# multiview-stitcher/multiview-stitcher

Measured on AMD Instinct MI355X. Metric: Mvoxels/s register+fuse, 3D tile grid, higher is better.
Workload: dtype u16 in/out, f32 accumulate, f64 coordinates

## Files before the change

multiview-stitcher_amd/csrc/mvs_context.hip:

```cpp
#include "mvs_internal.h"
#include <vector>
#include <algorithm>

#include <algorithm>
#include <cstring>

static MvsContext g_ctx[MVS_MAX_DEVICES * MVS_MAX_LANES];

MvsContext* mvs_ctx(int device) {
    if (device < 0 || (device & 0xff) >= MVS_MAX_DEVICES || (device >> 8) >= MVS_MAX_LANES) return nullptr;
    return &g_ctx[mvs_ctx_index(device)];
}

int mvs_fail(MvsContext* c, int code, const char* fmt, ...) {
    char buf[1024];
    va_list ap;
    va_start(ap, fmt);
    vsnprintf(buf, sizeof(buf), fmt, ap);
    va_end(ap);
    if (c) { c->last_error = buf; c->last_code = code; }
    return code;
}

int mvs_check_ready(int device, MvsContext** out) {
// ... 73 lines not shown
    *host = c->mbox_host;
    *dev = c->mbox_dev;
    return MVS_OK;
}

__global__ void mvs_small_copy_kernel(const uint4* __restrict__ src, uint4* __restrict__ dst, size_t n16) {
    for (size_t i = (size_t)blockIdx.x * blockDim.x + threadIdx.x; i < n16; i += (size_t)gridDim.x * blockDim.x) dst[i] = src[i];
}
int mvs_upload_from_mapped(MvsContext* c, void* dst_dev, const void* src_mapped_dev, size_t nbytes) {
    if ((((uintptr_t)dst_dev | (uintptr_t)src_mapped_dev) & 15) || (nbytes & 15))
        return mvs_fail(c, MVS_ERR_INVALID_ARG, "mvs_upload_from_mapped: 16-byte granularity");
    const size_t n16 = nbytes / 16;
    if (!n16) return MVS_OK;
    const unsigned blocks = (unsigned)std::min<size_t>((n16 + 255) / 256, 64);
    hipLaunchKernelGGL(mvs_small_copy_kernel, dim3(blocks), dim3(256), 0, c->stream, (const uint4*)src_mapped_dev, (uint4*)dst_dev, n16);
    MVS_HIP_TRY(c, hipGetLastError());
    return MVS_OK;
}

int mvs_ensure_aux_streams(MvsContext* c) {
    if (c->ev_fork) return MVS_OK;
    MVS_HIP_TRY(c, hipEventCreateWithFlags(&c->ev_fork, hipEventDisableTiming));
    int prio_lo = 0, prio_hi = 0;
    hipDeviceGetStreamPriorityRange(&prio_lo, &prio_hi);
    for (int a = 0; a < 4; ++a) {
        MVS_HIP_TRY(c, hipStreamCreateWithPriority(&c->aux_stream[a], hipStreamNonBlocking, prio_lo));
        MVS_HIP_TRY(c, hipEventCreateWithFlags(&c->ev_join[a], hipEventDisableTiming));
    }
    return MVS_OK;
}

__global__ void mvs_copy_bytes_kernel(const unsigned char* __restrict__ src, unsigned char* __restrict__ dst, size_t nbytes) {
    const size_t n16 = nbytes >> 4, tid = (size_t)blockIdx.x * blockDim.x + threadIdx.x, nth = (size_t)gridDim.x * blockDim.x;
    for (size_t i = tid; i < n16; i += nth) reinterpret_cast<uint4*>(dst)[i] = reinterpret_cast<const uint4*>(src)[i];
    for (size_t i = (n16 << 4) + tid; i < nbytes; i += nth) dst[i] = src[i];
}
int mvs_upload_small(MvsContext* c, void* dst_dev, const void* src_pinned, size_t nbytes) {
    if (!nbytes) return MVS_OK;
    void* sdev = nullptr;
    if (nbytes <= ((size_t)32 << 20) && !(((uintptr_t)dst_dev | (uintptr_t)src_pinned) & 15) &&
        hipHostGetDevicePointer(&sdev, const_cast<void*>(src_pinned), 0) == hipSuccess && sdev) {
        const unsigned blocks = (unsigned)std::min<size_t>(((nbytes >> 4) + 255) / 256 + 1, 512);
        hipLaunchKernelGGL(mvs_copy_bytes_kernel, dim3(blocks), dim3(256), 0, c->stream, (const unsigned char*)sdev, (unsigned char*)dst_dev, nbytes);
        MVS_HIP_TRY(c, hipGetLastError());
        return MVS_OK;
    }
    (void)hipGetLastError();
    MVS_HIP_TRY(c, hipMemcpyAsync(dst_dev, src_pinned, nbytes, hipMemcpyHostToDevice, c->stream));
    return MVS_OK;
}

void mvs_pinned_mark(MvsContext* c, int slot) {
    const int k = slot ? 1 : 0;
    if (hipEventRecord(c->pinned_ev[k], c->stream) == hipSuccess) c->pinned_pending[k] = true;
    else hipStreamSynchronize(c->stream);
}

static size_t pool_round(uint64_t nbytes) {
    if (nbytes == 0) nbytes = 1;
    const size_t q = nbytes >= ((size_t)1 << 20) ? ((size_t)2 << 20) : 4096;
    return (nbytes + q - 1) / q * q;
}

static void pool_flush(MvsContext* c) {
    if (c->pool_free.empty()) return;
    hipStreamSynchronize(c->stream);
    for (auto& kv : c->pool_free) hipFree(kv.second);
    c->pool_free.clear();
    c->pool_cached_bytes = 0;
}

struct MvsBoolOption { const char* key; bool MvsContext::* field; };
static const MvsBoolOption kBoolOptions[] = {
    {"force_generic", &MvsContext::force_generic},
    {"no_regions", &MvsContext::no_regions},
    {"deconv_general", &MvsContext::deconv_general},
    {"dct_general", &MvsContext::dct_general},
    {"rows_v1", &MvsContext::rows_v1},
    {"cb_mask_count", &MvsContext::cb_mask_count},
    {"cb_mask_closed_form", &MvsContext::cb_mask_closed_form},
    {"fuse_mixed", &MvsContext::fuse_mixed},
    {"serial_classes", &MvsContext::serial_classes},
    {"reg_unfused", &MvsContext::reg_unfused},
    {"ssim_two_pass", &MvsContext::ssim_two_pass},
    {"ssim_f32", &MvsContext::ssim_f32},
    {"ssim_prune", &MvsContext::ssim_prune},
    {"materialize_shifts", &MvsContext::materialize_shifts},
    {"cb_exact", &MvsContext::cb_exact},
    {"cb_blend_generic", &MvsContext::cb_blend_generic},
    {"cb_nosplit", &MvsContext::cb_nosplit},
    {"cb_unpaired", &MvsContext::cb_unpaired},
    {"fft_no_pair", &MvsContext::fft_no_pair},
    {"fft_no_slab", &MvsContext::fft_no_slab},
    {"fft_no_line", &MvsContext::fft_no_line},
};
static int set_option(MvsContext* c, const char* key, int64_t value) {
    for (const MvsBoolOption& e : kBoolOptions)
        if (!strcmp(key, e.key)) {
            c->*e.field = value != 0;
            return MVS_OK;
        }
    if (!strcmp(key, "pool_cache_limit_mb")) {
        std::lock_guard<std::mutex> plock(c->pool_mu);
        c->pool_cache_limit = (size_t)std::max<int64_t>(value, 0) << 20;
        if (c->pool_cached_bytes > c->pool_cache_limit) pool_flush(c);
        return MVS_OK;
    }
    if (!strcmp(key, "cb_taps_f64")) {
        if (value < 0 || value > 3) return mvs_fail(c, MVS_ERR_INVALID_ARG, "mvs_set_option: cb_taps_f64 is 0, 1, 2 or 3");
        c->cb_taps = (int)value;
        return MVS_OK;
    }
    if (!strcmp(key, "fft_slab_axes")) {
        if (value < 0 || value > 7) return mvs_fail(c, MVS_ERR_INVALID_ARG, "mvs_set_option: fft_slab_axes is a mask of 3 bits");
        c->fft_slab_axes = (int)value;
        return MVS_OK;
    }
    if (!strcmp(key, "ablate")) {
        c->ablate = (int)value;
        return MVS_OK;
    }
    return mvs_fail(c, MVS_ERR_INVALID_ARG, "mvs_set_option: unknown key '%s'", key);
}
struct MvsCounter { const char* key; double MvsContext::* real; long long MvsContext::* count; };
static const MvsCounter kCounters[] = {
    {"reg_alg_bytes", &MvsContext::reg_alg_bytes, nullptr},
    {"reg_alg_bytes_full", &MvsContext::reg_alg_bytes_full, nullptr},
    {"reg_pairs", nullptr, &MvsContext::reg_pairs},
    {"reg_candidates", nullptr, &MvsContext::reg_candidates},
    {"reg_rewalks", nullptr, &MvsContext::reg_rewalks},
    {"reg_pruned", nullptr, &MvsContext::reg_pruned},
    {"reg_cand_volumes", &MvsContext::reg_cand_volumes, nullptr},
    {"reg_slab_pairs", nullptr, &MvsContext::reg_slab_pairs},
    {"cb_mask_views", nullptr, &MvsContext::cb_mask_views},
    {"cb_mask_boxes", nullptr, &MvsContext::cb_mask_boxes},
    {"cb_line_launches", nullptr, &MvsContext::cb_line_launches},
    {"cb_overflows_redone", nullptr, &MvsContext::cb_overflows},
};

double mvs_rows_last_plan_ms(MvsContext* c);
double mvs_regions_last_plan_ms(MvsContext* c);
double mvs_regions_class_stat(MvsContext* c, int what, int cls);

extern "C" {

const char* mvs_version(void) { return "mvs_hip 0.1 (gfx950)"; }

int mvs_device_count(void) {
    int n = 0;
    if (hipGetDeviceCount(&n) != hipSuccess) return 0;
    return n;
}

int mvs_init(int device) {
    MvsContext* c = mvs_ctx(device);
    if (!c) return MVS_ERR_INVALID_ARG;
    std::lock_guard<std::recursive_mutex> lock(c->mu);
    if (c->ready) return MVS_OK;
    int n = 0;
    hipError_t e = hipGetDeviceCount(&n);
    if (e != hipSuccess || mvs_hip_device(device) >= n)
        return mvs_fail(c, MVS_ERR_HIP, "no HIP device %d (count=%d, %s)", mvs_hip_device(device), n,
                        hipGetErrorString(e));
    MVS_HIP_TRY(c, hipSetDevice(mvs_hip_device(device)));
    {
        const char* ev = nullptr;
#ifdef MVS_PROFILING_ABLATIONS
        ev = getenv("MVS_LANE_CU_MASK");
        if (ev) {
            const size_t pre = !strncmp(ev, "xcd", 3) ? 3 : (!strncmp(ev, "spread", 6) ? 6 : 0);
            if (!pre || ev[pre] < '1' || ev[pre] > '8' || ev[pre + 1] != '\0') ev = nullptr;
        }
#endif
        const int lane = (device >> 8) & 0xff;
        bool masked = false;
        if (ev && lane < 15) {
            hipDeviceProp_t prop;
            MVS_HIP_TRY(c, hipGetDeviceProperties(&prop, mvs_hip_device(device)));
            const int ncu = prop.multiProcessorCount;
            const bool xcd = !strncmp(ev, "xcd", 3);
            const int k = std::max(1, std::min(8, atoi(ev + (xcd ? 3 : 6))));
            std::vector<uint32_t> mask((size_t)(ncu + 31) / 32, 0u);
            for (int i = 0; i < ncu; ++i) {
                bool on;
                if (xcd) { const int x = i % 8, first = (lane * k) % 8; on = ((x - first + 8) % 8) < k; }
                else { const int slot = (i / 8) % 8, first = (lane * k) % 8; on = ((slot - first + 8) % 8) < k; }
                if (on) mask[(size_t)i / 32] |= 1u << (i % 32);
            }
            if (hipExtStreamCreateWithCUMask(&c->own_stream, (uint32_t)mask.size(), mask.data()) == hipSuccess) masked = true;
            else (void)hipGetLastError();
        }
        if (!masked) MVS_HIP_TRY(c, hipStreamCreateWithFlags(&c->own_stream, hipStreamNonBlocking));
    }
    MVS_HIP_TRY(c, hipEventCreate(&c->ev_start));
    MVS_HIP_TRY(c, hipEventCreate(&c->ev_stop));
    MVS_HIP_TRY(c, hipEventCreateWithFlags(&c->pinned_ev[0], hipEventDisableTiming));
    MVS_HIP_TRY(c, hipEventCreateWithFlags(&c->pinned_ev[1], hipEventDisableTiming));
    c->pinned_pending[0] = c->pinned_pending[1] = false;
    c->stream = c->own_stream;
    c->device = device;
    c->pool_cache_limit = ((device >> 8) ? (size_t)4 : (size_t)32) << 30;
    if (((device >> 8) & 0xff) == 0) {
        size_t f = 0, t = 0;
        if (hipMemGetInfo(&f, &t) == hipSuccess) c->pool_cache_limit = std::max(c->pool_cache_limit, t / 2);
        else (void)hipGetLastError();
    }
    {
        static const char* const env_switch[][2] = {{"MVS_SSIM_PRUNE", "ssim_prune"},   {"MVS_SSIM_F32", "ssim_f32"},
                                                    {"MVS_FUSE_MIXED", "fuse_mixed"},   {"MVS_FFT_SLAB_AXES", "fft_slab_axes"},
                                                    {"MVS_FFT_NO_SLAB", "fft_no_slab"}, {"MVS_FFT_NO_PAIR", "fft_no_pair"}};
        for (const auto& e : env_switch) {
            const char* ev = getenv(e[0]);
            if (ev && *ev) (void)set_option(c, e[1], atoi(ev));
        }
    }
    c->ready = true;
// ... 401 lines not shown
```

multiview-stitcher_amd/csrc/mvs_fft.h:

```cpp
#pragma once
#include "mvs_internal.h"

struct MvsFftFuse {
    const float* re_src = nullptr;
    const float* im_src = nullptr;
    const float2* xp_src = nullptr;
    float2* xp_p2 = nullptr;
    int xp_sel_a = 0, xp_sel_b = 0;
    bool xp_used = false;
    float* peak_val[2] = {nullptr, nullptr};
    long long* peak_idx[2] = {nullptr, nullptr};
    int peak_cap = 0;
    int n_peak = 0;
    bool src_used = false;
};
int mvs_fft3_c2c(MvsContext* c, float2* data, const int64_t shape[3], bool inverse, MvsFftFuse* fuse = nullptr);
int mvs_phasecorr_slab_axis(const MvsContext* c, const int64_t shape[3]);
int mvs_phasecorr_slab_peaks(const int64_t shape[3], int short_axis);
int mvs_phasecorr_slab(MvsContext* c, const float* a, const float* b, float2* Z, float2* CC, float2* P2, float2* dc, const int64_t shape[3],
                       int short_axis, int sel_a, int sel_b, float* const peak_val[2], long long* const peak_idx[2], float2* z0_out);
bool mvs_fft_reg_length(int n);

__device__ __forceinline__ void mvs_xpower_scales(float2 z0, long long n, float* scale_phase, float* scale_plain) {
    const float dc = fabsf(z0.x * z0.y);
    *scale_plain = (dc > 0.f && dc < INFINITY) ? ldexpf(1.f, -ilogbf(dc)) : 1.f;
    *scale_phase = ldexpf(1.f, -ilogbf((float)n));
}
__device__ __forceinline__ float2 mvs_xpower_value(float2 z, float2 m, int sel_a, int sel_b, float scale_phase, float scale_plain,
                                                   float2* p_out, float2* p1_out) {
    const float floor_ = 100.f * 1.1920928955078125e-7f;
    const float2 f = make_float2(0.5f * (z.x + m.x), 0.5f * (z.y - m.y));
    const float2 g = make_float2(0.5f * (z.y + m.y), -0.5f * (z.x - m.x));
    const float2 p = make_float2(f.x * g.x + f.y * g.y, f.y * g.x - f.x * g.y);
    const float a = fmaxf(hypotf(p.x, p.y), floor_);
    const float2 p1 = make_float2(p.x / a, p.y / a);
    *p_out = p;
    *p1_out = p1;
    const float2 pa = sel_a ? p1 : p;
    if (sel_b < 0) return pa;
    const float2 pb = sel_b ? p1 : p;
    const float sa = sel_a ? scale_phase : scale_plain, sb = sel_b ? scale_phase : scale_plain;
    return make_float2(pa.x * sa - pb.y * sb, pa.y * sa + pb.x * sb);
}
```

multiview-stitcher_amd/csrc/mvs_fft.hip:

```cpp
#include "mvs_fft.h"
#include "mvs_fft_dev.h"
#include "mvs_fft_reg.h"

#include <cmath>
#include <cstdlib>
#include <map>
#include <vector>

namespace {




__device__ __forceinline__ float2* stockham(float2* a, float2* b, int lpb, int M, int log2M, const float2* tw, bool inv) {
    const int half = M >> 1, quarter = M >> 2;
    const int log2q = log2M - 2;
    int s = 0;
    for (; s + 2 <= log2M; s += 2) {
        const int p = 1 << s;
        const int tstep = M >> (s + 2);
        for (int t = threadIdx.x; t < (lpb << log2q); t += blockDim.x) {
            const int line = t >> log2q, i = t & (quarter - 1);
            const int k = i & (p - 1);
            const int j = ((i - k) << 2) + k;
// ... 536 lines not shown
        rc = launch_pow2_lines(c, scr, p.M1, (long long)nl * p.M2, p.M2, p.M2, p.M, inv1);
        if (rc) break;
        hipLaunchKernelGGL(big_twiddle_kernel, dim3(grid(total)), dim3(256), 0, c->stream, scr, total, p.M, p.M2, log2M2, inv1 ? 1 : 0);
        rc = launch_pow2_lines(c, scr, p.M2, (long long)nl * p.M1, 1, 1, p.M2, inv1);
        if (rc) break;
        if (blu) {
            hipLaunchKernelGGL(big_mul_kernel, dim3(grid(total)), dim3(256), 0, c->stream, scr, p.bfft_t, total, p.M);
            rc = launch_pow2_lines(c, scr, p.M2, (long long)nl * p.M1, 1, 1, p.M2, true);
            if (rc) break;
            hipLaunchKernelGGL(big_twiddle_kernel, dim3(grid(total)), dim3(256), 0, c->stream, scr, total, p.M, p.M2, log2M2, 1);
            rc = launch_pow2_lines(c, scr, p.M1, (long long)nl * p.M2, p.M2, p.M2, p.M, true);
            if (rc) break;
        }
        hipLaunchKernelGGL(big_scatter_kernel, dim3(grid((long long)nl * n)), dim3(256), 0, c->stream, data, scr, l0, nl, n, p.M, p.M1, p.M2, stride,
                           inner, outer_stride, blu ? p.chirp : nullptr, inverse ? 1 : 0, blu ? 0 : 1);
    }
    hipError_t e = hipGetLastError();
    mvs_free(c->device, scr_v);
    if (rc) return rc;
    if (e != hipSuccess) return mvs_fail(c, MVS_ERR_HIP, "FFT four-step launch failed: %s", hipGetErrorString(e));
    return MVS_OK;
}

}

int mvs_fft_twiddles(MvsContext* c, int n, const float2** tw) {
    if (n < 2 || (n & (n - 1)) != 0) return mvs_fail(c, MVS_ERR_INVALID_ARG, "mvs_fft_twiddles: n = %d is not a power of two", n);
    FftPlan p;
    const int rc = get_plan(c, n, &p);
    if (rc) return rc;
    *tw = p.tw;
    return MVS_OK;
}

bool mvs_fft_reg_length(int n) {
    if (n < 2) return false;
    if (mvs_dft_line_length(n)) return true;
    if ((n & (n - 1)) == 0) return n == 64 || n == 128 || n == 256;
    int M = 1;
    while (M < 2 * n - 1) M <<= 1;
    return M >= 64 && M <= 256;
}

int mvs_fft3_c2c(MvsContext* c, float2* data, const int64_t shape[3], bool inverse, MvsFftFuse* fuse) {
    const long long nz = shape[0], ny = shape[1], nx = shape[2];
    int first_axis = -1, last_axis = -1;
    for (int axis = 2; axis >= 0; --axis)
        if (shape[axis] > 1) { if (first_axis < 0) first_axis = axis; last_axis = axis; }
    if (fuse) { fuse->n_peak = 0; fuse->src_used = false; fuse->xp_used = false; }
    for (int axis = 2; axis >= 0; --axis) {
        const int n = (int)shape[axis];
        if (n == 1) continue;
        const bool pow2n = (n & (n - 1)) == 0;
        if (n > 4096 || (!pow2n && n > 2048)) {
            int rcb;
            if (axis == 2) rcb = fft_axis_big(c, data, n, nz * ny, 1, 1, nx, inverse);
            else if (axis == 1) rcb = fft_axis_big(c, data, n, nz * nx, nx, nx, ny * nx, inverse);
            else rcb = fft_axis_big(c, data, n, ny * nx, ny * nx, ny * nx, 0, inverse);
            if (rcb) return rcb;
            continue;
        }
        FftPlan p;
        int rc = get_plan(c, n, &p);
        if (rc) return rc;
        FftArgs A;
        A.data = data;
        A.n = n; A.M = p.M; A.log2M = p.log2M;
        A.inverse = inverse ? 1 : 0;
        A.tw = p.tw; A.chirp = p.chirp; A.bfft = p.bfft;
        if (axis == 2) { A.stride = 1; A.n_lines = nz * ny; A.inner = 1; A.outer_stride = nx; }
        else if (axis == 1) { A.stride = nx; A.n_lines = nz * nx; A.inner = nx; A.outer_stride = ny * nx; }
        else { A.stride = ny * nx; A.n_lines = ny * nx; A.inner = ny * nx; A.outer_stride = 0; }
        int lpb = std::max(1, std::min(8, 4096 / p.M));
        if (axis == 2) lpb = std::max(1, std::min(8, 2048 / p.M));
        A.lpb = lpb;
        const size_t lds = (2ull * lpb * p.M + p.M / 2 + 1) * sizeof(float2);
        const long long nblocks = (A.n_lines + lpb - 1) / lpb;
        const bool reg_pow2 = !p.bluestein && (n == 64 || n == 128 || n == 256);
        const bool reg_blue = p.bluestein && p.M <= 256 && p.M >= 64;
        const bool reg_line = mvs_dft_line_length(n) && !c->fft_no_line;
        if (reg_pow2 || reg_blue || reg_line) {
            const int lpw = reg_line ? 64 : ((reg_pow2 && n == 64) || (reg_blue && p.M == 64)) ? 32 : 16;
            unsigned grid = (unsigned)((A.n_lines + lpw - 1) / lpw);
            if (fuse && axis == first_axis && fuse->re_src && fuse->im_src) {
                A.re_src = fuse->re_src;
                A.im_src = fuse->im_src;
                fuse->src_used = true;
            }
            if (fuse && axis == first_axis && axis == 2 && inverse && fuse->xp_src && fuse->xp_p2) {
                A.xp_src = fuse->xp_src; A.xp_p2 = fuse->xp_p2;
                A.xp_ny = (int)ny; A.xp_nz = (int)nz;
                A.xp_sel_a = fuse->xp_sel_a; A.xp_sel_b = fuse->xp_sel_b;
                fuse->xp_used = true;
                if (reg_pow2 && lpw % 2 == 0 && !c->fft_no_pair) {
                    const long long h = ny / 2 + 1, ncanon = h + ((nz - 1) / 2) * ny + ((nz % 2 == 0) ? h : 0);
                    A.xp_pair = 1;
                    grid = (unsigned)((ncanon + lpw / 2 - 1) / (lpw / 2));
                }
            }
            if (fuse && axis == last_axis && fuse->peak_val[0] && (long long)grid <= fuse->peak_cap) {
                for (int k = 0; k < 2; ++k) { A.peak_val[k] = fuse->peak_val[k]; A.peak_idx[k] = fuse->peak_idx[k]; }
                fuse->n_peak = (int)grid;
            }
            if (reg_line) {
                if (!(n <= 44 ? mvs_launch_dft_line_lo(c, A, grid) : mvs_launch_dft_line_hi(c, A, grid))) return mvs_fail(c, MVS_ERR_UNSUPPORTED, "FFT: no whole-line kernel for n = %d", n);
            } else if (reg_pow2) {
                if (n == 256) hipLaunchKernelGGL((fft_reg2_kernel<16, 16>), dim3(grid), dim3(256), 0, c->stream, A);
                else if (n == 128) hipLaunchKernelGGL((fft_reg2_kernel<16, 8>), dim3(grid), dim3(256), 0, c->stream, A);
                else hipLaunchKernelGGL((fft_reg2_kernel<8, 8>), dim3(grid), dim3(256), 0, c->stream, A);
            } else {
                if (p.M == 256) hipLaunchKernelGGL((bluestein_reg_kernel<16, 16>), dim3(grid), dim3(256), 0, c->stream, A);
                else if (p.M == 128) hipLaunchKernelGGL((bluestein_reg_kernel<16, 8>), dim3(grid), dim3(256), 0, c->stream, A);
                else hipLaunchKernelGGL((bluestein_reg_kernel<8, 8>), dim3(grid), dim3(256), 0, c->stream, A);
            }
        } else if (p.bluestein) {
            MVS_HIP_TRY(c, hipFuncSetAttribute((const void*)fft_lines_kernel<true>, hipFuncAttributeMaxDynamicSharedMemorySize, (int)lds));
            hipLaunchKernelGGL(fft_lines_kernel<true>, dim3((unsigned)nblocks), dim3(256), lds, c->stream, A);
        } else {
            MVS_HIP_TRY(c, hipFuncSetAttribute((const void*)fft_lines_kernel<false>, hipFuncAttributeMaxDynamicSharedMemorySize, (int)lds));
            hipLaunchKernelGGL(fft_lines_kernel<false>, dim3((unsigned)nblocks), dim3(256), lds, c->stream, A);
        }
        MVS_HIP_TRY(c, hipGetLastError());
    }
    return MVS_OK;
}
```

multiview-stitcher_amd/csrc/mvs_fft_dev.h:

```cpp
#pragma once
#include "mvs_fft.h"

struct FftArgs {
    float2* data;
    long long n_lines;
    int n;
    int M, log2M;
    long long stride;
    long long inner;
    long long outer_stride;
    int lpb;
    int inverse;
    const float2* tw;
    const float2* chirp;
    const float2* bfft;
    const float* re_src = nullptr;
    const float* im_src = nullptr;
    float* peak_val[2] = {nullptr, nullptr};
    long long* peak_idx[2] = {nullptr, nullptr};
    const float2* xp_src = nullptr;
    float2* xp_p2 = nullptr;
    int xp_ny = 0, xp_nz = 0, xp_sel_a = 0, xp_sel_b = 0;
    int xp_pair = 0;
};

__device__ __forceinline__ long long line_base(const FftArgs& A, int l) {
    const int inner = (int)A.inner;
    return (long long)(l / inner) * A.outer_stride + (l % inner);
}

__device__ __forceinline__ float2 fft_load(const FftArgs& A, long long i) {
    if (!A.re_src) return A.data[i];
    float re = A.re_src[i], im = A.im_src[i];
    re = (re != re) ? 0.f : re;
    im = (im != im) ? 0.f : im;
    return make_float2(re, im);
}
struct XpLine { long long mbase; float scale_phase, scale_plain; };
__device__ __forceinline__ XpLine xp_line(const FftArgs& A, long long l) {
    XpLine x;
    const int ky = (int)(l % A.xp_ny), kz = (int)(l / A.xp_ny);
    const int my = ky ? A.xp_ny - ky : 0, mz = kz ? A.xp_nz - kz : 0;
    x.mbase = ((long long)mz * A.xp_ny + my) * A.n;
    x.scale_phase = x.scale_plain = 1.f;
    if (A.xp_sel_b >= 0) mvs_xpower_scales(A.xp_src[0], (long long)A.xp_nz * A.xp_ny * A.n, &x.scale_phase, &x.scale_plain);
    return x;
}
__device__ __forceinline__ float2 xp_load(const FftArgs& A, const XpLine& xl, long long base, int kx) {
    const int mx = kx ? A.n - kx : 0;
    float2 p, p1;
    const float2 v = mvs_xpower_value(A.xp_src[base + kx], A.xp_src[xl.mbase + mx], A.xp_sel_a, A.xp_sel_b, xl.scale_phase, xl.scale_plain, &p, &p1);
    A.xp_p2[base + kx] = p;
    return v;
}
struct Peak2 { float v[2]; long long i[2]; };
__device__ __forceinline__ void peak_init(Peak2& p) { p.v[0] = p.v[1] = -1.f; p.i[0] = p.i[1] = 0x7fffffffffffffffLL; }
__device__ __forceinline__ void peak_add(Peak2& p, float2 o, long long idx) {
    const float a[2] = {fabsf(o.x), fabsf(o.y)};
#pragma unroll
    for (int k = 0; k < 2; ++k)
        if (a[k] > p.v[k] || (a[k] == p.v[k] && idx < p.i[k])) { p.v[k] = a[k]; p.i[k] = idx; }
}
struct SlabArgs {
    float2* data = nullptr;
    const float* re_src = nullptr;
    const float* im_src = nullptr;
    int S = 0, L = 0;
    int short_contig = 0;
    int inverse = 0;
    long long slab_stride = 0;
    long long row_stride = 0;
    const float2* tw = nullptr;
    float2* dc = nullptr;
    float* peak_val[2] = {nullptr, nullptr};
    long long* peak_idx[2] = {nullptr, nullptr};
};
bool mvs_launch_slab_lo(MvsContext* c, const SlabArgs& A, unsigned grid, size_t lds_bytes, hipError_t* err);
bool mvs_launch_slab_hi(MvsContext* c, const SlabArgs& A, unsigned grid, size_t lds_bytes, hipError_t* err);

struct LongArgs {
    const float2* Z = nullptr;
    float2* CC = nullptr;
    float2* P2 = nullptr;
    long long stride = 0;
    int PA = 0, PB = 0;
    long long pa_stride = 0;
    int sel_a = 0, sel_b = 0;
    const float2* tw = nullptr;
    const float2* dc = nullptr;
    int ndc = 0;
    long long ntotal = 0;
    float2* z0_out = nullptr;
};
int mvs_fft_twiddles(MvsContext* c, int n, const float2** tw);

constexpr bool mvs_dft_line_length(int n) {
    if (n < 17 || n > 64 || (n & (n - 1)) == 0) return false;
    for (int p = 2; p <= 19; ++p)
        while (n % p == 0) n /= p;
    return n == 1;
}
bool mvs_launch_dft_line_lo(MvsContext* c, const FftArgs& A, unsigned grid);
bool mvs_launch_dft_line_hi(MvsContext* c, const FftArgs& A, unsigned grid);
```

multiview-stitcher_amd/csrc/mvs_fft_slab.hip:

```cpp
#include "mvs_fft.h"
#include "mvs_fft_dev.h"
#include "mvs_fft_reg.h"

#include <algorithm>

namespace {

template <int R1, int R2>
__global__ __launch_bounds__(256) void long_xp_kernel(LongArgs A) {
    constexpr int M = R1 * R2, TPL = R1 > R2 ? R1 : R2, LPB = 256 / TPL;
    constexpr int PS = TPL + 1, LS = (TPL * PS > M ? TPL * PS : M) + 1;
    __shared__ float2 ex[LPB * LS];
    __shared__ float2 tw[M / 2];
    __shared__ float2 red[256];
    const int tid = (int)threadIdx.x;
    for (int t = tid; t < M / 2; t += 256) tw[t] = A.tw[t];
    red[tid] = tid < A.ndc ? A.dc[tid] : make_float2(0.f, 0.f);
    __syncthreads();
    for (int off = 128; off > 0; off >>= 1) {
        if (tid < off) red[tid] = make_float2(red[tid].x + red[tid + off].x, red[tid].y + red[tid + off].y);
        __syncthreads();
    }
    const float2 z0 = red[0];
    float scale_phase = 1.f, scale_plain = 1.f;
// ... 15 lines not shown
        }
    }
    bool live = a >= 0;
    bool selfp = false;
    if (live) {
        const int ma = a ? A.PA - a : 0, mb = b ? A.PB - b : 0;
        selfp = ma == a && mb == b;
        if (line & 1) {
            if (selfp) live = false;
            a = ma; b = mb;
        }
    }
    const long long base = live ? (long long)a * A.pa_stride + b : 0;
    float2* row = ex + line * LS;
    const float2* prow = ex + (selfp ? line : (line ^ 1)) * LS;
    if (idx < R2) {
        float2 v[R1];
#pragma unroll
        for (int q = 0; q < R1; ++q) v[q] = live ? A.Z[base + (long long)(q * R2 + idx) * A.stride] : make_float2(0.f, 0.f);
        dft_reg<R1>(v);
#pragma unroll
        for (int p = 0; p < R1; ++p) row[p * PS + idx] = p == 0 ? v[0] : cmul(v[p], tw_at(tw, idx * p, M / 2));
    }
    __syncthreads();
    float2 u[R2];
    if (idx < R1) {
#pragma unroll
        for (int j = 0; j < R2; ++j) u[j] = row[idx * PS + j];
        dft_reg<R2>(u);
    }
    __syncthreads();
    if (idx < R1) {
#pragma unroll
        for (int k = 0; k < R2; ++k) row[idx + R1 * k] = u[k];
    }
    __syncthreads();
    if (idx < R1) {
#pragma unroll
        for (int k = 0; k < R2; ++k) {
            const int m = idx + R1 * k;
            const float2 zp = prow[(M - m) & (M - 1)];
            float2 p, p1;
            const float2 w = mvs_xpower_value(u[k], zp, A.sel_a, A.sel_b, scale_phase, scale_plain, &p, &p1);
            if (live) A.P2[base + (long long)m * A.stride] = p;
            u[k] = make_float2(w.y, w.x);
        }
    }
    __syncthreads();
    if (idx < R1) {
        dft_reg<R2>(u);
#pragma unroll
        for (int p = 0; p < R2; ++p) row[p * PS + idx] = p == 0 ? u[0] : cmul(u[p], tw_at(tw, idx * p, M / 2));
    }
    __syncthreads();
    if (idx < R2) {
        float2 w[R1];
#pragma unroll
        for (int j = 0; j < R1; ++j) w[j] = row[idx * PS + j];
        dft_reg<R1>(w);
        if (live) {
#pragma unroll
            for (int k = 0; k < R1; ++k) A.CC[base + (long long)(idx + R2 * k) * A.stride] = make_float2(w[k].y, w[k].x);
        }
    }
}

bool slab_long_length(int64_t n) { return n == 64 || n == 128 || n == 256; }

}

int mvs_phasecorr_slab_axis(const MvsContext* c, const int64_t shape[3]) {
    if (c->fft_no_slab || c->fft_no_line || c->reg_unfused) return -1;
    int as = -1;
    for (int k = 0; k < 3; ++k) {
        if (slab_long_length(shape[k])) continue;
        if (shape[k] > 64 || !mvs_dft_line_length((int)shape[k]) || as >= 0) return -1;
        as = k;
    }
    if (as >= 0 && !((c->fft_slab_axes >> as) & 1)) return -1;
    return as;
}
int mvs_phasecorr_slab_peaks(const int64_t shape[3], int short_axis) { return (int)(short_axis == 0 ? shape[1] : shape[0]); }

int mvs_phasecorr_slab(MvsContext* c, const float* a, const float* b, float2* Z, float2* CC, float2* P2, float2* dc, const int64_t shape[3],
                       int short_axis, int sel_a, int sel_b, float* const peak_val[2], long long* const peak_idx[2], float2* z0_out) {
    const long long nz = shape[0], ny = shape[1], nx = shape[2];
    const int S = (int)shape[short_axis];
    SlabArgs F;
    LongArgs G;
    int L, N2;
    if (short_axis == 2) {
        L = (int)ny; N2 = (int)nz;
        F.short_contig = 1; F.slab_stride = ny * nx; F.row_stride = nx;
        G.stride = ny * nx; G.PA = (int)ny; G.PB = (int)nx; G.pa_stride = nx;
    } else if (short_axis == 1) {
        L = (int)nx; N2 = (int)nz;
        F.short_contig = 0; F.slab_stride = ny * nx; F.row_stride = nx;
        G.stride = ny * nx; G.PA = (int)ny; G.PB = (int)nx; G.pa_stride = nx;
    } else {
        L = (int)nx; N2 = (int)ny;
        F.short_contig = 0; F.slab_stride = nx; F.row_stride = ny * nx;
        G.stride = nx; G.PA = (int)nz; G.PB = (int)nx; G.pa_stride = ny * nx;
    }
    const int nslab = N2;
    if (nslab > 256) return mvs_fail(c, MVS_ERR_UNSUPPORTED, "phase correlation (slab path): %d slabs", nslab);
    const int R1 = L == 64 ? 8 : 16, R2 = L == 256 ? 16 : 8;
    F.S = S; F.L = L;
    const int lpb = 256 / std::max(R1, R2), ls = (std::max(L, R1 * (R2 + 1)) + 1) | 1;
    const size_t lds = (size_t)std::max(lpb * ls, 64 * (S | 1)) * sizeof(float2);
    int rc = mvs_fft_twiddles(c, L, &F.tw);
    if (rc) return rc;
    rc = mvs_fft_twiddles(c, N2, &G.tw);
    if (rc) return rc;
    F.data = Z; F.re_src = a; F.im_src = b; F.inverse = 0; F.dc = dc;
    hipError_t err = hipSuccess;
    if (!(S <= 44 ? mvs_launch_slab_lo(c, F, (unsigned)nslab, lds, &err) : mvs_launch_slab_hi(c, F, (unsigned)nslab, lds, &err)))
        return mvs_fail(c, MVS_ERR_UNSUPPORTED, "phase correlation (slab path): no slab kernel for S = %d", S);
    MVS_HIP_TRY(c, err);
    G.Z = Z; G.CC = CC; G.P2 = P2; G.sel_a = sel_a; G.sel_b = sel_b; G.dc = dc; G.ndc = nslab; G.ntotal = nz * ny * nx; G.z0_out = z0_out;
    {
        const long long h = G.PB / 2 + 1, ncanon = h + (long long)((G.PA - 1) / 2) * G.PB + ((G.PA % 2 == 0) ? h : 0);
        const int lpw = N2 == 64 ? 32 : 16;
        const unsigned grid = (unsigned)((ncanon + lpw / 2 - 1) / (lpw / 2));
        if (N2 == 256) MVS_DUP("long_xp", hipLaunchKernelGGL((long_xp_kernel<16, 16>), dim3(grid), dim3(256), 0, c->stream, G));
        else if (N2 == 128) hipLaunchKernelGGL((long_xp_kernel<16, 8>), dim3(grid), dim3(256), 0, c->stream, G);
        else hipLaunchKernelGGL((long_xp_kernel<8, 8>), dim3(grid), dim3(256), 0, c->stream, G);
        MVS_HIP_TRY(c, hipGetLastError());
    }
    F.data = CC; F.re_src = nullptr; F.im_src = nullptr; F.inverse = 1; F.dc = nullptr;
    for (int k = 0; k < 2; ++k) { F.peak_val[k] = peak_val[k]; F.peak_idx[k] = peak_idx[k]; }
    if (!(S <= 44 ? mvs_launch_slab_lo(c, F, (unsigned)nslab, lds, &err) : mvs_launch_slab_hi(c, F, (unsigned)nslab, lds, &err)))
        return mvs_fail(c, MVS_ERR_UNSUPPORTED, "phase correlation (slab path): no slab kernel for S = %d", S);
    MVS_HIP_TRY(c, err);
    return MVS_OK;
}
```

multiview-stitcher_amd/csrc/mvs_fft_slab.inc:

```
#include "mvs_dft_small.h"
#include "mvs_fft_dev.h"
#include "mvs_fft_reg.h"

namespace {

__device__ __forceinline__ void slab_peak_flush(Peak2 p, const SlabArgs& A) {
    __shared__ float sv[2][4];
    __shared__ long long si[2][4];
    const int lane = threadIdx.x & 63, wave = threadIdx.x >> 6;
#pragma unroll
    for (int k = 0; k < 2; ++k) {
        for (int off = 32; off > 0; off >>= 1) {
            const float ob = __shfl_down(p.v[k], off);
            const long long oi = __shfl_down(p.i[k], off);
            if (ob > p.v[k] || (ob == p.v[k] && oi < p.i[k])) { p.v[k] = ob; p.i[k] = oi; }
        }
        if (lane == 0) { sv[k][wave] = p.v[k]; si[k][wave] = p.i[k]; }
    }
    __syncthreads();
    if (threadIdx.x == 0) {
#pragma unroll
        for (int k = 0; k < 2; ++k) {
            for (int w = 1; w < 4; ++w)
                if (sv[k][w] > p.v[k] || (sv[k][w] == p.v[k] && si[k][w] < p.i[k])) { p.v[k] = sv[k][w]; p.i[k] = si[k][w]; }
            A.peak_val[k][blockIdx.x] = p.v[k];
            A.peak_idx[k][blockIdx.x] = p.i[k];
        }
    }
}

__device__ __forceinline__ float2 slab_load(const SlabArgs& A, long long g, bool inv) {
    if (A.re_src) {
        float re = A.re_src[g], im = A.im_src[g];
        re = (re != re) ? 0.f : re;
        im = (im != im) ? 0.f : im;
        return make_float2(re, im);
    }
    const float2 x = A.data[g];
    return inv ? make_float2(x.y, x.x) : x;
}

template <int S, int R1, int R2>
__device__ __forceinline__ void slab_long_axis(float2 (&v)[S], float2* __restrict__ T, const float2* __restrict__ tw, const SlabArgs& A,
                                               long long base, bool inv, Peak2& pk) {
    constexpr int M = R1 * R2, TPL = R1 > R2 ? R1 : R2, LPB = 256 / TPL, PS = R2 + 1;
    constexpr int LS = ((R1 * PS > M ? R1 * PS : M) + 1) | 1;
    constexpr int NB = (S + LPB - 1) / LPB;
    const int tid = (int)threadIdx.x;
    const int line = A.short_contig ? tid % LPB : tid / TPL, idx = A.short_contig ? tid / LPB : tid % TPL;
    float2* row = T + line * LS;
    sdft::static_for<0, NB>([&](auto b_) {
        constexpr int s0 = decltype(b_)::value * LPB;
        if (tid < M) {
            sdft::static_for<0, LPB>([&](auto l_) {
                constexpr int l = decltype(l_)::value;
                if constexpr (s0 + l < S) T[l * LS + tid] = v[s0 + l];
            });
        }
        __syncthreads();
        const int s = s0 + line;
        const bool live = s < S;
        float2 x[R1];
        if (live && idx < R2) {
#pragma unroll
            for (int q = 0; q < R1; ++q) x[q] = row[q * R2 + idx];
            dft_reg<R1>(x);
        }
        __syncthreads();
        if (live && idx < R2) {
#pragma unroll
            for (int p = 0; p < R1; ++p) row[p * PS + idx] = p == 0 ? x[0] : cmul(x[p], tw_at(tw, idx * p, M / 2));
        }
        __syncthreads();
        if (live && idx < R1) {
            float2 u[R2];
#pragma unroll
            for (int j = 0; j < R2; ++j) u[j] = row[idx * PS + j];
            dft_reg<R2>(u);
            if (A.dc && s == 0 && idx == 0) A.dc[blockIdx.x] = u[0];
#pragma unroll
            for (int k = 0; k < R2; ++k) {
                const int m = idx + R1 * k;
                const float2 o = inv ? make_float2(u[k].y, u[k].x) : u[k];
                const long long g = A.short_contig ? base + (long long)m * S + s : base + (long long)s * A.row_stride + m;
                if (A.peak_val[0]) peak_add(pk, o, g); else A.data[g] = o;
            }
        }
        __syncthreads();
    });
}

template <int S>
__global__ __launch_bounds__(256) void slab_kernel(SlabArgs A) {
    constexpr int LSH = S | 1;
    constexpr int NW = (64 * S + 255) / 256;
    extern __shared__ float2 T[];
    __shared__ float2 tw[128];
    const int tid = (int)threadIdx.x;
    const int L = A.L;
    for (int t = tid; t < L / 2; t += 256) tw[t] = A.tw[t];
    const long long base = (long long)blockIdx.x * A.slab_stride;
    const bool inv = A.inverse != 0;
    const bool mine = tid < L;
    float2 v[S];
    if (!A.short_contig) {
        sdft::static_for<0, S>([&](auto s_) {
            constexpr int s = decltype(s_)::value;
            v[s] = mine ? slab_load(A, base + (long long)s * A.row_stride + tid, inv) : make_float2(0.f, 0.f);
        });
    } else {
        sdft::static_for<0, S>([&](auto s_) { constexpr int s = decltype(s_)::value; v[s] = make_float2(0.f, 0.f); });
        for (int r0 = 0; r0 < L; r0 += 64) {
            const int nt = (L - r0 < 64 ? L - r0 : 64) * S;
            float2 w[NW];
// ... 46 lines not shown
```

multiview-stitcher_amd/csrc/mvs_fuse.hip:

```cpp
#include "mvs_internal.h"
#include "mvs_fuse_dev.h"
#include "mvs_dct_dev.h"
#include "mvs_fuse_tr.h"

#include <cmath>
#include <cstring>
#include <type_traits>

namespace {

constexpr int kBrickX = 64;
constexpr int kVPT = 4;
constexpr int kLdsTables = 8;

struct FuseParams {
    const DevView* views;
    int nviews;
    void* out;
    int oz, oy, ox;
    int tz, ty, tx;
    int nbz, nby, nbx;
    int bz, by;
    const int* cull;
    int ablate;
// ... 822 lines not shown
    }
    d->pad[0] = (order == 0) ? 0.f : 1.f;
    d->tr_ok = 1;
}

template <typename TIn, int ORDER>
__global__ __launch_bounds__(256) void resample_kernel(DevView V, float* out, int oz, int oy, int ox, float cval, int z0, int y0, int x0) {
    const long long n = (long long)oz * oy * ox;
    for (long long i = (long long)blockIdx.x * blockDim.x + threadIdx.x; i < n; i += (long long)gridDim.x * blockDim.x) {
        int x = (int)(i % ox);
        long long t = i / ox;
        int y = (int)(t % oy);
        int z = (int)(t / oy);
        const double pz = (double)(z + z0), py = (double)(y + y0), px = (double)(x + x0);
        const double cz = ((pz * V.m[0] + py * V.m[1]) + px * V.m[2]) + V.off[0];
        const double cy = ((pz * V.m[3] + py * V.m[4]) + px * V.m[5]) + V.off[1];
        const double cx = ((pz * V.m[6] + py * V.m[7]) + px * V.m[8]) + V.off[2];
        const bool inb = !(cz < 0.0 || cz > (double)(V.nz - 1) || cy < 0.0 || cy > (double)(V.ny - 1) ||
                           cx < 0.0 || cx > (double)(V.nx - 1));
        out[i] = inb ? sample_view<TIn, ORDER>(V, cz, cy, cx) : cval;
    }
}

template <typename TIn>
__global__ __launch_bounds__(256) void crop_int_kernel(const TIn* __restrict__ data, long long stride_z, long long stride_y, int nz, int ny,
                                                       int nx, int tz, int ty, int tx, float* __restrict__ out, int oz, int oy, int ox,
                                                       float cval, char* __restrict__ stats) {
    typedef TIn in8_t __attribute__((ext_vector_type(8), aligned(sizeof(TIn))));
    typedef float f4_t __attribute__((ext_vector_type(4), aligned(4)));
    const int gpr = (ox + 7) / 8;
    const long long ngroups = (long long)oz * oy * gpr;
    float smn = INFINITY, smx = -INFINITY;
    long long snv = 0;
    for (long long g = (long long)blockIdx.x * blockDim.x + threadIdx.x; g < ngroups; g += (long long)gridDim.x * blockDim.x) {
        const int xg = (int)(g % gpr) * 8;
        const long long row = g / gpr;
        const int y = (int)(row % oy), z = (int)(row / oy);
        const int iz = z + tz, iy = y + ty, ix = xg + tx;
        float* o = out + row * ox + xg;
        const bool zy = iz >= 0 && iz < nz && iy >= 0 && iy < ny;
        const TIn* p = data + (long long)iz * stride_z + (long long)iy * stride_y + ix;
        if (zy && xg + 8 <= ox && ix >= 0 && ix + 8 <= nx) {
            const in8_t v = *reinterpret_cast<const in8_t*>(p);
            f4_t a, b;
            a.x = (float)v[0]; a.y = (float)v[1]; a.z = (float)v[2]; a.w = (float)v[3];
            b.x = (float)v[4]; b.y = (float)v[5]; b.z = (float)v[6]; b.w = (float)v[7];
            *reinterpret_cast<f4_t*>(o) = a;
            *reinterpret_cast<f4_t*>(o + 4) = b;
            if (stats) {
                smn = fminf(smn, fminf(fminf(fminf(a.x, a.y), fminf(a.z, a.w)), fminf(fminf(b.x, b.y), fminf(b.z, b.w))));
                smx = fmaxf(smx, fmaxf(fmaxf(fmaxf(a.x, a.y), fmaxf(a.z, a.w)), fmaxf(fmaxf(b.x, b.y), fmaxf(b.z, b.w))));
                snv += 8;
            }
        } else {
            for (int j = 0; j < 8 && xg + j < ox; ++j) {
                const bool in = zy && ix + j >= 0 && ix + j < nx;
                const float v = in ? (float)p[j] : cval;
                o[j] = v;
                if (stats && in) { smn = fminf(smn, v); smx = fmaxf(smx, v); ++snv; }
            }
        }
    }
    if (stats) {
        for (int off = 32; off > 0; off >>= 1) {
            smn = fminf(smn, __shfl_down(smn, off));
            smx = fmaxf(smx, __shfl_down(smx, off));
            snv += __shfl_down(snv, off);
        }
        __shared__ float s_mn[4], s_mx[4];
        __shared__ long long s_nv[4];
        const int lane = threadIdx.x & 63, wave = threadIdx.x >> 6;
        if (lane == 0) { s_mn[wave] = smn; s_mx[wave] = smx; s_nv[wave] = snv; }
        __syncthreads();
        if (threadIdx.x == 0) {
            for (int w = 1; w < 4; ++w) { smn = fminf(smn, s_mn[w]); smx = fmaxf(smx, s_mx[w]); snv += s_nv[w]; }
            const int nb = gridDim.x;
            ((float*)stats)[blockIdx.x] = smn;
            ((float*)stats)[nb + blockIdx.x] = smx;
            ((long long*)(stats + (size_t)nb * 8))[blockIdx.x] = snv;
        }
    }
}

template <typename TIn>
__global__ __launch_bounds__(1024) void crop_bin_kernel(const TIn* __restrict__ data, long long stride_z, long long stride_y, int nz, int ny,
                                                       int nx, int bz, int by, int bx, int tz, int ty, int tx, float* __restrict__ out, int oz,
                                                       int oy, int ox, float cval, char* __restrict__ stats) {
    typedef float f4_t __attribute__((ext_vector_type(4), aligned(4)));
    typedef unsigned int u32x4_t __attribute__((ext_vector_type(4), aligned(4)));
    const int gpr = (ox + 7) / 8;
    const long long ngroups = (long long)oz * oy * gpr;
    const double inv = 1.0 / ((double)bz * by * bx);
    const bool pairs_aligned = (((unsigned long long)data & 3ull) == 0ull) && ((stride_z & 1ll) == 0ll) && ((stride_y & 1ll) == 0ll);
    float smn = INFINITY, smx = -INFINITY;
    long long snv = 0;
    for (long long g = (long long)blockIdx.x * blockDim.x + threadIdx.x; g < ngroups; g += (long long)gridDim.x * blockDim.x) {
        const int xg0 = (int)(g % gpr) * 8;
        const int xg = (ox >= 8 && xg0 + 8 > ox) ? ox - 8 : xg0;
        const int dup = xg0 - xg;
        const long long row = g / gpr;
        const int y = (int)(row % oy), z = (int)(row / oy);
        const int iz = z + tz, iy = y + ty, ix = xg + tx;
        float* o = out + row * ox + xg;
        const bool zy = iz >= 0 && iz < nz && iy >= 0 && iy < ny;
        const TIn* p = data + (long long)iz * bz * stride_z + (long long)iy * by * stride_y + (long long)ix * bx;
        float v[8];
        bool in[8];
        if (sizeof(TIn) == 2 && bx == 2 && pairs_aligned && zy && xg + 8 <= ox && ix >= 0 && ix + 8 <= nx) {
            unsigned int acc[8] = {0u, 0u, 0u, 0u, 0u, 0u, 0u, 0u};
            for (int dz = 0; dz < bz; ++dz)
                for (int dy = 0; dy < by; ++dy) {
                    const TIn* r = p + (long long)dz * stride_z + (long long)dy * stride_y;
                    const u32x4_t a = *reinterpret_cast<const u32x4_t*>(r);
                    const u32x4_t b = *reinterpret_cast<const u32x4_t*>(r + 8);
#pragma unroll
                    for (int k = 0; k < 4; ++k) { acc[k] += (a[k] & 0xffffu) + (a[k] >> 16); acc[4 + k] += (b[k] & 0xffffu) + (b[k] >> 16); }
                }
#pragma unroll
            for (int k = 0; k < 8; ++k) { v[k] = (float)(TIn)((double)acc[k] * inv); in[k] = true; }
        } else if (sizeof(TIn) == 2 && bx == 2 && pairs_aligned) {
            for (int j = 0; j < 8; ++j) {
                in[j] = zy && xg + j < ox && ix + j >= 0 && ix + j < nx;
                v[j] = cval;
                if (!in[j]) continue;
                unsigned int acc = 0u;
                for (int dz = 0; dz < bz; ++dz)
                    for (int dy = 0; dy < by; ++dy) {
                        const unsigned int w = *reinterpret_cast<const unsigned int*>(p + (long long)dz * stride_z + (long long)dy * stride_y + (long long)j * 2);
                        acc += (w & 0xffffu) + (w >> 16);
                    }
                v[j] = (float)(TIn)((double)acc * inv);
            }
        } else {
            for (int j = 0; j < 8; ++j) {
                in[j] = zy && xg + j < ox && ix + j >= 0 && ix + j < nx;
                v[j] = cval;
                if (!in[j]) continue;
                double acc = 0.0;
                for (int dz = 0; dz < bz; ++dz)
                    for (int dy = 0; dy < by; ++dy) {
                        const TIn* r = p + (long long)dz * stride_z + (long long)dy * stride_y + (long long)j * bx;
                        for (int dx = 0; dx < bx; ++dx) acc += (double)r[dx];
                    }
                v[j] = (float)(TIn)(acc * inv);
            }
        }
        if (xg + 8 <= ox) {
            f4_t a, b;
            a.x = v[0]; a.y = v[1]; a.z = v[2]; a.w = v[3];
            b.x = v[4]; b.y = v[5]; b.z = v[6]; b.w = v[7];
            *reinterpret_cast<f4_t*>(o) = a;
            *reinterpret_cast<f4_t*>(o + 4) = b;
        } else {
            for (int j = 0; j < 8 && xg + j < ox; ++j) o[j] = v[j];
        }
        if (stats)
            for (int j = 0; j < 8; ++j)
                if (in[j] && xg + j < ox && j >= dup) { smn = fminf(smn, v[j]); smx = fmaxf(smx, v[j]); ++snv; }
    }
    if (stats) {
        for (int off = 32; off > 0; off >>= 1) {
            smn = fminf(smn, __shfl_down(smn, off));
            smx = fmaxf(smx, __shfl_down(smx, off));
            snv += __shfl_down(snv, off);
        }
        __shared__ float s_mn[16], s_mx[16];
        __shared__ long long s_nv[16];
        const int lane = threadIdx.x & 63, wave = threadIdx.x >> 6;
        if (lane == 0) { s_mn[wave] = smn; s_mx[wave] = smx; s_nv[wave] = snv; }
        __syncthreads();
        if (threadIdx.x == 0) {
            for (int w = 1; w < (int)(blockDim.x >> 6); ++w) { smn = fminf(smn, s_mn[w]); smx = fmaxf(smx, s_mx[w]); snv += s_nv[w]; }
            const int nb = gridDim.x;
            ((float*)stats)[blockIdx.x] = smn;
            ((float*)stats)[nb + blockIdx.x] = smx;
            ((long long*)(stats + (size_t)nb * 8))[blockIdx.x] = snv;
        }
    }
}

static bool is_integer_crop(const DevView& V, int dtype, int t[3]) {
    if (dtype != MVS_U8 && dtype != MVS_U16) return false;
    const double I[9] = {1, 0, 0, 0, 1, 0, 0, 0, 1};
    for (int k = 0; k < 9; ++k)
        if (V.m[k] != I[k]) return false;
    for (int k = 0; k < 3; ++k) {
        if (!(V.off[k] == std::floor(V.off[k])) || std::fabs(V.off[k]) > 1e9) return false;
        t[k] = (int)V.off[k];
    }
    return true;
}

__global__ __launch_bounds__(256) void blend_kernel(DevView V, float* out, int oz, int oy, int ox, int z0, int y0, int x0) {
    const long long n = (long long)oz * oy * ox;
    for (long long i = (long long)blockIdx.x * blockDim.x + threadIdx.x; i < n; i += (long long)gridDim.x * blockDim.x) {
        int x = (int)(i % ox);
        long long t = i / ox;
        int y = (int)(t % oy);
        int z = (int)(t / oy);
        const double pz = (double)(z + z0), py = (double)(y + y0), px = (double)(x + x0);
        const double cz = ((pz * V.wm[0] + py * V.wm[1]) + px * V.wm[2]) + V.woff[0];
        const double cy = ((pz * V.wm[3] + py * V.wm[4]) + px * V.wm[5]) + V.woff[1];
        const double cx = ((pz * V.wm[6] + py * V.wm[7]) + px * V.wm[8]) + V.woff[2];
        out[i] = blend_weight<false>(V.edt, V.wnz, cz, cy, cx);
    }
}

struct BoxItem { const void* data; long long stride_z, stride_y; int nz, ny, nx, tz, ty, tx; float* out; int oz, oy, ox, z0, y0, x0; };
struct BoxBatch { BoxItem v[8]; int blk0[9]; };
template <typename TIn>
__global__ __launch_bounds__(256) void crop_int_batch_kernel(BoxBatch B, float cval) {
    typedef TIn in8_t __attribute__((ext_vector_type(8), aligned(sizeof(TIn))));
    typedef float f4_t __attribute__((ext_vector_type(4), aligned(4)));
    int v = 0;
    while (v < 7 && (int)blockIdx.x >= B.blk0[v + 1]) ++v;
    const BoxItem& C = B.v[v];
    const int bx = (int)blockIdx.x - B.blk0[v], nbk = B.blk0[v + 1] - B.blk0[v];
    const TIn* data = (const TIn*)C.data;
    const int gpr = (C.ox + 7) / 8;
    const long long ngroups = (long long)C.oz * C.oy * gpr;
    for (long long g = (long long)bx * blockDim.x + threadIdx.x; g < ngroups; g += (long long)nbk * blockDim.x) {
        const int xg = (int)(g % gpr) * 8;
        const long long row = g / gpr;
        const int y = (int)(row % C.oy), z = (int)(row / C.oy);
        const int iz = z + C.tz, iy = y + C.ty, ix = xg + C.tx;
        float* o = C.out + row * C.ox + xg;
        const bool zy = iz >= 0 && iz < C.nz && iy >= 0 && iy < C.ny;
        const TIn* p = data + (long long)iz * C.stride_z + (long long)iy * C.stride_y + ix;
        if (zy && xg + 8 <= C.ox && ix >= 0 && ix + 8 <= C.nx) {
            const in8_t q = *reinterpret_cast<const in8_t*>(p);
// ... 374 lines not shown
        char* s = nullptr;
        if (host_bytes) {
            s = (char*)mvs_scratch(c, 0, host_bytes);
            if (!s) return mvs_alloc_failed(c);
        }
        rc = mvs_stage_view(c, *view, es, s, &cursor, &dptr);
        if (rc) return rc;
    }
    mvs_view_t tmp = *view;
    if (!need_data) { tmp.shape[0] = tmp.shape[1] = tmp.shape[2] = 1; tmp.stride[0] = tmp.stride[1] = tmp.stride[2] = 1; }
    return fill_dev_view(c, tmp, ndim, dptr, d);
}
}

extern "C" int mvs_resample(int device, const mvs_view_t* view, const int64_t out_shape[3],
                            int32_t order, float cval, float* out, int32_t out_mem) {
    return mvs_resample_impl(device, view, out_shape, order, cval, out, out_mem, MvsResampleOpts{});
}

int mvs_resample_impl(int device, const mvs_view_t* view, const int64_t out_shape[3], int32_t order, float cval, float* out, int32_t out_mem,
                      const MvsResampleOpts& ro) {
    MvsContext* c;
    int rc = mvs_check_ready(device, &c);
    if (rc) return rc;
    std::lock_guard<std::recursive_mutex> lock(c->mu);
    if (!view || !out_shape || !out) return mvs_fail(c, MVS_ERR_INVALID_ARG, "mvs_resample: NULL argument");
    if (order != 0 && order != 1) return mvs_fail(c, MVS_ERR_UNSUPPORTED, "mvs_resample: order %d (only 0|1)", order);
    for (int k = 0; k < 3; ++k)
        if (out_shape[k] < 1 || out_shape[k] > 0x7fffffffLL)
            return mvs_fail(c, MVS_ERR_INVALID_ARG, "mvs_resample: bad out_shape");
    MVS_HIP_TRY(c, hipSetDevice(mvs_hip_device(device)));
    DevView d;
    rc = stage_single_view(c, view, 3, true, &d);
    if (rc) return rc;
    const long long n = (long long)out_shape[0] * out_shape[1] * out_shape[2];
    float* dout = out;
    if (out_mem == MVS_MEM_HOST) {
        dout = (float*)mvs_scratch(c, 1, (size_t)n * 4);
        if (!dout) return mvs_alloc_failed(c);
    }
    MVS_HIP_TRY(c, hipEventRecord(c->ev_start, c->stream));
    mvs_launch_resample(c, d, view->dtype, order, cval, dout, out_shape, nullptr, out_mem == MVS_MEM_DEVICE ? ro.stats : nullptr, ro.stats_k);
    MVS_HIP_TRY(c, hipGetLastError());
    MVS_HIP_TRY(c, hipEventRecord(c->ev_stop, c->stream));
    c->timing_valid = true;
    if (out_mem == MVS_MEM_HOST)
        MVS_HIP_TRY(c, hipMemcpyAsync(out, dout, (size_t)n * 4, hipMemcpyDeviceToHost, c->stream));
    if (!(ro.defer_sync && out_mem == MVS_MEM_DEVICE)) MVS_HIP_TRY(c, hipStreamSynchronize(c->stream));
    return MVS_OK;
}

extern "C" int mvs_blend_weights(int device, const mvs_view_t* view, int32_t ndim,
                                 const int64_t out_shape[3], float* out, int32_t out_mem) {
    MvsContext* c;
    int rc = mvs_check_ready(device, &c);
    if (rc) return rc;
    std::lock_guard<std::recursive_mutex> lock(c->mu);
    if (!view || !out_shape || !out) return mvs_fail(c, MVS_ERR_INVALID_ARG, "mvs_blend_weights: NULL argument");
    if (ndim != 2 && ndim != 3) return mvs_fail(c, MVS_ERR_INVALID_ARG, "mvs_blend_weights: ndim must be 2 or 3");
    MVS_HIP_TRY(c, hipSetDevice(mvs_hip_device(device)));
    DevView d;
    rc = stage_single_view(c, view, ndim, false, &d);
    if (rc) return rc;
    const long long n = (long long)out_shape[0] * out_shape[1] * out_shape[2];
    float* dout = out;
    if (out_mem == MVS_MEM_HOST) {
        dout = (float*)mvs_scratch(c, 1, (size_t)n * 4);
        if (!dout) return mvs_alloc_failed(c);
    }
    int nblocks = (int)std::min<long long>((n + 255) / 256, 256 * 16);
    MVS_HIP_TRY(c, hipEventRecord(c->ev_start, c->stream));
    hipLaunchKernelGGL(blend_kernel, dim3(nblocks), dim3(256), 0, c->stream, d, dout, (int)out_shape[0],
                       (int)out_shape[1], (int)out_shape[2], 0, 0, 0);
    MVS_HIP_TRY(c, hipGetLastError());
    MVS_HIP_TRY(c, hipEventRecord(c->ev_stop, c->stream));
    c->timing_valid = true;
    if (out_mem == MVS_MEM_HOST)
        MVS_HIP_TRY(c, hipMemcpyAsync(out, dout, (size_t)n * 4, hipMemcpyDeviceToHost, c->stream));
    MVS_HIP_TRY(c, hipStreamSynchronize(c->stream));
    return MVS_OK;
}


int mvs_crop_bin_impl(int device, const mvs_view_t* view, const int32_t bin[3], const int64_t out_shape[3], float* out, const MvsResampleOpts& ro) {
    MvsContext* c;
    int rc = mvs_check_ready(device, &c);
    if (rc) return rc;
    std::lock_guard<std::recursive_mutex> lock(c->mu);
    if (!view || !bin || !out_shape || !out) return mvs_fail(c, MVS_ERR_INVALID_ARG, "mvs_crop_bin: NULL argument");
    if ((view->dtype != MVS_U8 && view->dtype != MVS_U16) || view->mem != MVS_MEM_DEVICE || view->stride[2] != 1)
        return mvs_fail(c, MVS_ERR_UNSUPPORTED, "mvs_crop_bin: needs a device-resident uint8 / uint16 window with unit x stride");
    const double I[9] = {1, 0, 0, 0, 1, 0, 0, 0, 1};
    int t[3], nb3[3];
    for (int k = 0; k < 9; ++k)
        if (view->matrix[k] != I[k]) return mvs_fail(c, MVS_ERR_UNSUPPORTED, "mvs_crop_bin: the view must be a whole-pixel translation");
    for (int k = 0; k < 3; ++k) {
        if (bin[k] < 1 || view->shape[k] < bin[k] || view->shape[k] % bin[k] || out_shape[k] < 1 || out_shape[k] > 0x7fffffffLL)
            return mvs_fail(c, MVS_ERR_INVALID_ARG, "mvs_crop_bin: bad bin / shape on axis %d", k);
        if (!(view->offset[k] == std::floor(view->offset[k])) || std::fabs(view->offset[k]) > 1e9)
            return mvs_fail(c, MVS_ERR_UNSUPPORTED, "mvs_crop_bin: the view must be a whole-pixel translation");
        t[k] = (int)view->offset[k];
        nb3[k] = (int)(view->shape[k] / bin[k]);
    }
    if ((long long)bin[0] * bin[1] > 16384) return mvs_fail(c, MVS_ERR_UNSUPPORTED, "mvs_crop_bin: bin too large");
    MVS_HIP_TRY(c, hipSetDevice(mvs_hip_device(device)));
    const long long ng = (long long)out_shape[0] * out_shape[1] * ((out_shape[2] + 7) / 8);
    const int nthr = 1024;
    int nblk = (int)std::min<long long>((ng + nthr - 1) / nthr, 256 * 8);
    char* stats = nullptr;
    if (ro.stats && ro.stats->base && ro.stats->nb > 0) {
        stats = ro.stats->base + (size_t)(ro.stats_k & 1) * (size_t)ro.stats->nb * 16;
        nblk = ro.stats->nb;
        ro.stats->done[ro.stats_k & 1] = true;
    }
    if (view->dtype == MVS_U8)
        MVS_DUP("crop", hipLaunchKernelGGL(crop_bin_kernel<unsigned char>, dim3(nblk), dim3(nthr), 0, c->stream, (const unsigned char*)view->data, (long long)view->stride[0],
                           (long long)view->stride[1], nb3[0], nb3[1], nb3[2], (int)bin[0], (int)bin[1], (int)bin[2], t[0], t[1], t[2], out,
                           (int)out_shape[0], (int)out_shape[1], (int)out_shape[2], NAN, stats));
    else
        MVS_DUP("crop", hipLaunchKernelGGL(crop_bin_kernel<unsigned short>, dim3(nblk), dim3(nthr), 0, c->stream, (const unsigned short*)view->data, (long long)view->stride[0],
                           (long long)view->stride[1], nb3[0], nb3[1], nb3[2], (int)bin[0], (int)bin[1], (int)bin[2], t[0], t[1], t[2], out,
                           (int)out_shape[0], (int)out_shape[1], (int)out_shape[2], NAN, stats));
    MVS_HIP_TRY(c, hipGetLastError());
    if (!ro.defer_sync) MVS_HIP_TRY(c, hipStreamSynchronize(c->stream));
    return MVS_OK;
}

int mvs_fill_dev_view(MvsContext* c, const mvs_view_t& v, int ndim, const void* dev_data, DevView* d) {
    return fill_dev_view(c, v, ndim, dev_data, d);
}

void mvs_launch_resample(MvsContext* c, const DevView& d, int dtype, int order, float cval, float* out, const int64_t shape[3], const int* box0,
                         MvsCropStats* crop_stats, int crop_stats_k) {
    const long long n = (long long)shape[0] * shape[1] * shape[2];
    int t[3];
    const int b0[3] = {box0 ? box0[0] : 0, box0 ? box0[1] : 0, box0 ? box0[2] : 0};
    if (!c->force_generic && is_integer_crop(d, dtype, t)) {
        for (int k = 0; k < 3; ++k) t[k] += b0[k];
        const long long ng = (long long)shape[0] * shape[1] * ((shape[2] + 7) / 8);
        int nb = (int)std::min<long long>((ng + 255) / 256, 256 * 16);
        char* stats = nullptr;
        if (crop_stats && crop_stats->base && crop_stats->nb > 0 && cval != cval && !box0) {
            stats = crop_stats->base + (size_t)(crop_stats_k & 1) * (size_t)crop_stats->nb * 16;
            nb = crop_stats->nb;
            crop_stats->done[crop_stats_k & 1] = true;
        }
        if (dtype == MVS_U8)
            hipLaunchKernelGGL(crop_int_kernel<unsigned char>, dim3(nb), dim3(256), 0, c->stream, (const unsigned char*)d.data, d.stride_z, d.stride_y,
                               d.nz, d.ny, d.nx, t[0], t[1], t[2], out, (int)shape[0], (int)shape[1], (int)shape[2], cval, stats);
        else
            hipLaunchKernelGGL(crop_int_kernel<unsigned short>, dim3(nb), dim3(256), 0, c->stream, (const unsigned short*)d.data, d.stride_z, d.stride_y,
                               d.nz, d.ny, d.nx, t[0], t[1], t[2], out, (int)shape[0], (int)shape[1], (int)shape[2], cval, stats);
        return;
    }
    const int nblocks = (int)std::min<long long>((n + 255) / 256, 256 * 16);
#define MVS_RS(T, O) hipLaunchKernelGGL((resample_kernel<T, O>), dim3(nblocks), dim3(256), 0, c->stream, d, out, \
                                        (int)shape[0], (int)shape[1], (int)shape[2], cval, b0[0], b0[1], b0[2])
    mvs_dispatch_dtype(dtype, [&](auto tag) {
        using T = decltype(tag);
        if (order) MVS_RS(T, 1); else MVS_RS(T, 0);
    });
#undef MVS_RS
}

void mvs_launch_blend(MvsContext* c, const DevView& d, float* out, const int64_t shape[3], const int* box0) {
    const long long n = (long long)shape[0] * shape[1] * shape[2];
    const int nblocks = (int)std::min<long long>((n + 255) / 256, 256 * 16);
    hipLaunchKernelGGL(blend_kernel, dim3(nblocks), dim3(256), 0, c->stream, d, out, (int)shape[0], (int)shape[1], (int)shape[2],
                       box0 ? box0[0] : 0, box0 ? box0[1] : 0, box0 ? box0[2] : 0);
}

void mvs_launch_boxes_batch(MvsContext* c, const DevView* hviews, const DevView* dviews, int n_views, int dtype, int order, float cval,
                            float* const* res_out, float* const* blend_out, const int64_t (*shapes)[3], const int (*box0)[3], const TrView* tr) {
    if (n_views > 8 || c->force_generic) {
        for (int i = 0; i < n_views; ++i) {
            if (shapes[i][0] * shapes[i][1] * shapes[i][2] == 0) continue;
            mvs_launch_resample(c, hviews[i], dtype, order, cval, res_out[i], shapes[i], box0[i]);
            mvs_launch_blend(c, hviews[i], blend_out[i], shapes[i], box0[i]);
        }
        return;
    }
    BoxBatch R, W;
    memset(&R, 0, sizeof(R));
    memset(&W, 0, sizeof(W));
    int nr = 0, nw = 0;
    for (int i = 0; i < 8; ++i) {
        R.blk0[i] = nr;
        W.blk0[i] = nw;
        if (i >= n_views) continue;
        const long long n = (long long)shapes[i][0] * shapes[i][1] * shapes[i][2];
        if (n == 0) continue;
        BoxItem it;
        memset(&it, 0, sizeof(it));
        it.oz = (int)shapes[i][0]; it.oy = (int)shapes[i][1]; it.ox = (int)shapes[i][2];
        it.z0 = box0[i][0]; it.y0 = box0[i][1]; it.x0 = box0[i][2];
        int t[3];
        if (is_integer_crop(hviews[i], dtype, t)) {
            it.data = hviews[i].data; it.stride_z = hviews[i].stride_z; it.stride_y = hviews[i].stride_y;
            it.nz = hviews[i].nz; it.ny = hviews[i].ny; it.nx = hviews[i].nx;
            it.tz = t[0] + box0[i][0]; it.ty = t[1] + box0[i][1]; it.tx = t[2] + box0[i][2];
            it.out = res_out[i];
            R.v[i] = it;
            const long long ng = (long long)shapes[i][0] * shapes[i][1] * ((shapes[i][2] + 7) / 8);
            nr += (int)std::min<long long>((ng + 255) / 256, 256 * 16);
        } else {
            mvs_launch_resample(c, hviews[i], dtype, order, cval, res_out[i], shapes[i], box0[i]);
        }
// ... 62 lines not shown
```

multiview-stitcher_amd/csrc/mvs_internal.h:

```cpp
#pragma once
#include <hip/hip_runtime.h>

#include <cstdarg>
#include <cstdint>
#include <cstdio>
#include <map>
#include <mutex>
#include <unordered_map>
#include <string>
#include <vector>

#include "mvs_hip.h"

#define MVS_MAX_DEVICES 16
#define MVS_MAX_LANES 16
static inline int mvs_hip_device(int id) { return id & 0xff; }
static inline int mvs_ctx_index(int id) { return ((id >> 8) & 0xff) * MVS_MAX_DEVICES + (id & 0xff); }

struct MvsScratch {
    void* ptr = nullptr;
    size_t cap = 0;
};

struct MvsContext {
    int device = -1;
    bool ready = false;
    hipStream_t own_stream = nullptr;
    hipStream_t stream = nullptr;
    hipEvent_t ev_start = nullptr, ev_stop = nullptr;
    bool timing_valid = false;
    int ablate = 0;
    bool force_generic = false;
    double reg_alg_bytes = 0.0;
    double reg_alg_bytes_full = 0.0;
    long long reg_pairs = 0, reg_candidates = 0, reg_pruned = 0;
    long long reg_slab_pairs = 0;
    double reg_cand_volumes = 0.0;
    hipStream_t aux_stream[4] = {nullptr, nullptr, nullptr, nullptr};
    hipEvent_t ev_fork = nullptr, ev_join[4] = {nullptr, nullptr, nullptr, nullptr};
    bool fuse_mixed = false;
    bool serial_classes = false;
    bool reg_unfused = false;
    bool ssim_f32 = true;
    long long reg_rewalks = 0;
    bool ssim_prune = true;
    bool fft_no_pair = false;
    bool ssim_two_pass = false;
    bool materialize_shifts = false;
    std::recursive_mutex mu;
    std::string last_error;
    MvsScratch dev[16];
    void* pinned = nullptr;
    size_t pinned_cap = 0;
    void* pinned2 = nullptr;
    size_t pinned2_cap = 0;
    hipEvent_t pinned_ev[2] = {nullptr, nullptr};
    hipEvent_t ticket_ev[32] = {};
    uint32_t ticket_next = 0;
    bool pinned_pending[2] = {false, false};
    int last_code = 0;
    void* mbox_host = nullptr;
    void* mbox_dev = nullptr;
    size_t mbox_cap = 0;
    uint64_t mbox_gen = 0;
    bool cb_mask_closed_form = false;
    bool cb_mask_count = false;
    long long cb_mask_views = 0, cb_mask_boxes = 0;
    bool cb_exact = false;
    bool cb_blend_generic = false;
    int cb_taps = 1;
    int* cb_flag_host = nullptr;
    int* cb_flag_dev = nullptr;
    long long cb_overflows = 0, cb_line_launches = 0;
    bool cb_nosplit = false;
    bool cb_unpaired = false;
    int fft_slab_axes = 4;
    bool fft_no_slab = false;
    bool fft_no_line = false;
    bool no_regions = false;
    bool deconv_general = false;
    bool dct_general = false;
    bool rows_v1 = false;
    std::mutex pool_mu;
    std::multimap<size_t, void*> pool_free;
    std::unordered_map<void*, size_t> pool_live;
    size_t pool_cached_bytes = 0;
    long long pool_misses = 0, pool_releases = 0;
    double pool_miss_bytes = 0.0;
    size_t pool_cache_limit = (size_t)32 << 30;
};

struct MvsScoreOpts {
    bool both_crops_finite = false;
    bool argmax_only = false;
    double value_bound = INFINITY;
    const float* raw_u16_keys[2] = {nullptr, nullptr};
    float raw_range[4] = {0.f, 0.f, 0.f, 0.f};
};
#ifdef MVS_PROFILING_ABLATIONS
bool mvs_dup_kernel(const char* tag);
#define MVS_DUP(tag, ...) do { __VA_ARGS__; if (mvs_dup_kernel(tag)) { __VA_ARGS__; } } while (0)
#else
#define MVS_DUP(tag, ...) do { __VA_ARGS__; } while (0)
#endif
struct MvsCropStats {
    char* base = nullptr;
    int nb = 0;
    uint64_t gen = 0;
    bool done[2] = {false, false};
};
struct MvsResampleOpts {
    bool defer_sync = false;
    MvsCropStats* stats = nullptr;
    int stats_k = 0;
};
int mvs_score_candidates_impl(int device, const float* fixed, const float* moving, int32_t mem, int32_t ndim, const int64_t shape[3],
                              const double* t_candidates, int32_t n_candidates, int32_t region_mode, double data_range, double im1_min,
                              int32_t quality_for_all, double* ssim_out, double* spearman_out, int32_t* code_out, const MvsScoreOpts& so);
int mvs_crop_bin_impl(int device, const mvs_view_t* view, const int32_t bin[3], const int64_t out_shape[3], float* out, const MvsResampleOpts& ro);
int mvs_resample_impl(int device, const mvs_view_t* view, const int64_t out_shape[3], int32_t order, float cval, float* out, int32_t out_mem,
                      const MvsResampleOpts& ro);

MvsContext* mvs_ctx(int device);
bool mvs_transfer_is_ticket(uint64_t ticket);
int mvs_transfer_event(MvsContext* c, uint64_t ticket, hipEvent_t* ev);
void mvs_transfer_shutdown(int dev);
int mvs_fail(MvsContext* c, int code, const char* fmt, ...);
int mvs_check_ready(int device, MvsContext** out);
void* mvs_scratch(MvsContext* c, int slot, size_t nbytes);
void* mvs_pinned(MvsContext* c, size_t nbytes);
void* mvs_pinned_slot(MvsContext* c, int slot, size_t nbytes);
void mvs_pinned_mark(MvsContext* c, int slot);
int mvs_mailbox(MvsContext* c, size_t nbytes, void** host, void** dev);
int mvs_ensure_aux_streams(MvsContext* c);
int mvs_upload_from_mapped(MvsContext* c, void* dst_dev, const void* src_mapped_dev, size_t nbytes);
int mvs_upload_small(MvsContext* c, void* dst_dev, const void* src_pinned, size_t nbytes);

static inline int mvs_alloc_failed(const MvsContext* c) { return c->last_code ? c->last_code : MVS_ERR_HIP; }

#define MVS_HIP_TRY(c, expr)                                                         \
    do {                                                                             \
        hipError_t _e = (expr);                                                      \
        if (_e != hipSuccess) {                                                      \
            (void)hipGetLastError();  \
            return mvs_fail((c), _e == hipErrorOutOfMemory ? MVS_ERR_OUT_OF_MEMORY : MVS_ERR_HIP,  \
                            "%s failed: %s (%s:%d)", #expr, hipGetErrorString(_e), __FILE__, __LINE__); \
        }                                                                            \
    } while (0)

struct MvsWorkArea {
    MvsContext* c;
    void* ptr = nullptr;
    explicit MvsWorkArea(MvsContext* ctx) : c(ctx) {}
    MvsWorkArea(const MvsWorkArea&) = delete;
    MvsWorkArea& operator=(const MvsWorkArea&) = delete;
    int alloc(size_t nbytes) { return mvs_malloc(c->device, nbytes, &ptr); }
    int release() {
        void* p = ptr;
        ptr = nullptr;
        return mvs_free(c->device, p);
    }
    ~MvsWorkArea() {
        if (!ptr) return;
        (void)hipStreamSynchronize(c->stream);
        mvs_free(c->device, ptr);
    }
};

static inline size_t align_up(size_t v, size_t a = 256) { return (v + a - 1) / a * a; }

static inline size_t mvs_dtype_size(int dtype) {
    switch (dtype) {
        case MVS_U8: return 1;
        case MVS_U16: return 2;
        case MVS_F32: return 4;
        default: return 0;
    }
}

template <typename F>
static inline void mvs_dispatch_dtype(int dtype, F&& f) {
    switch (dtype) {
        case MVS_U8: f((unsigned char)0); break;
        case MVS_U16: f((unsigned short)0); break;
        default: f(0.f); break;
    }
}
```

multiview-stitcher_amd/csrc/mvs_pair.hip:

```cpp
#include "mvs_internal.h"

int mvs_rescale_pair_device(MvsContext* c, const float* in0, const float* in1, long long n, float* out0, float* out1,
                            float mn[2], float mx[2], long long nvalid[2], long long n_not_u16[2], const MvsCropStats* parked);

#include <algorithm>
#include <cmath>
#include <vector>

static int register_crops_impl(int device, const float* fixed, const float* moving, int32_t mem, int32_t ndim, const int64_t shape[3],
                               int32_t upsample_factor, int32_t region_mode, int32_t constant_check, double t_out[3], double* quality_out,
                               int32_t* status_out, int32_t* n_candidates_out, const MvsCropStats* parked);

extern "C" int mvs_register_crops(int device, const float* fixed, const float* moving, int32_t mem, int32_t ndim, const int64_t shape[3],
                                  int32_t upsample_factor, int32_t region_mode, int32_t constant_check, double t_out[3], double* quality_out,
                                  int32_t* status_out, int32_t* n_candidates_out) {
    return register_crops_impl(device, fixed, moving, mem, ndim, shape, upsample_factor, region_mode, constant_check, t_out, quality_out, status_out,
                               n_candidates_out, nullptr);
}

static int register_crops_impl(int device, const float* fixed, const float* moving, int32_t mem, int32_t ndim, const int64_t shape[3],
                               int32_t upsample_factor, int32_t region_mode, int32_t constant_check, double t_out[3], double* quality_out,
                               int32_t* status_out, int32_t* n_candidates_out, const MvsCropStats* parked) {
    MvsContext* c;
    int rc = mvs_check_ready(device, &c);
    if (rc) return rc;
    std::lock_guard<std::recursive_mutex> lock(c->mu);
    if (!fixed || !moving || !shape || !t_out || !quality_out || !status_out)
        return mvs_fail(c, MVS_ERR_INVALID_ARG, "mvs_register_crops: NULL argument");
    if (ndim != 2 && ndim != 3) return mvs_fail(c, MVS_ERR_INVALID_ARG, "mvs_register_crops: ndim must be 2 or 3");
    if (ndim == 2 && shape[0] != 1) return mvs_fail(c, MVS_ERR_INVALID_ARG, "mvs_register_crops: 2D needs shape[0]==1");
    if (region_mode < -1 || region_mode > 1) return mvs_fail(c, MVS_ERR_INVALID_ARG, "mvs_register_crops: region_mode must be -1, 0 or 1");
    const int64_t n = shape[0] * shape[1] * shape[2];
    if (n < 1) return mvs_fail(c, MVS_ERR_INVALID_ARG, "mvs_register_crops: empty shape");
    const int k0 = 3 - ndim;
    t_out[0] = t_out[1] = t_out[2] = 0.0;
    *quality_out = NAN;
    *status_out = 0;
    if (n_candidates_out) *n_candidates_out = 0;

    float* r0 = (float*)mvs_scratch(c, 9, (size_t)n * 4);
    float* r1 = (float*)mvs_scratch(c, 10, (size_t)n * 4);
    if (!r0 || !r1) return mvs_alloc_failed(c);
    float min0, max0, min1, max1;
    int64_t nv0, nv1;
    const float* raw_keys0 = nullptr;
    const float* raw_keys1 = nullptr;
    if (mem == MVS_MEM_DEVICE) {
        MVS_HIP_TRY(c, hipSetDevice(mvs_hip_device(device)));
        float mn[2], mx[2];
        long long nv[2], not_u16[2];
        rc = mvs_rescale_pair_device(c, fixed, moving, n, r0, r1, mn, mx, nv, not_u16, parked);
        if (rc) return rc;
        raw_keys0 = (not_u16[0] == 0) ? fixed : nullptr;
        raw_keys1 = (not_u16[1] == 0) ? moving : nullptr;
        min0 = mn[0]; max0 = mx[0]; nv0 = nv[0];
        min1 = mn[1]; max1 = mx[1]; nv1 = nv[1];
    } else {
        rc = mvs_rescale_intensity(device, fixed, mem, n, r0, MVS_MEM_DEVICE, &min0, &max0, &nv0);
        if (rc) return rc;
        rc = mvs_rescale_intensity(device, moving, mem, n, r1, MVS_MEM_DEVICE, &min1, &max1, &nv1);
        if (rc) return rc;
    }
    if (constant_check && (min0 == max0 || min1 == max1)) {
        *status_out = 2;
        return MVS_OK;
    }
    const bool has_nan = (nv0 < n) || (nv1 < n);
    if (region_mode < 0) region_mode = has_nan ? 1 : 0;

    const int32_t norms[2] = {1, 0};
    double shifts[6];
    rc = mvs_phasecorr_multi(device, r0, r1, MVS_MEM_DEVICE, ndim, shape, norms, 2, upsample_factor, shifts, nullptr, nullptr);
    if (rc) return rc;
    std::vector<std::vector<float>> estimates;
    for (int e = 0; e < 2; ++e) {
        std::vector<float> s(ndim);
        for (int k = 0; k < ndim; ++k) s[k] = (float)shifts[3 * e + k0 + k];
        estimates.push_back(s);
    }
    if (has_nan) estimates.push_back(std::vector<float>(ndim, 0.f));

    auto rescaled_range = [](float mn, float mx, int64_t nv, float& lo, float& hi) {
        if (nv == 0) { lo = hi = NAN; return; }
        if (mx != mn) { lo = 0.f; hi = 1.f; } else { lo = hi = mn; }
    };
    float lo0, hi0, lo1, hi1;
    rescaled_range(min0, max0, nv0, lo0, hi0);
    rescaled_range(min1, max1, nv1, lo1, hi1);
    auto nanmaxf = [](float a, float b) { return (a != a) ? b : (b != b) ? a : std::max(a, b); };
    auto nanminf = [](float a, float b) { return (a != a) ? b : (b != b) ? a : std::min(a, b); };
    const float data_range = nanmaxf(hi0, hi1) - nanminf(lo0, lo1);
    const double im1_min = (double)lo1;

    float max_shift = 0.f;
    for (int k = 0; k < ndim; ++k) max_shift = std::max(max_shift, (float)shape[k0 + k]);
    std::vector<double> cand;
    for (const std::vector<float>& sc : estimates) {
        int nvar[3], idx[3] = {0, 0, 0};
        float var[3][4];
        for (int d = 0; d < ndim; ++d) {
            const float nn = (float)shape[k0 + d];
            if (sc[d] == 0.f) { nvar[d] = 1; var[d][0] = sc[d]; }
            else { nvar[d] = 4; var[d][0] = sc[d]; var[d][1] = -sc[d]; var[d][2] = -(sc[d] - nn); var[d][3] = -sc[d] - nn; }
        }
        for (;;) {
            float amax = 0.f;
            for (int d = 0; d < ndim; ++d) amax = std::max(amax, std::fabs(var[d][idx[d]]));
            if (amax < max_shift)
                for (int d = 0; d < ndim; ++d) cand.push_back((double)var[d][idx[d]]);
            int d = ndim - 1;
            while (d >= 0 && ++idx[d] == nvar[d]) { idx[d] = 0; --d; }
            if (d < 0) break;
        }
    }
    const int n_all = (int)(cand.size() / (size_t)ndim);
    if (n_candidates_out) *n_candidates_out = n_all;
    if (n_all == 0) {
        *status_out = 1;
        return MVS_OK;
    }

    std::vector<int> uniq_of(n_all, -1);
    std::vector<double> uniq;
    for (int i = 0; i < n_all; ++i) {
        const int nu = (int)(uniq.size() / (size_t)ndim);
        for (int u = 0; u < nu && uniq_of[i] < 0; ++u) {
            bool same = true;
            for (int d = 0; d < ndim; ++d) same = same && (uniq[(size_t)u * ndim + d] == cand[(size_t)i * ndim + d]);
            if (same) uniq_of[i] = u;
        }
        if (uniq_of[i] < 0) {
            uniq_of[i] = nu;
            for (int d = 0; d < ndim; ++d) uniq.push_back(cand[(size_t)i * ndim + d]);
        }
    }
    const int n_uniq = (int)(uniq.size() / (size_t)ndim);
    std::vector<double> ssim_u(n_uniq), spear_u(n_uniq);
    std::vector<int32_t> code_u(n_uniq);
    MvsScoreOpts so;
    so.both_crops_finite = !has_nan && std::isfinite(min0) && std::isfinite(max0) && std::isfinite(min1) && std::isfinite(max1) &&
                           !c->materialize_shifts;
    so.raw_u16_keys[0] = c->materialize_shifts ? nullptr : raw_keys0;
    so.raw_u16_keys[1] = c->materialize_shifts ? nullptr : raw_keys1;
    so.raw_range[0] = min0; so.raw_range[1] = max0; so.raw_range[2] = min1; so.raw_range[3] = max1;
    so.argmax_only = true;
    so.value_bound = (double)std::max(std::max(std::fabs(lo0), std::fabs(hi0)), std::max(std::fabs(lo1), std::fabs(hi1)));
    const double cand_vol0 = c->reg_cand_volumes;
    rc = mvs_score_candidates_impl(device, r0, r1, MVS_MEM_DEVICE, ndim, shape, uniq.data(), n_uniq, region_mode, (double)data_range, im1_min, 0,
                                   ssim_u.data(), spear_u.data(), code_u.data(), so);
    if (rc) return rc;
    int n_scored = 0;
    for (int u = 0; u < n_uniq; ++u) n_scored += (code_u[u] == 0) ? 1 : 0;
    double cand_vol = c->reg_cand_volumes - cand_vol0;
    if (!(cand_vol > 0.0)) { cand_vol = (double)n_scored; c->reg_cand_volumes = cand_vol0 + cand_vol; }
    c->reg_alg_bytes += (double)n * (2.0 * 28.0 + 20.0 * cand_vol + 64.0);
    c->reg_alg_bytes_full += (double)n * (2.0 * 28.0 + 20.0 * (double)n_scored + 64.0);
    c->reg_pairs += 1;
    c->reg_candidates += n_scored;

    int best_pos = -1, pos = 0;
    double best = 0.0, best_quality = NAN;
    for (int i = 0; i < n_all; ++i) {
        const int u = uniq_of[i];
        if (code_u[u] == 2) continue;
        const double sv = ssim_u[u];
        if (sv == sv && (best_pos < 0 || sv > best)) { best = sv; best_pos = pos; best_quality = spear_u[u]; }
        ++pos;
    }
    if (best_pos < 0) {
        *status_out = 3;
        return MVS_OK;
    }
    for (int d = 0; d < ndim; ++d) t_out[k0 + d] = cand[(size_t)best_pos * ndim + d];
    *quality_out = best_quality;
    return MVS_OK;
}


static int register_views_impl(int device, const mvs_view_t* fixed_view, const mvs_view_t* moving_view, int32_t ndim, const int64_t out_shape[3],
                               int32_t upsample_factor, int32_t region_mode, int32_t constant_check, const int32_t* bin, double t_out[3],
                               double* quality_out, int32_t* status_out, int32_t* n_candidates_out);

extern "C" int mvs_register_views(int device, const mvs_view_t* fixed_view, const mvs_view_t* moving_view, int32_t ndim,
                                  const int64_t out_shape[3], int32_t upsample_factor, int32_t region_mode, int32_t constant_check,
                                  double t_out[3], double* quality_out, int32_t* status_out, int32_t* n_candidates_out) {
    return register_views_impl(device, fixed_view, moving_view, ndim, out_shape, upsample_factor, region_mode, constant_check, nullptr, t_out,
                               quality_out, status_out, n_candidates_out);
}

static int register_views_impl(int device, const mvs_view_t* fixed_view, const mvs_view_t* moving_view, int32_t ndim, const int64_t out_shape[3],
                               int32_t upsample_factor, int32_t region_mode, int32_t constant_check, const int32_t* bin, double t_out[3],
                               double* quality_out, int32_t* status_out, int32_t* n_candidates_out) {
    MvsContext* c;
    int rc = mvs_check_ready(device, &c);
    if (rc) return rc;
    std::lock_guard<std::recursive_mutex> lock(c->mu);
    if (!fixed_view || !moving_view || !out_shape) return mvs_fail(c, MVS_ERR_INVALID_ARG, "mvs_register_views: NULL argument");
    for (int k = 0; k < 3; ++k)
        if (out_shape[k] < 1) return mvs_fail(c, MVS_ERR_INVALID_ARG, "mvs_register_views: bad out_shape");
    const int64_t n = out_shape[0] * out_shape[1] * out_shape[2];
    float* crop0 = (float*)mvs_scratch(c, 11, (size_t)n * 4);
    float* crop1 = (float*)mvs_scratch(c, 12, (size_t)n * 4);
    if (!crop0 || !crop1) return mvs_alloc_failed(c);
    const int nb_stats = (int)std::min<int64_t>(std::min<int64_t>((n + 255) / 256, 256 * 8), 512);
    void *mb_host = nullptr, *mb_dev = nullptr;
    rc = mvs_mailbox(c, (size_t)nb_stats * 32, &mb_host, &mb_dev);
    if (rc) return rc;
    MvsCropStats stats;
    stats.base = c->reg_unfused ? nullptr : (char*)mb_dev;
    stats.nb = nb_stats;
    stats.gen = c->mbox_gen;
    MvsResampleOpts ro;
    ro.defer_sync = true;
    ro.stats = &stats;
    ro.stats_k = 0;
    rc = bin ? mvs_crop_bin_impl(device, fixed_view, bin, out_shape, crop0, ro) : mvs_resample_impl(device, fixed_view, out_shape, 1, NAN, crop0, MVS_MEM_DEVICE, ro);
    if (rc) return rc;
    ro.stats_k = 1;
    rc = bin ? mvs_crop_bin_impl(device, moving_view, bin, out_shape, crop1, ro) : mvs_resample_impl(device, moving_view, out_shape, 1, NAN, crop1, MVS_MEM_DEVICE, ro);
    if (rc) return rc;
    return register_crops_impl(device, crop0, crop1, MVS_MEM_DEVICE, ndim, out_shape, upsample_factor, region_mode, constant_check, t_out,
                               quality_out, status_out, n_candidates_out, &stats);
}


#include <atomic>
#include <condition_variable>
#include <thread>

namespace {
inline int64_t bisect_left(const double* c, int64_t n, double x) {
    int64_t lo = 0, hi = n;
    while (lo < hi) { const int64_t mid = (lo + hi) / 2; if (c[mid] < x) lo = mid + 1; else hi = mid; }
    return lo;
}
inline int64_t bisect_right(const double* c, int64_t n, double x) {
    int64_t lo = 0, hi = n;
    while (lo < hi) { const int64_t mid = (lo + hi) / 2; if (x < c[mid]) hi = mid; else lo = mid + 1; }
    return lo;
}
inline double around10(double x) { return std::rint(x * 1e10) / 1e10; }
inline double pymax(double a, double b) { return b > a ? b : a; }
inline double pymin(double a, double b) { return b < a ? b : a; }
}

extern "C" int mvs_plan_pairs(int32_t ndim, int32_t n_views, const double* const* coords, const int64_t* coord_len, const double* translation,
                              const double* tol, int32_t n_pairs, const int32_t* pairs, int64_t* windows_out, double* out_origin_out,
                              double* out_spacing_out, int64_t* out_shape_out, double* matrix_diag_out, double* offset_out, int32_t* status_out) {
    if (ndim < 1 || ndim > 3 || n_views < 1 || n_pairs < 0 || !coords || !coord_len || !translation || (n_pairs > 0 && !pairs) || !windows_out ||
        !out_origin_out || !out_spacing_out || !out_shape_out || !matrix_diag_out || !offset_out || !status_out)
        return MVS_ERR_INVALID_ARG;
    for (int v = 0; v < n_views * ndim; ++v)
        if (!coords[v] || coord_len[v] < 1) return MVS_ERR_INVALID_ARG;
    for (int p = 0; p < n_pairs; ++p) {
        const int v[2] = {pairs[2 * p], pairs[2 * p + 1]};
        status_out[p] = 1;
        if (v[0] < 0 || v[1] < 0 || v[0] >= n_views || v[1] >= n_views) return MVS_ERR_INVALID_ARG;
        double lowers[2][3], uppers[2][3];
        bool ok = true;
        for (int k = 0; k < ndim && ok; ++k) {
            double lo2[2], hi2[2];
            for (int i = 0; i < 2; ++i) {
                const double* c = coords[(size_t)v[i] * ndim + k];
                int64_t n = coord_len[(size_t)v[i] * ndim + k];
                double o = c[0];
                const double s = n > 1 ? c[1] - c[0] : 1.0;
                if (tol) { n = n + (int64_t)std::ceil(2 * tol[k] / s); o = o - tol[k]; }
                const double t = translation[(size_t)v[i] * ndim + k];
                lo2[i] = o + t;
                hi2[i] = ((double)(n - 1) * 1.0 * s + o) + t;
            }
            const double lo = pymax(lo2[0], lo2[1]), hi = pymin(hi2[0], hi2[1]);
            if (hi < lo) { ok = false; break; }
            const double up = 1.0 * (hi - lo) + lo;
            for (int i = 0; i < 2; ++i) {
                const double t = translation[(size_t)v[i] * ndim + k];
                lowers[i][k] = lo + (-t);
                uppers[i][k] = up + (-t);
            }
        }
        if (!ok) continue;
        double origins[2][3], spacings[2][3];
        for (int i = 0; i < 2 && ok; ++i)
            for (int k = 0; k < ndim; ++k) {
                const double* c = coords[(size_t)v[i] * ndim + k];
                const int64_t n = coord_len[(size_t)v[i] * ndim + k];
                const double gs = n > 1 ? c[1] - c[0] : 1.0;
                const double start = lowers[i][k] - 1e-6 - gs, stop = uppers[i][k] + 1e-6 + gs;
                const int64_t a = bisect_left(c, n, start), b = bisect_right(c, n, stop);
                if (b <= a) { ok = false; break; }
                windows_out[(((size_t)p * 2 + i) * 3 + k) * 2] = a;
                windows_out[(((size_t)p * 2 + i) * 3 + k) * 2 + 1] = b;
                origins[i][k] = c[a];
                spacings[i][k] = (b - a > 1) ? c[a + 1] - c[a] : 1.0;
            }
        if (!ok) continue;
        for (int k = 0; k < ndim; ++k) {
            const double osp = pymax(spacings[0][k], spacings[1][k]);
            const double oo = lowers[0][k];
            out_spacing_out[(size_t)p * 3 + k] = osp;
            out_origin_out[(size_t)p * 3 + k] = oo;
            out_shape_out[(size_t)p * 3 + k] = (int64_t)std::floor((uppers[0][k] - lowers[0][k]) / osp + 1);
            const double t_rel = translation[(size_t)v[0] * ndim + k] + (-translation[(size_t)v[1] * ndim + k]);
            for (int i = 0; i < 2; ++i) {
                const double tt = i == 0 ? 0.0 : t_rel;
// ... 139 lines not shown
```

multiview-stitcher_amd/csrc/mvs_reg.hip:

```cpp
#include "mvs_fft.h"

#include <rocprim/warp/warp_reduce.hpp>

#include <cfloat>
#include <cmath>
#include <vector>

namespace {

__global__ void pack_pair_kernel(const float* __restrict__ a, const float* __restrict__ b, float2* __restrict__ dst, long long n) {
    for (long long i = (long long)blockIdx.x * blockDim.x + threadIdx.x; i < n; i += (long long)gridDim.x * blockDim.x) {
        float va = a[i], vb = b[i];
        if (va != va) va = 0.f;
        if (vb != vb) vb = 0.f;
        dst[i] = make_float2(va, vb);
    }
}

__global__ void xpower_packed_kernel(const float2* __restrict__ Z, float2* __restrict__ P1, float2* __restrict__ P2,
                                     float2* __restrict__ C, int nz, int ny, int nx, int sel_a, int sel_b) {
    const long long n = (long long)nz * ny * nx;
    float scale_phase = 1.f, scale_plain = 1.f;
    if (sel_b >= 0) mvs_xpower_scales(Z[0], n, &scale_phase, &scale_plain);
    for (long long i = (long long)blockIdx.x * blockDim.x + threadIdx.x; i < n; i += (long long)gridDim.x * blockDim.x) {
// ... 210 lines not shown
#pragma unroll
                for (int i = 0; i < 4; ++i) {
                    if (64 * i >= nx) continue;
                    r.x += kx[i].x * s[j][b][i].x - kx[i].y * s[j][b][i].y;
                    r.y += kx[i].x * s[j][b][i].y + kx[i].y * s[j][b][i].x;
                }
                WaveSum().reduce(r.x, r.x, wsum[wave]);
                WaveSum().reduce(r.y, r.y, wsum[wave]);
                if (lane == 0) red[wave][(j * U + b) * U + a] = r;
            }
        }
    __syncthreads();
    if (threadIdx.x < 2 * U * U) {
        const int t = threadIdx.x, j = t / (U * U), ba = t % (U * U);
        float2 r = red[0][t];
        for (int w = 1; w < 4; ++w) { r.x += red[w][t].x; r.y += red[w][t].y; }
        q.out[j][(long long)blockIdx.x * (U * U) + ba] = r;
    }
}

__global__ __launch_bounds__(256) void updft_mid_kernel(const float2* __restrict__ in, const float2* __restrict__ K, float2* __restrict__ out,
                                                        int n_outer, int n_red, int n_inner, int U, int kdiv = 1) {
    const long long total = (long long)n_outer * U * n_inner;
    const int lane = threadIdx.x & 63;
    for (long long t = (long long)blockIdx.x * 4 + (threadIdx.x >> 6); t < total; t += (long long)gridDim.x * 4) {
        const int i = (int)(t % n_inner);
        const int b = (int)((t / n_inner) % U);
        const int o = (int)(t / ((long long)n_inner * U));
        float2 acc = make_float2(0.f, 0.f);
        for (int r = lane; r < n_red; r += 64) {
            const float2 v = in[((long long)o * n_red + r) * n_inner + i];
            const float2 k = kdiv == 1 ? K[b * n_red + r] : K[b * (n_red / kdiv) + r / kdiv];
            acc.x += k.x * v.x - k.y * v.y;
            acc.y += k.x * v.y + k.y * v.x;
        }
        for (int off = 32; off > 0; off >>= 1) {
            acc.x += __shfl_down(acc.x, off);
            acc.y += __shfl_down(acc.y, off);
        }
        if (lane == 0) out[t] = acc;
    }
}

__global__ __launch_bounds__(256) void nanminmax_kernel(const float* __restrict__ a, long long n, float* __restrict__ pmin,
                                                        float* __restrict__ pmax, long long* __restrict__ pvalid) {
    float mn = INFINITY, mx = -INFINITY;
    long long nv = 0;
    for (long long i = (long long)blockIdx.x * blockDim.x + threadIdx.x; i < n; i += (long long)gridDim.x * blockDim.x) {
        const float v = a[i];
        if (v == v) {
            mn = fminf(mn, v); mx = fmaxf(mx, v); ++nv;
            if (!(v >= 0.f && v <= 65535.f && v == floorf(v))) nv += 1ll << 32;
        }
    }
    for (int off = 32; off > 0; off >>= 1) {
        mn = fminf(mn, __shfl_down(mn, off));
        mx = fmaxf(mx, __shfl_down(mx, off));
        nv += __shfl_down(nv, off);
    }
    __shared__ float smn[4], smx[4];
    __shared__ long long snv[4];
    const int lane = threadIdx.x & 63, wave = threadIdx.x >> 6;
    if (lane == 0) { smn[wave] = mn; smx[wave] = mx; snv[wave] = nv; }
    __syncthreads();
    if (threadIdx.x == 0) {
        for (int w = 1; w < 4; ++w) { mn = fminf(mn, smn[w]); mx = fmaxf(mx, smx[w]); nv += snv[w]; }
        pmin[blockIdx.x] = mn; pmax[blockIdx.x] = mx; pvalid[blockIdx.x] = nv;
    }
}

__global__ void rescale_kernel(const float* __restrict__ src, float* __restrict__ dst, long long n, float lo, float hi, int degenerate) {
    const float d = hi - lo;
    for (long long i = (long long)blockIdx.x * blockDim.x + threadIdx.x; i < n; i += (long long)gridDim.x * blockDim.x) {
        float v = src[i];
        if (v == v) {
            v = fminf(fmaxf(v, lo), hi);
            if (!degenerate) v = (v - lo) / d;
            v = v * 1.0f + 0.0f;
        }
        dst[i] = v;
    }
}

struct PairPtrs { const float* in[2]; float* out[2]; float lo[2], hi[2]; int degenerate[2]; };
__global__ __launch_bounds__(256) void nanminmax_pair_kernel(PairPtrs P, long long n, char* __restrict__ partials, int nb) {
    const int k = blockIdx.y;
    const float* __restrict__ a = P.in[k];
    char* part = partials + (size_t)k * nb * 16;
    float mn = INFINITY, mx = -INFINITY;
    long long nv = 0;
    for (long long i = (long long)blockIdx.x * blockDim.x + threadIdx.x; i < n; i += (long long)gridDim.x * blockDim.x) {
        const float v = a[i];
        if (v == v) {
            mn = fminf(mn, v); mx = fmaxf(mx, v); ++nv;
            if (!(v >= 0.f && v <= 65535.f && v == floorf(v))) nv += 1ll << 32;
        }
    }
    for (int off = 32; off > 0; off >>= 1) {
        mn = fminf(mn, __shfl_down(mn, off));
        mx = fmaxf(mx, __shfl_down(mx, off));
        nv += __shfl_down(nv, off);
    }
    __shared__ float smn[4], smx[4];
    __shared__ long long snv[4];
    const int lane = threadIdx.x & 63, wave = threadIdx.x >> 6;
    if (lane == 0) { smn[wave] = mn; smx[wave] = mx; snv[wave] = nv; }
    __syncthreads();
    if (threadIdx.x == 0) {
        for (int w = 1; w < 4; ++w) { mn = fminf(mn, smn[w]); mx = fmaxf(mx, smx[w]); nv += snv[w]; }
        ((float*)part)[blockIdx.x] = mn;
        ((float*)part)[nb + blockIdx.x] = mx;
        ((long long*)(part + (size_t)nb * 8))[blockIdx.x] = nv;
    }
}
__global__ void rescale_pair_kernel(PairPtrs P, long long n) {
    const int k = blockIdx.y;
    const float* __restrict__ src = P.in[k];
    float* __restrict__ dst = P.out[k];
    const float lo = P.lo[k], hi = P.hi[k];
    const int degenerate = P.degenerate[k];
    const float d = hi - lo;
    for (long long i = (long long)blockIdx.x * blockDim.x + threadIdx.x; i < n; i += (long long)gridDim.x * blockDim.x) {
        float v = src[i];
        if (v == v) {
            v = fminf(fmaxf(v, lo), hi);
            if (!degenerate) v = (v - lo) / d;
            v = v * 1.0f + 0.0f;
        }
        dst[i] = v;
    }
}

inline int grid_for(long long n) { return (int)std::min<long long>((n + 255) / 256, 256 * 8); }

__global__ void peek_kernel(const unsigned int* __restrict__ src, unsigned int* __restrict__ dst, int nwords) {
    for (int i = threadIdx.x; i < nwords; i += blockDim.x) dst[i] = src[i];
}

inline double fftfreq(int n, double d, int x) {
    const int half = (n - 1) / 2 + 1;
    return (double)(x < half ? x : x - n) / ((double)n * d);
}

}

int mvs_device_nanminmax(MvsContext* c, const float* d_in, long long n, float* mn, float* mx, long long* nvalid) {
    const int nb = grid_for(n);
    char* scratch = (char*)mvs_scratch(c, 3, (size_t)nb * 16);
    if (!scratch) return mvs_alloc_failed(c);
    float* pmin = (float*)scratch;
    float* pmax = pmin + nb;
    long long* pval = (long long*)(scratch + (size_t)nb * 8);
    hipLaunchKernelGGL(nanminmax_kernel, dim3(nb), dim3(256), 0, c->stream, d_in, n, pmin, pmax, pval);
    MVS_HIP_TRY(c, hipGetLastError());
    std::vector<char> h((size_t)nb * 16);
    MVS_HIP_TRY(c, hipMemcpyAsync(h.data(), scratch, h.size(), hipMemcpyDeviceToHost, c->stream));
    MVS_HIP_TRY(c, hipStreamSynchronize(c->stream));
    const float* hmin = (const float*)h.data();
    const float* hmax = hmin + nb;
    const long long* hval = (const long long*)(h.data() + (size_t)nb * 8);
    float a = INFINITY, b = -INFINITY;
    long long v = 0;
    for (int i = 0; i < nb; ++i) { a = std::min(a, hmin[i]); b = std::max(b, hmax[i]); v += hval[i]; }
    v &= 0xffffffffll;
    if (v == 0) { a = NAN; b = NAN; }
    *mn = a; *mx = b; *nvalid = v;
    return MVS_OK;
}

int mvs_rescale_pair_device(MvsContext* c, const float* in0, const float* in1, long long n, float* out0, float* out1,
                            float mn[2], float mx[2], long long nvalid[2], long long n_not_u16[2], const MvsCropStats* parked) {
    const int nb = std::min(grid_for(n), 512);
    void *mb_host = nullptr, *mb_dev = nullptr;
    int rcm = mvs_mailbox(c, (size_t)nb * 32, &mb_host, &mb_dev);
    if (rcm) return rcm;
    char* scratch = (char*)mb_dev;
    PairPtrs PP;
    PP.in[0] = in0; PP.in[1] = in1; PP.out[0] = out0; PP.out[1] = out1;
    if (!(parked && parked->done[0] && parked->done[1] && parked->nb == nb && parked->gen == c->mbox_gen && (void*)parked->base == mb_dev))
        hipLaunchKernelGGL(nanminmax_pair_kernel, dim3(nb, 2), dim3(256), 0, c->stream, PP, n, scratch, nb);
    MVS_HIP_TRY(c, hipGetLastError());
    MVS_HIP_TRY(c, hipStreamSynchronize(c->stream));
    for (int k = 0; k < 2; ++k) {
        const char* part = (const char*)mb_host + (size_t)k * nb * 16;
        const float* hmin = (const float*)part;
        const float* hmax = hmin + nb;
        const long long* hval = (const long long*)(part + (size_t)nb * 8);
        float a = INFINITY, b = -INFINITY;
        long long v = 0;
        for (int i = 0; i < nb; ++i) { a = std::min(a, hmin[i]); b = std::max(b, hmax[i]); v += hval[i]; }
        n_not_u16[k] = v >> 32;
        v &= 0xffffffffll;
        if (v == 0) { a = NAN; b = NAN; }
        mn[k] = a; mx[k] = b; nvalid[k] = v;
        PP.lo[k] = a; PP.hi[k] = b; PP.degenerate[k] = a == b ? 1 : 0;
    }
    MVS_DUP("rescale", hipLaunchKernelGGL(rescale_pair_kernel, dim3(nb, 2), dim3(256), 0, c->stream, PP, n));
    MVS_HIP_TRY(c, hipGetLastError());
    return MVS_OK;
}

int mvs_stage_float_volume(MvsContext* c, const float* src, int32_t mem, long long n, int slot, float** dptr) {
    if (mem == MVS_MEM_DEVICE) { *dptr = (float*)src; return MVS_OK; }
    float* d = (float*)mvs_scratch(c, slot, (size_t)n * 4);
    if (!d) return mvs_alloc_failed(c);
    MVS_HIP_TRY(c, hipMemcpyAsync(d, src, (size_t)n * 4, hipMemcpyHostToDevice, c->stream));
    *dptr = d;
    return MVS_OK;
}

extern "C" int mvs_rescale_intensity(int device, const float* in, int32_t mem, int64_t n, float* out, int32_t out_mem,
                                     float* min_out, float* max_out, int64_t* nvalid_out) {
    MvsContext* c;
    int rc = mvs_check_ready(device, &c);
    if (rc) return rc;
    std::lock_guard<std::recursive_mutex> lock(c->mu);
    if (!in || !out || n < 1) return mvs_fail(c, MVS_ERR_INVALID_ARG, "mvs_rescale_intensity: bad argument");
    MVS_HIP_TRY(c, hipSetDevice(mvs_hip_device(device)));
    float* din;
    rc = mvs_stage_float_volume(c, in, mem, n, 4, &din);
    if (rc) return rc;
    float mn, mx;
    long long nv;
    rc = mvs_device_nanminmax(c, din, n, &mn, &mx, &nv);
    if (rc) return rc;
    float* dout = out;
    if (out_mem == MVS_MEM_HOST) {
        dout = (float*)mvs_scratch(c, 5, (size_t)n * 4);
        if (!dout) return mvs_alloc_failed(c);
    }
    hipLaunchKernelGGL(rescale_kernel, dim3(grid_for(n)), dim3(256), 0, c->stream, din, dout, (long long)n, mn, mx, mn == mx ? 1 : 0);
    MVS_HIP_TRY(c, hipGetLastError());
    if (out_mem == MVS_MEM_HOST) MVS_HIP_TRY(c, hipMemcpyAsync(out, dout, (size_t)n * 4, hipMemcpyDeviceToHost, c->stream));
    MVS_HIP_TRY(c, hipStreamSynchronize(c->stream));
    if (min_out) *min_out = mn;
    if (max_out) *max_out = mx;
    if (nvalid_out) *nvalid_out = nv;
    return MVS_OK;
}

extern "C" int mvs_fft_c2c(int device, void* data, int32_t mem, int32_t ndim, const int64_t shape[3], int32_t inverse) {
    MvsContext* c;
    int rc = mvs_check_ready(device, &c);
    if (rc) return rc;
    std::lock_guard<std::recursive_mutex> lock(c->mu);
    if (!data || !shape || (ndim != 2 && ndim != 3)) return mvs_fail(c, MVS_ERR_INVALID_ARG, "mvs_fft_c2c: bad argument");
    for (int k = 0; k < 3; ++k)
        if (shape[k] < 1) return mvs_fail(c, MVS_ERR_INVALID_ARG, "mvs_fft_c2c: bad shape");
    if (ndim == 2 && shape[0] != 1) return mvs_fail(c, MVS_ERR_INVALID_ARG, "mvs_fft_c2c: 2D needs shape[0]==1");
    MVS_HIP_TRY(c, hipSetDevice(mvs_hip_device(device)));
    const size_t bytes = (size_t)shape[0] * shape[1] * shape[2] * sizeof(float2);
    float2* d = (float2*)data;
    if (mem == MVS_MEM_HOST) {
        d = (float2*)mvs_scratch(c, 6, bytes);
        if (!d) return mvs_alloc_failed(c);
        MVS_HIP_TRY(c, hipMemcpyAsync(d, data, bytes, hipMemcpyHostToDevice, c->stream));
    }
    rc = mvs_fft3_c2c(c, d, shape, inverse != 0);
    if (rc) return rc;
    if (mem == MVS_MEM_HOST) MVS_HIP_TRY(c, hipMemcpyAsync(data, d, bytes, hipMemcpyDeviceToHost, c->stream));
    MVS_HIP_TRY(c, hipStreamSynchronize(c->stream));
    return MVS_OK;
}

extern "C" int mvs_phasecorr(int device, const float* fixed, const float* moving, int32_t mem, int32_t ndim,
                             const int64_t shape[3], int32_t normalization, int32_t upsample_factor,
                             double shift_out[3], int64_t peak_index_out[3], float* peak_abs_out) {
    return mvs_phasecorr_multi(device, fixed, moving, mem, ndim, shape, &normalization, 1, upsample_factor, shift_out,
                               peak_index_out, peak_abs_out);
}

extern "C" int mvs_phasecorr_multi(int device, const float* fixed, const float* moving, int32_t mem, int32_t ndim,
                                   const int64_t shape[3], const int32_t* normalizations, int32_t n_norm,
                                   int32_t upsample_factor, double* shifts_out, int64_t* peak_indices_out,
                                   float* peak_abs_out_all) {
    MvsContext* c;
    int rc = mvs_check_ready(device, &c);
    if (rc) return rc;
    std::lock_guard<std::recursive_mutex> lock(c->mu);
    if (!fixed || !moving || !shape || !shifts_out || !normalizations || n_norm < 1)
        return mvs_fail(c, MVS_ERR_INVALID_ARG, "mvs_phasecorr: NULL argument");
    if (ndim != 2 && ndim != 3) return mvs_fail(c, MVS_ERR_INVALID_ARG, "mvs_phasecorr: ndim must be 2 or 3");
    if (upsample_factor < 1) return mvs_fail(c, MVS_ERR_INVALID_ARG, "mvs_phasecorr: upsample_factor < 1");
    for (int k = 0; k < 3; ++k)
        if (shape[k] < 1) return mvs_fail(c, MVS_ERR_INVALID_ARG, "mvs_phasecorr: bad shape");
    if (ndim == 2 && shape[0] != 1) return mvs_fail(c, MVS_ERR_INVALID_ARG, "mvs_phasecorr: 2D needs shape[0]==1");
    MVS_HIP_TRY(c, hipSetDevice(mvs_hip_device(device)));
    const long long n = (long long)shape[0] * shape[1] * shape[2];
    const int nz = (int)shape[0], ny = (int)shape[1], nx = (int)shape[2];

    float *da, *db;
    rc = mvs_stage_float_volume(c, fixed, mem, n, 4, &da);
    if (rc) return rc;
    rc = mvs_stage_float_volume(c, moving, mem, n, 5, &db);
    if (rc) return rc;
    float2* Z = (float2*)mvs_scratch(c, 6, (size_t)n * 8 * 4);
    if (!Z) return mvs_alloc_failed(c);
    float2* P1 = Z + n;
    float2* P2 = P1 + n;
    float2* CC = P2 + n;

    MVS_HIP_TRY(c, hipEventRecord(c->ev_start, c->stream));
    const int gb = grid_for(n);
    int first_axis = -1, last_axis = -1;
    for (int axis = 2; axis >= 0; --axis)
        if (shape[axis] > 1) { if (first_axis < 0) first_axis = axis; last_axis = axis; }
    const int slab_axis = (ndim == 3 && n_norm == 2 && (normalizations[0] != 0) != (normalizations[1] != 0) && !c->materialize_shifts &&
                           (int)ceilf((float)upsample_factor * 1.5f) <= 4)
                              ? mvs_phasecorr_slab_axis(c, shape) : -1;
    if (slab_axis >= 0) {
        rc = MVS_OK;
    } else if (first_axis >= 0 && mvs_fft_reg_length((int)shape[first_axis]) && !c->reg_unfused) {
        MvsFftFuse ff;
        ff.re_src = da;
        ff.im_src = db;
        rc = mvs_fft3_c2c(c, Z, shape, false, &ff);
    } else {
        hipLaunchKernelGGL(pack_pair_kernel, dim3(gb), dim3(256), 0, c->stream, da, db, Z, n);
        rc = mvs_fft3_c2c(c, Z, shape, false);
    }
    if (rc) return rc;
  const bool packed = n_norm == 2 && (normalizations[0] != 0) != (normalizations[1] != 0) && !c->materialize_shifts;
  const int up_U0 = (int)ceilf((float)upsample_factor * 1.5f);
  const size_t res_elems = upsample_factor > 1 ? (ndim == 3 ? (size_t)up_U0 * up_U0 * up_U0 : (size_t)up_U0 * up_U0) : 0;
  int ga = std::min(gb, 512);
  {
      int la = -1;
      for (int axis = 2; axis >= 0; --axis) if (shape[axis] > 1) la = axis;
      if (la >= 0 && mvs_fft_reg_length((int)shape[la])) ga = std::max<long long>(ga, (n / shape[la] + 15) / 16);
      if (slab_axis >= 0) ga = std::max(ga, mvs_phasecorr_slab_peaks(shape, slab_axis));
  }
  const size_t mb_red = (size_t)ga * 32, mb_z0 = mb_red, mb_res = mb_red + 256, mb_res_stride = align_up(res_elems * sizeof(float2));
  void *mb_host = nullptr, *mb_dev = nullptr;
  const size_t mb_k = mb_res + mb_res_stride * (size_t)n_norm;
  const size_t mb_kbytes = upsample_factor > 1 ? align_up((size_t)up_U0 * (size_t)(nz + ny + nx) * sizeof(float2)) : 0;
  rc = mvs_mailbox(c, mb_k + mb_kbytes * (size_t)n_norm, &mb_host, &mb_dev);
  if (rc) return rc;
  char* red = (char*)mb_dev;
  const char* hred = (const char*)mb_host;
  float packed_scale[2] = {1.f, 1.f};
  int n_red_packed = ga;
  const bool fuse_xp = slab_axis >= 0 || (packed && first_axis == 2 && mvs_fft_reg_length((int)nx) && up_U0 <= 4 && !c->reg_unfused);
  const bool fuse_yx = fuse_xp && ndim == 3 && up_U0 == 3 && nx <= 256 && ny >= 4;
  const int yx_chunks = fuse_yx ? std::max(1, std::min(kYxChunksMax, ((int)ny + kYxRows - 1) / kYxRows)) : 1;
  if (packed && slab_axis >= 0) {
    float* pv[2] = {(float*)red, (float*)(red + (size_t)ga * 16)};
    long long* pi[2] = {(long long*)(red + (size_t)ga * 8), (long long*)(red + (size_t)ga * 24)};
    rc = mvs_phasecorr_slab(c, da, db, Z, CC, P2, P1 , shape, slab_axis, normalizations[0] ? 1 : 0,
                            normalizations[1] ? 1 : 0, pv, pi, (float2*)((char*)mb_dev + mb_z0));
    if (rc) return rc;
    n_red_packed = mvs_phasecorr_slab_peaks(shape, slab_axis);
    c->reg_slab_pairs += 1;
    MVS_HIP_TRY(c, hipStreamSynchronize(c->stream));
    const float2 z0 = *(const float2*)((const char*)mb_host + mb_z0);
    const float dc = std::fabs(z0.x * z0.y);
    const float s_plain = (dc > 0.f && dc < INFINITY) ? std::ldexp(1.f, -std::ilogb(dc)) : 1.f;
    const float s_phase = std::ldexp(1.f, -std::ilogb((float)n));
    for (int ch = 0; ch < 2; ++ch) packed_scale[ch] = normalizations[ch] ? s_phase : s_plain;
  } else if (packed) {
    if (!fuse_xp)
        hipLaunchKernelGGL(xpower_packed_kernel, dim3(gb), dim3(256), 0, c->stream, Z, P1, P2, CC, nz, ny, nx, normalizations[0] ? 1 : 0,
                           normalizations[1] ? 1 : 0);
    MvsFftFuse fp;
    if (last_axis >= 0 && mvs_fft_reg_length((int)shape[last_axis]) && !c->reg_unfused) {
        fp.peak_val[0] = (float*)red; fp.peak_idx[0] = (long long*)(red + (size_t)ga * 8);
        fp.peak_val[1] = (float*)(red + (size_t)ga * 16); fp.peak_idx[1] = (long long*)(red + (size_t)ga * 24);
        fp.peak_cap = ga;
    }
    if (fuse_xp) { fp.xp_src = Z; fp.xp_p2 = P2; fp.xp_sel_a = normalizations[0] ? 1 : 0; fp.xp_sel_b = normalizations[1] ? 1 : 0; }
    rc = mvs_fft3_c2c(c, CC, shape, true, &fp);
    if (rc) return rc;
    if (fuse_xp && !fp.xp_used) return mvs_fail(c, MVS_ERR_UNSUPPORTED, "phase correlation: the fused cross-power pass was not taken");
    if (fp.n_peak > 0) {
        n_red_packed = fp.n_peak;
        hipLaunchKernelGGL(peek_kernel, dim3(1), dim3(64), 0, c->stream, (const unsigned int*)Z, (unsigned int*)((char*)mb_dev + mb_z0), 2);
    } else {
        hipLaunchKernelGGL(argmax_abs2_kernel, dim3(ga), dim3(256), 0, c->stream, CC, n, (float*)red, (long long*)(red + (size_t)ga * 8),
                           (float*)(red + (size_t)ga * 16), (long long*)(red + (size_t)ga * 24), Z, (float2*)((char*)mb_dev + mb_z0));
    }
    MVS_HIP_TRY(c, hipGetLastError());
    MVS_HIP_TRY(c, hipStreamSynchronize(c->stream));
    const float2 z0 = *(const float2*)((const char*)mb_host + mb_z0);
    const float dc = std::fabs(z0.x * z0.y);
    const float s_plain = (dc > 0.f && dc < INFINITY) ? std::ldexp(1.f, -std::ilogb(dc)) : 1.f;
    const float s_phase = std::ldexp(1.f, -std::ilogb((float)n));
    for (int ch = 0; ch < 2; ++ch) packed_scale[ch] = normalizations[ch] ? s_phase : s_plain;
  }
  struct NormState {
      float shift[3]; size_t nout = 0;
      const float2* P = nullptr; float2 *dk = nullptr, *o1 = nullptr, *o2 = nullptr, *o3 = nullptr; size_t koff[3] = {0, 0, 0};
  };
  std::vector<NormState> state((size_t)n_norm);
  const int up_U = (int)ceilf((float)upsample_factor * 1.5f);
  const size_t up_kbytes = align_up((size_t)up_U * (size_t)(nz + ny + nx) * sizeof(float2));
  const size_t up_s1 = (size_t)nz * ny * up_U, up_s2 = (size_t)nz * up_U * up_U, up_s3 = (size_t)up_U * up_U * up_U;
  const size_t up_bytes = up_kbytes + (up_s1 + up_s2 + up_s3) * sizeof(float2) + 1024;
  char* up_base = nullptr;
  if (upsample_factor > 1) {
      up_base = (char*)mvs_scratch(c, 7, up_bytes * (size_t)n_norm);
      if (!up_base) return mvs_alloc_failed(c);
  }
  for (int inorm = 0; inorm < n_norm; ++inorm) {
    const int normalization = normalizations[inorm];
    int64_t* peak_index_out = peak_indices_out ? peak_indices_out + 3 * inorm : nullptr;
    float* peak_abs_out = peak_abs_out_all ? peak_abs_out_all + inorm : nullptr;
    const float2* P = normalization ? P1 : P2;
    const char* hpart = hred + (packed ? (size_t)inorm * ga * 16 : 0);
    const int n_part = packed ? n_red_packed : ga;
    if (!packed) {
        hipLaunchKernelGGL(xpower_packed_kernel, dim3(gb), dim3(256), 0, c->stream, Z, P1, P2, CC, nz, ny, nx, normalization ? 1 : 0, -1);
        rc = mvs_fft3_c2c(c, CC, shape, true);
        if (rc) return rc;
        hipLaunchKernelGGL(argmax_abs_kernel<0>, dim3(ga), dim3(256), 0, c->stream, CC, n, (float*)red, (long long*)(red + (size_t)ga * 8));
        MVS_HIP_TRY(c, hipGetLastError());
        MVS_HIP_TRY(c, hipStreamSynchronize(c->stream));
    }
    float best = -1.f;
    long long bi = 0;
    {
        const float* hv = (const float*)hpart;
        const long long* hi = (const long long*)(hpart + (size_t)ga * 8);
        for (int i = 0; i < n_part; ++i)
            if (hv[i] > best || (hv[i] == best && hi[i] < bi)) { best = hv[i]; bi = hi[i]; }
    }
    if (packed) best /= packed_scale[inorm];
    const long long pz = bi / ((long long)ny * nx), py = (bi / nx) % ny, px = bi % nx;
    const long long peak[3] = {pz, py, px};
    if (peak_index_out) { peak_index_out[0] = pz; peak_index_out[1] = py; peak_index_out[2] = px; }
    if (peak_abs_out) *peak_abs_out = best / (float)n;

    float (&shift)[3] = state[inorm].shift;
// ... 283 lines not shown
```

multiview-stitcher_amd/csrc/mvs_score.hip:

```cpp
#include "mvs_internal.h"
#include "mvs_prune_search.h"

#include <cstring>

#include <rocprim/rocprim.hpp>

#include <cmath>
#include <cstdlib>
#include <vector>

int mvs_stage_float_volume(MvsContext* c, const float* src, int32_t mem, long long n, int slot, float** dptr);
int mvs_device_nanminmax(MvsContext* c, const float* d_in, long long n, float* mn, float* mx, long long* nvalid);

namespace {

constexpr int kStatBlocks = 1024;
constexpr int kMaxResident = 16;
static_assert(kMaxResident == kPruneMaxCand, "PruneSearch holds one batch");
constexpr int kChunk = 8;

inline int grid_for(long long n) { return (int)std::min<long long>((n + 255) / 256, 256 * 8); }

struct Shape3 { int nz, ny, nx; };

// ... 729 lines not shown
#pragma unroll
            for (int k = 0; k < NR; ++k) {
                an[k] = __int_as_float(__builtin_amdgcn_raw_buffer_load_b32(r0, v0[k], pn0, 0));
                ao[k] = have_old ? __int_as_float(__builtin_amdgcn_raw_buffer_load_b32(r0, v0[k], po0, 0)) : 0.f;
            }
        };
        if (col < LX) load_plane(z0 - H);
        const int xrow = tid / (TX / NO), xch = tid % (TX / NO);
        const bool xact = tid < TY * (TX / NO) && y0 + xrow < S.ny - pad;
        for (int p = z0 - H; p < z1 + H; ++p) {
            if (col < LX) {
#pragma unroll
                for (int k = 0; k < NR; ++k) {
                    const int row = wrow + 4 * k;
                    if (row >= LY) break;
                    const float a = an[k], a2 = ao[k];
                    s1[k] += (double)a - (double)a2;
                    s2[k] += (double)(a * a) - (double)(a2 * a2);
                    if (p >= z0 + H) {
                        sz_[0][row][col] = (float)(s1[k] * inv);
                        sz_[1][row][col] = (float)(s2[k] * inv);
                    }
                }
                if (p + 1 < z1 + H) load_plane(p + 1);
            }
            if (p < z0 + H) continue;
            __syncthreads();
            if (col < LX) {
#pragma unroll
                for (int a = 0; a < 2; ++a) {
                    float v[NI], f[NO];
#pragma unroll
                    for (int k = 0; k < NI; ++k) v[k] = sz_[a][wrow * NO + k][col];
                    box_means<WIN, NO>(v, f);
#pragma unroll
                    for (int k = 0; k < NO; ++k) sy_[a][wrow * NO + k][col] = f[k];
                }
            }
            __syncthreads();
            if (xact) {
                float f[2][NO];
#pragma unroll
                for (int a = 0; a < 2; ++a) {
                    float v[NI];
#pragma unroll
                    for (int k = 0; k < NI; ++k) v[k] = sy_[a][xrow][xch * NO + k];
                    box_means<WIN, NO>(v, f[a]);
                }
                const int obase = ((p - H) * S.ny + y0 + xrow) * S.nx + x0 + xch * NO;
#pragma unroll
                for (int k = 0; k < NO; ++k) {
                    if (x0 + xch * NO + k >= S.nx - pad) continue;
                    ux[obase + k] = f[0][k];
                    uxx[obase + k] = f[1][k];
                }
            }
        }
        __syncthreads();
    }
}

__global__ __launch_bounds__(256) void finish_region_kernel(const float* __restrict__ pmax, const int* __restrict__ phasnan,
                                                            const double* __restrict__ psum, RegionStats* __restrict__ out,
                                                            int nblk = kStatBlocks) {
    const size_t o = (size_t)blockIdx.x * kStatBlocks;
    float mx = -INFINITY;
    int hn = 0;
    double sum = 0.0;
    for (int i = threadIdx.x; i < nblk; i += 256) { mx = fmaxf(mx, pmax[o + i]); hn |= phasnan[o + i]; sum += psum[o + i]; }
    for (int off = 32; off > 0; off >>= 1) {
        mx = fmaxf(mx, __shfl_down(mx, off)); hn |= __shfl_down(hn, off); sum += __shfl_down(sum, off);
    }
    __shared__ float s_mx[4];
    __shared__ int s_hn[4];
    __shared__ double s_sum[4];
    if ((threadIdx.x & 63) == 0) { s_mx[threadIdx.x >> 6] = mx; s_hn[threadIdx.x >> 6] = hn; s_sum[threadIdx.x >> 6] = sum; }
    __syncthreads();
    if (threadIdx.x == 0) {
        for (int w = 1; w < 4; ++w) { mx = fmaxf(mx, s_mx[w]); hn |= s_hn[w]; sum += s_sum[w]; }
        out[blockIdx.x].mx = mx; out[blockIdx.x].hasnan = hn; out[blockIdx.x].ssim_sum = sum;
    }
}

__global__ __launch_bounds__(256) void compact_kernel(const float* __restrict__ im0, const float* __restrict__ im1t, long long n,
                                                      float* __restrict__ kx, float* __restrict__ ky,
                                                      unsigned int* __restrict__ counter, const float* __restrict__ raw0) {
    constexpr int K = 8;
    __shared__ unsigned int s_wave[4];
    __shared__ unsigned int s_base;
    const int lane = threadIdx.x & 63, wave = threadIdx.x >> 6;
    const long long tile = 256LL * K;
    for (long long t0 = (long long)blockIdx.x * tile; t0 < n; t0 += (long long)gridDim.x * tile) {
        const long long i0 = t0 + (long long)threadIdx.x * K;
        float a[K], b[K];
        unsigned int cnt = 0;
#pragma unroll
        for (int k = 0; k < K; ++k) {
            const long long i = i0 + k;
            a[k] = (i < n) ? im0[i] : NAN;
            b[k] = (i < n) ? im1t[i] : NAN;
            cnt += (a[k] == a[k] && b[k] == b[k]) ? 1u : 0u;
        }
        unsigned int incl = cnt;
        for (int off = 1; off < 64; off <<= 1) {
            const unsigned int o = __shfl_up(incl, off);
            if (lane >= off) incl += o;
        }
        if (lane == 63) s_wave[wave] = incl;
        __syncthreads();
        unsigned int wbase = 0;
        for (int w = 0; w < wave; ++w) wbase += s_wave[w];
        if (threadIdx.x == 255) s_base = atomicAdd(counter, wbase + incl);
        __syncthreads();
        unsigned int p = s_base + wbase + incl - cnt;
#pragma unroll
        for (int k = 0; k < K; ++k)
            if (a[k] == a[k] && b[k] == b[k]) {
                if (raw0) reinterpret_cast<unsigned int*>(kx)[p] = (unsigned int)raw0[i0 + k];
                else kx[p] = a[k];
                ky[p] = b[k] - 1.0f;
                ++p;
            }
        __syncthreads();
    }
}

constexpr int kRankItems = 8, kRankChunk = 256 * kRankItems;

template <typename K>
__device__ __forceinline__ void chunk_average_ranks(const K* __restrict__ sorted, unsigned int n, unsigned int chunk0,
                                                    float (&rank)[kRankItems], bool (&valid)[kRankItems]) {
    __shared__ unsigned int s_first[4], s_last[4], s_edge[2];
    const unsigned int tid = threadIdx.x, lane = tid & 63, wave = tid >> 6;
    const unsigned int base = chunk0 + tid * kRankItems;
    const unsigned int chunk_end = min(chunk0 + (unsigned int)kRankChunk, n);
    K k[kRankItems + 2];
#pragma unroll
    for (int j = 0; j < kRankItems + 2; ++j) {
        const long long idx = (long long)base + j - 1;
        k[j] = (idx >= 0 && idx < (long long)n) ? sorted[idx] : (K)0;
    }
    if (tid == 0) {
        unsigned int first = chunk0;
        if (chunk0 > 0 && chunk0 < n && sorted[chunk0 - 1] == sorted[chunk0]) {
            const K key = sorted[chunk0];
            unsigned int pos = chunk0, step = 1;
            while (pos >= step && sorted[pos - step] == key) { pos -= step; step <<= 1; }
            unsigned int lo = pos >= step ? pos - step + 1 : 0, hi = pos;
            while (lo < hi) { const unsigned int m = (lo + hi) >> 1; if (sorted[m] < key) lo = m + 1; else hi = m; }
            first = lo;
        }
        s_edge[0] = first;
    }
    if (tid == 64) {
        unsigned int last = chunk_end;
        if (chunk_end < n && chunk_end > 0 && sorted[chunk_end] == sorted[chunk_end - 1]) {
            const K key = sorted[chunk_end - 1];
            unsigned int pos = chunk_end - 1, step = 1;
            while (pos + step < n && sorted[pos + step] == key) { pos += step; step <<= 1; }
            unsigned int lo = pos + 1, hi = min(pos + step, n);
            while (lo < hi) { const unsigned int m = (lo + hi) >> 1; if (sorted[m] <= key) lo = m + 1; else hi = m; }
            last = lo;
        }
        s_edge[1] = last;
    }
    unsigned int first[kRankItems], cur = 0;
#pragma unroll
    for (int j = 0; j < kRankItems; ++j) {
        const unsigned int idx = base + j;
// ... 6 lines not shown
    for (int off = 1; off < 64; off <<= 1) {
        const unsigned int o = __shfl_up(incl, off);
        if (lane >= (unsigned int)off) incl = max(incl, o);
    }
    unsigned int carry_f = __shfl_up(incl, 1);
    if (lane == 0) carry_f = 0;
    if (lane == 63) s_first[wave] = incl;
    unsigned int last[kRankItems], curl = 0xffffffffu;
#pragma unroll
    for (int j = kRankItems - 1; j >= 0; --j) {
        const unsigned int idx = base + j;
        if (idx < n && (idx == n - 1 || k[j + 1] != k[j + 2])) curl = idx + 1;
        last[j] = curl;
    }
    unsigned int incl_l = curl;
#pragma unroll
    for (int off = 1; off < 64; off <<= 1) {
        const unsigned int o = __shfl_down(incl_l, off);
        if (lane + (unsigned int)off < 64) incl_l = min(incl_l, o);
    }
    unsigned int carry_l = __shfl_down(incl_l, 1);
    if (lane == 63) carry_l = 0xffffffffu;
    if (lane == 0) s_last[wave] = incl_l;
    __syncthreads();
    for (unsigned int w = 0; w < wave; ++w) carry_f = max(carry_f, s_first[w]);
    for (unsigned int w = wave + 1; w < 4; ++w) carry_l = min(carry_l, s_last[w]);
    const unsigned int edge_first = s_edge[0], edge_last = s_edge[1];
#pragma unroll
    for (int j = 0; j < kRankItems; ++j) {
        unsigned int f = max(first[j], carry_f), l = min(last[j], carry_l);
        f = f ? f - 1 : edge_first;
        if (l == 0xffffffffu) l = edge_last;
        rank[j] = (float)(0.5 * ((double)f + (double)l + 1.0));
    }
    __syncthreads();
}

template <typename K>
__global__ __launch_bounds__(256) void ranks_sorted_kernel(const K* __restrict__ sorted, unsigned int n, float* __restrict__ rank_out) {
    const unsigned int nchunks = (n + kRankChunk - 1) / kRankChunk;
    for (unsigned int c = blockIdx.x; c < nchunks; c += gridDim.x) {
        float rank[kRankItems];
        bool valid[kRankItems];
        chunk_average_ranks(sorted, n, c * kRankChunk, rank, valid);
        const unsigned int base = c * kRankChunk + threadIdx.x * kRankItems;
        if (base + kRankItems <= n) {
            *reinterpret_cast<float4*>(rank_out + base) = make_float4(rank[0], rank[1], rank[2], rank[3]);
            *reinterpret_cast<float4*>(rank_out + base + 4) = make_float4(rank[4], rank[5], rank[6], rank[7]);
        } else {
#pragma unroll
            for (int j = 0; j < kRankItems; ++j) if (valid[j]) rank_out[base + j] = rank[j];
        }
    }
}

__global__ __launch_bounds__(256) void rankcorr_kernel(const float* __restrict__ ysorted, const float* __restrict__ rx, unsigned int n,
                                                       double mean, double* __restrict__ partial) {
    double sxy = 0.0, sxx = 0.0, syy = 0.0;
    const unsigned int nchunks = (n + kRankChunk - 1) / kRankChunk;
    for (unsigned int c = blockIdx.x; c < nchunks; c += gridDim.x) {
        float rank[kRankItems];
        bool valid[kRankItems];
        chunk_average_ranks(ysorted, n, c * kRankChunk, rank, valid);
        const unsigned int base = c * kRankChunk + threadIdx.x * kRankItems;
#pragma unroll
        for (int j = 0; j < kRankItems; ++j)
            if (valid[j]) {
                const double a = (double)rx[base + j] - mean, b = (double)rank[j] - mean;
                sxy += a * b; sxx += a * a; syy += b * b;
            }
    }
    for (int off = 32; off > 0; off >>= 1) {
        sxy += __shfl_down(sxy, off); sxx += __shfl_down(sxx, off); syy += __shfl_down(syy, off);
    }
    __shared__ double s[3][4];
    if ((threadIdx.x & 63) == 0) { s[0][threadIdx.x >> 6] = sxy; s[1][threadIdx.x >> 6] = sxx; s[2][threadIdx.x >> 6] = syy; }
    __syncthreads();
    if (threadIdx.x == 0)
        for (int k = 0; k < 3; ++k) partial[blockIdx.x * 3 + k] = s[k][0] + s[k][1] + s[k][2] + s[k][3];
}

constexpr int kHistParts = 256;
constexpr int kHistBinsMax = 48 * 1024;
__device__ __forceinline__ int shifted_keysum(const float* __restrict__ raw1, int sy, int sz, const AxisTap& Z, const AxisTap& Y,
                                              const AxisTap& X) {
    if (!(Z.ok && Y.ok && X.ok)) return -1;
    const bool fz = Z.w != 0.0, fy = Y.w != 0.0, fx = X.w != 0.0;
    float acc = 0.f;
    for (int a = 0; a <= (fz ? 1 : 0); ++a)
        for (int b = 0; b <= (fy ? 1 : 0); ++b)
            for (int q = 0; q <= (fx ? 1 : 0); ++q)
                acc += raw1[(a ? Z.i1 : Z.i0) * sz + (b ? Y.i1 : Y.i0) * sy + (q ? X.i1 : X.i0)];
    return (int)acc;
}
template <bool CORR>
__global__ __launch_bounds__(CORR ? 256 : 1024) void hist_rank_kernel(const float* __restrict__ raw0, const float* __restrict__ raw1, Shape3 S, double tz,
                                                        double ty, double tx, int kx0, int nbx, int ky0, int nby,
                                                        unsigned int* __restrict__ hx, unsigned int* __restrict__ hy,
                                                        const float* __restrict__ rx, const float* __restrict__ ry,
                                                        double* __restrict__ partial, unsigned int* __restrict__ parts) {
    extern __shared__ unsigned int s_hist[];
    const unsigned int n = (unsigned int)S.nz * S.ny * S.nx;
    const int sy = S.nx, sz = S.ny * S.nx;
    const int nwords = (nbx + nby + 1) / 2;
    if (!CORR) {
        for (int i = threadIdx.x; i < nwords; i += blockDim.x) s_hist[i] = 0u;
        __syncthreads();
    }
    double sxy = 0.0;
    const unsigned int ngroups = (n + 3) / 4;
    const unsigned int per = (ngroups + gridDim.x - 1) / gridDim.x;
    const unsigned int g0 = blockIdx.x * per, g1 = min(g0 + per, ngroups);
    for (unsigned int g = g0 + threadIdx.x; g < g1; g += blockDim.x) {
        const unsigned int i0 = g * 4;
        int x = (int)(i0 % (unsigned int)S.nx);
        const unsigned int t = i0 / (unsigned int)S.nx;
        int y = (int)(t % (unsigned int)S.ny), z = (int)(t / (unsigned int)S.ny);
        int row_z = -1, row_y = -1;
        AxisTap Z = {0, 0, 0, 0.0}, Y = {0, 0, 0, 0.0};
#pragma unroll
        for (int k = 0; k < 4; ++k) {
            if (i0 + k < n) {
                if (z != row_z || y != row_y) {
                    row_z = z; row_y = y;
                    Z = axis_tap(z, tz, S.nz);
                    Y = axis_tap(y, ty, S.ny);
                }
                const int ks = shifted_keysum(raw1, sy, sz, Z, Y, axis_tap(x, tx, S.nx));
                if (ks >= 0) {
                    const int kx = (int)raw0[i0 + k] - kx0, ky = ks - ky0;
                    if (CORR) sxy += (double)rx[kx] * (double)ry[ky];
                    else {
                        atomicAdd(&s_hist[kx >> 1], 1u << (16 * (kx & 1)));
                        const int q = nbx + ky;
                        atomicAdd(&s_hist[q >> 1], 1u << (16 * (q & 1)));
                    }
                }
                if (++x == S.nx) { x = 0; if (++y == S.ny) { y = 0; ++z; } }
            }
        }
    }
    if (CORR) {
        for (int off = 32; off > 0; off >>= 1) sxy += __shfl_down(sxy, off);
        __shared__ double s[4];
        if ((threadIdx.x & 63) == 0) s[threadIdx.x >> 6] = sxy;
        __syncthreads();
        if (threadIdx.x == 0) partial[blockIdx.x] = s[0] + s[1] + s[2] + s[3];
    } else if (parts) {
        __syncthreads();
        unsigned int* mine = parts + (size_t)blockIdx.x * nwords;
        for (int i = threadIdx.x; i < nwords; i += blockDim.x) mine[i] = s_hist[i];
    } else {
        __syncthreads();
        for (int i = threadIdx.x; i < nwords; i += blockDim.x) {
            const unsigned int w = s_hist[i];
            if (w) {
                const int b0 = 2 * i, b1 = 2 * i + 1;
                const unsigned int c0 = w & 0xffffu, c1 = w >> 16;
                if (c0) atomicAdd((b0 < nbx) ? hx + b0 : hy + (b0 - nbx), c0);
                if (c1) atomicAdd((b1 < nbx) ? hx + b1 : hy + (b1 - nbx), c1);
            }
        }
    }
}
__global__ __launch_bounds__(1024) void hist_fold_kernel(const unsigned int* __restrict__ parts, int nparts, int nwords, int nbx, int nby,
                                                         unsigned int* __restrict__ hx, unsigned int* __restrict__ hy) {
    __shared__ unsigned int s0[16][64], s1[16][64];
    const int lane = threadIdx.x & 63, q = threadIdx.x >> 6;
    const int i = blockIdx.x * 64 + lane;
    unsigned int c0 = 0, c1 = 0;
    if (i < nwords)
        for (int w = q; w < nparts; w += 16) {
            const unsigned int v = parts[(size_t)w * nwords + i];
            c0 += v & 0xffffu;
            c1 += v >> 16;
        }
    s0[q][lane] = c0; s1[q][lane] = c1;
    __syncthreads();
    if (q == 0 && i < nwords) {
// ... 517 lines not shown
    }
    return MVS_OK;
}

int score_batch(ScoreCall& sc, ScoreBatch& b, size_t n_todo) {
    MvsContext* c = sc.c;
    bool have_rs = false;
    if (b.any_batched && !c->ssim_two_pass) {
        bool prune = sc.so->argmax_only && c->ssim_prune && n_todo <= (size_t)sc.nres;
        int n_in = 0;
        for (int j = 0; j < b.nb; ++j) {
            if (b.fused.c[j].src) ++n_in;
            else if (b.scored[j]) prune = false;
        }
        const double vb = sc.so->value_bound;
        const double slack = 1e-2 * std::max(1.0, (vb / sc.data_range) * (vb / sc.data_range));
        prune = prune && n_in >= 2 && sc.data_range > 0.0 && std::isfinite(slack) && slack <= 0.05;
        if (!prune) score_full(sc, b, n_in);
        else {
            const int rc = score_pruned(sc, b, slack);
            if (rc) return rc;
            have_rs = true;
        }
    } else if (b.any_batched) {
        score_two_pass(sc, b);
    }
    bool any = false;
    for (int j = 0; j < b.nb; ++j) any = any || b.scored[j];
    if (any && !have_rs) {
        hipLaunchKernelGGL(finish_region_kernel, dim3(b.nb), dim3(256), 0, c->stream, sc.pmax, sc.phasnan, sc.psum, sc.reg_out, kStatBlocks);
        MVS_HIP_TRY(c, hipStreamSynchronize(c->stream));
        for (int j = 0; j < b.nb; ++j) b.h_rs[j] = sc.h_reg[j];
    }
    return MVS_OK;
}

void decode_results(ScoreCall& sc, const ScoreBatch& b) {
    for (int j = 0; j < b.nb; ++j) {
        const int ic = b.ics[j];
        if (sc.code_out[ic] != 0) continue;
        float region_nanmax = NAN;
        int region_hasnan = 0;
        if (b.scored[j]) {
            region_hasnan = b.h_rs[j].hasnan;
            region_nanmax = (b.h_rs[j].mx == -INFINITY) ? NAN : b.h_rs[j].mx;
        }
        if (region_nanmax <= (float)sc.im1_min) {
            sc.code_out[ic] = 2;
            continue;
        }
        const Shape3 R = b.Rs[j];
        const int win = ssim_window(sc, R);
        const float region_max = region_hasnan ? NAN : region_nanmax;
        if (win < 3 || region_max <= (float)sc.im1_min || !b.scored[j]) {
            sc.ssim_out[ic] = -1.0;
        } else {
            const int pad = (win - 1) / 2;
            double cropn = 1.0;
            for (int k = sc.k0; k < 3; ++k) cropn *= (double)((&R.nz)[k] - 2 * pad);
            sc.ssim_out[ic] = b.h_rs[j].ssim_sum / cropn;
        }
    }
}

struct HistPlan { double t[3]; long long kx0, nbx, ky0, nby, hgb; bool fold; };
bool hist_ranks_apply(const ScoreCall& sc, int ic, HistPlan* hp) {
    const MvsScoreOpts& so = *sc.so;
    sc.shift_of(ic, hp->t);
    bool halves = true;
    int nf = 0;
    for (int k = 0; k < 3; ++k) {
        halves = halves && (std::floor(hp->t[k] * 2.0) == hp->t[k] * 2.0);
        nf += (std::floor(hp->t[k]) != hp->t[k]) ? 1 : 0;
    }
    hp->kx0 = (long long)so.raw_range[0]; hp->nbx = (long long)so.raw_range[1] - hp->kx0 + 1;
    hp->ky0 = (long long)so.raw_range[2] * (1 << nf); hp->nby = ((long long)so.raw_range[3] - (long long)so.raw_range[2]) * (1 << nf) + 1;
    const long long hneed = (sc.n / 4 + 16382) / 16383;
    hp->fold = hneed <= kHistParts;
    hp->hgb = hp->fold ? std::max<long long>(hneed, std::min<long long>(kHistParts, (sc.n + 8191) / 8192)) : std::max<long long>(sc.gb, hneed);
    return halves && so.raw_u16_keys[0] && so.raw_u16_keys[1] && so.both_crops_finite && !sc.c->materialize_shifts && hp->nbx > 0 && hp->nby > 0 &&
           hp->nbx + hp->nby <= kHistBinsMax && hp->hgb <= 65535;
}

int spearman_hist(ScoreCall& sc, int ic, const HistPlan& hp) {
    MvsContext* c = sc.c;
    const MvsScoreOpts& so = *sc.so;
    const long long kx0 = hp.kx0, nbx = hp.nbx, ky0 = hp.ky0, nby = hp.nby, hgb = hp.hgb;
    unsigned int* d_hist = sc.d_hist;
    float* d_rank = sc.d_rank;
    static bool lds_attr[MVS_MAX_DEVICES] = {false};
    if (!lds_attr[mvs_hip_device(sc.device)]) {
        MVS_HIP_TRY(c, hipFuncSetAttribute((const void*)hist_rank_kernel<false>, hipFuncAttributeMaxDynamicSharedMemorySize, 128 * 1024));
        lds_attr[mvs_hip_device(sc.device)] = true;
    }
    const size_t lds_bytes = (size_t)((nbx + nby + 1) / 2) * 4;
    if (!hp.fold) MVS_HIP_TRY(c, hipMemsetAsync(d_hist, 0, sizeof(unsigned int) * (size_t)(nbx + nby), c->stream));
    MVS_DUP("hist_count", hipLaunchKernelGGL(hist_rank_kernel<false>, dim3((unsigned)hgb), dim3(1024), lds_bytes, c->stream, so.raw_u16_keys[0], so.raw_u16_keys[1],
                       sc.S, hp.t[0], hp.t[1], hp.t[2], (int)kx0, (int)nbx, (int)ky0, (int)nby, d_hist, d_hist + nbx, (const float*)nullptr,
                       (const float*)nullptr, (double*)nullptr, hp.fold ? sc.d_parts : (unsigned int*)nullptr));
    if (hp.fold) {
        const int nwords = (int)((nbx + nby + 1) / 2);
        MVS_DUP("hist_fold", hipLaunchKernelGGL(hist_fold_kernel, dim3((nwords + 63) / 64), dim3(1024), 0, c->stream, sc.d_parts, (int)hgb, nwords, (int)nbx, (int)nby,
                           d_hist, d_hist + nbx));
    }
    MVS_DUP("rank_table", hipLaunchKernelGGL(rank_table_kernel, dim3(2), dim3(1024), 0, c->stream, d_hist, (int)nbx, d_rank, d_hist + nbx, (int)nby,
                       d_rank + nbx, sc.partial));
    MVS_DUP("hist_corr", hipLaunchKernelGGL(hist_rank_kernel<true>, dim3(sc.gb), dim3(256), 0, c->stream, so.raw_u16_keys[0], so.raw_u16_keys[1], sc.S, hp.t[0], hp.t[1],
                       hp.t[2], (int)kx0, (int)nbx, (int)ky0, (int)nby, d_hist, d_hist + nbx, d_rank, d_rank + nbx, sc.partial + 4, (unsigned int*)nullptr));
    MVS_HIP_TRY(c, hipGetLastError());
    MVS_HIP_TRY(c, hipStreamSynchronize(c->stream));
    const double* hpart = sc.h_partial;
    double sxy = 0;
    for (int i = 0; i < sc.gb; ++i) sxy += hpart[4 + i];
    sc.spearman_out[ic] = sxy / std::sqrt(hpart[0] * hpart[2]);
    return MVS_OK;
}

int spearman_sorted(ScoreCall& sc, int ic, const float* im1t) {
    MvsContext* c = sc.c;
    float* const* setA = sc.setA;
    float* const* setB = sc.setB;
    if (!im1t) {
        double t[3];
        sc.shift_of(ic, t);
        hipLaunchKernelGGL(shift_kernel, dim3(kStatBlocks), dim3(256), 0, c->stream, sc.im1, sc.im0, sc.im1t_buf[0], sc.S, t[0], t[1], t[2], sc.im1_all_finite, sc.vox_partial);
        std::fill(sc.resident.begin(), sc.resident.end(), -1);
        sc.resident[ic] = 0;
        im1t = sc.im1t_buf[0];
    }
    MVS_HIP_TRY(c, hipMemsetAsync(sc.d_counter, 0, 4, c->stream));
    const float* raw0 = sc.so->raw_u16_keys[0];
    hipLaunchKernelGGL(compact_kernel, dim3(sc.gb), dim3(256), 0, c->stream, sc.im0, im1t, sc.n, setA[0], setA[1], sc.d_counter, raw0);
    const unsigned int m = (unsigned int)sc.cnts[ic];
    const int mgb = (int)std::min<long long>(((long long)m + kRankChunk - 1) / kRankChunk, 2048);
    if (raw0) {
        MVS_HIP_TRY(c, rocprim::radix_sort_pairs(sc.sort_temp, sc.sort_temp_bytes, (unsigned int*)setA[0], (unsigned int*)setA[2], setA[1], setA[3], (size_t)m,
                                                0, 16, c->stream));
        hipLaunchKernelGGL(ranks_sorted_kernel<unsigned int>, dim3(mgb), dim3(256), 0, c->stream, (const unsigned int*)setA[2], m, setA[4]);
    } else {
        MVS_HIP_TRY(c, rocprim::radix_sort_pairs(sc.sort_temp, sc.sort_temp_bytes, setA[0], setA[2], setA[1], setA[3], (size_t)m, 0, 32, c->stream));
        hipLaunchKernelGGL(ranks_sorted_kernel<float>, dim3(mgb), dim3(256), 0, c->stream, setA[2], m, setA[4]);
    }
    MVS_HIP_TRY(c, rocprim::radix_sort_pairs(sc.sort_temp, sc.sort_temp_bytes, setA[3], setB[0], setA[4], setB[1], (size_t)m, 0, 32, c->stream));
    hipLaunchKernelGGL(rankcorr_kernel, dim3(mgb), dim3(256), 0, c->stream, setB[0], setB[1], m, 0.5 * ((double)m + 1.0), sc.partial);
    MVS_HIP_TRY(c, hipGetLastError());
    MVS_HIP_TRY(c, hipStreamSynchronize(c->stream));
    const double* hp = sc.h_partial;
    double sxy = 0, sxx = 0, syy = 0;
    for (int i = 0; i < mgb; ++i) { sxy += hp[i * 3]; sxx += hp[i * 3 + 1]; syy += hp[i * 3 + 2]; }
    sc.spearman_out[ic] = sxy / std::sqrt(sxx * syy);
    return MVS_OK;
}

int spearman_from(ScoreCall& sc, int ic, const float* im1t) {
    HistPlan hp;
    return hist_ranks_apply(sc, ic, &hp) ? spearman_hist(sc, ic, hp) : spearman_sorted(sc, ic, im1t);
}

}

extern "C" int mvs_score_candidates(int device, const float* fixed, const float* moving, int32_t mem, int32_t ndim,
                                    const int64_t shape[3], const double* t_candidates, int32_t n_candidates,
                                    int32_t region_mode, double data_range, double im1_min, int32_t quality_for_all,
                                    double* ssim_out, double* spearman_out, int32_t* code_out) {
    return mvs_score_candidates_impl(device, fixed, moving, mem, ndim, shape, t_candidates, n_candidates, region_mode, data_range, im1_min,
                                     quality_for_all, ssim_out, spearman_out, code_out, MvsScoreOpts{});
}

int mvs_score_candidates_impl(int device, const float* fixed, const float* moving, int32_t mem, int32_t ndim, const int64_t shape[3],
                              const double* t_candidates, int32_t n_candidates, int32_t region_mode, double data_range, double im1_min,
                              int32_t quality_for_all, double* ssim_out, double* spearman_out, int32_t* code_out, const MvsScoreOpts& so) {
    MvsContext* c;
    int rc = mvs_check_ready(device, &c);
    if (rc) return rc;
    std::lock_guard<std::recursive_mutex> lock(c->mu);
    if (!fixed || !moving || !shape || !t_candidates || !ssim_out || !spearman_out || !code_out || n_candidates < 0)
        return mvs_fail(c, MVS_ERR_INVALID_ARG, "mvs_score_candidates: bad argument");
    if (ndim != 2 && ndim != 3) return mvs_fail(c, MVS_ERR_INVALID_ARG, "mvs_score_candidates: ndim must be 2 or 3");
    if (ndim == 2 && shape[0] != 1) return mvs_fail(c, MVS_ERR_INVALID_ARG, "mvs_score_candidates: 2D needs shape[0]==1");
    MVS_HIP_TRY(c, hipSetDevice(mvs_hip_device(device)));
    ScoreCall sc;
    sc.c = c; sc.so = &so; sc.device = device;
    sc.S = Shape3{(int)shape[0], (int)shape[1], (int)shape[2]};
    const Shape3 S = sc.S;
    const long long n = sc.n = (long long)S.nz * S.ny * S.nx;
    if (n >= (1ll << 31) - 8) return mvs_fail(c, MVS_ERR_UNSUPPORTED, "mvs_score_candidates: volume too large");
    sc.ndim = ndim; sc.k0 = 3 - ndim; sc.region_mode = region_mode; sc.quality_for_all = quality_for_all;
    sc.data_range = data_range; sc.im1_min = im1_min;
    sc.t_candidates = t_candidates; sc.ssim_out = ssim_out; sc.spearman_out = spearman_out; sc.code_out = code_out;

    rc = mvs_stage_float_volume(c, fixed, mem, n, 4, &sc.im0);
    if (rc) return rc;
    rc = mvs_stage_float_volume(c, moving, mem, n, 5, &sc.im1);
    if (rc) return rc;

    sc.nres = (int)std::max<long long>(1, std::min<long long>(std::min(kMaxResident, std::max(n_candidates, 1)), (4ll << 30) / (n * 4)));
    sc.sort_temp_bytes = 0;
    MVS_HIP_TRY(c, rocprim::radix_sort_pairs(nullptr, sc.sort_temp_bytes, (float*)nullptr, (float*)nullptr, (float*)nullptr,
                                            (float*)nullptr, (size_t)n, 0, 32, c->stream));
    {
        size_t tb16 = 0;
        MVS_HIP_TRY(c, rocprim::radix_sort_pairs(nullptr, tb16, (unsigned int*)nullptr, (unsigned int*)nullptr, (float*)nullptr,
                                                (float*)nullptr, (size_t)n, 0, 16, c->stream));
        sc.sort_temp_bytes = std::max(sc.sort_temp_bytes, tb16);
    }
    sc.gb = grid_for(n);
    sc.may_batch = ndim == 3 && region_mode == 0 && !quality_for_all && !c->materialize_shifts && (long long)n * 12 * sc.nres <= (3ll << 30);
    rc = layout_scratch(sc);
    if (rc) return rc;
    rc = image_boxes(sc);
    if (rc) return rc;

    MVS_HIP_TRY(c, hipEventRecord(c->ev_start, c->stream));
    std::vector<int> todo;
    for (int ic = 0; ic < n_candidates; ++ic) {
        double t[3];
        sc.shift_of(ic, t);
        ssim_out[ic] = -1.0;
        spearman_out[ic] = -1.0;
        code_out[ic] = 0;
        if (passes_pretest(sc, t)) todo.push_back(ic);
        else code_out[ic] = 1;
    }

    sc.cnts.assign((size_t)std::max(n_candidates, 1), 0ull);
    sc.resident.assign((size_t)std::max(n_candidates, 1), -1);
    const float Rf = (float)data_range;
    sc.C1 = (0.01f * Rf) * (0.01f * Rf);
    sc.C2 = (0.03f * Rf) * (0.03f * Rf);

    sc.shared_x = ndim == 3 && region_mode == 0 && sc.im0_all_finite && todo.size() >= 2 && std::min(S.nz, std::min(S.ny, S.nx)) >= 7 &&
                  !c->materialize_shifts;
    if (sc.shared_x)
        launch_ssim_shared_x<7>(c->stream, sc.im0, S, S, sc.setA, sc.setB, sc.pmax, sc.phasnan, !c->ssim_two_pass && (long long)S.nz * S.ny * S.nx * 4 < (1ll << 31));

    for (size_t b0 = 0; b0 < todo.size(); b0 += (size_t)sc.nres) {
        ScoreBatch b;
        b.nb = (int)std::min<size_t>((size_t)sc.nres, todo.size() - b0);
        b.ics = todo.data() + b0;
// ... 33 lines not shown
```

Before: 102,800.

## Keep registration crops in u16 and fuse rescale into first FFT pass

Crop/bin now writes both fixed and moving crops as 16-bit in one paired launch instead of float. The min/max rescale is folded into the first FFT or slab pass, which reads u16 directly and writes back the normalized floats. Spearman histogram and compact kernels are templated to take u16 raw keys. This is meant to cut memory traffic and a separate rescale launch, at the cost of more code paths and an added branch in the FFT load routines.

```diff
diff --git a/multiview-stitcher_amd/csrc/mvs_context.hip b/multiview-stitcher_amd/csrc/mvs_context.hip
--- a/multiview-stitcher_amd/csrc/mvs_context.hip
+++ b/multiview-stitcher_amd/csrc/mvs_context.hip
@@ -179,6 +179,7 @@
     {"fuse_mixed", &MvsContext::fuse_mixed},
     {"serial_classes", &MvsContext::serial_classes},
     {"reg_unfused", &MvsContext::reg_unfused},
+    {"reg_u16_crops", &MvsContext::reg_u16_crops},
     {"ssim_two_pass", &MvsContext::ssim_two_pass},
     {"ssim_f32", &MvsContext::ssim_f32},
     {"ssim_prune", &MvsContext::ssim_prune},
@@ -229,6 +230,7 @@
     {"reg_pruned", nullptr, &MvsContext::reg_pruned},
     {"reg_cand_volumes", &MvsContext::reg_cand_volumes, nullptr},
     {"reg_slab_pairs", nullptr, &MvsContext::reg_slab_pairs},
+    {"reg_u16_pairs", nullptr, &MvsContext::reg_u16_pairs},
     {"cb_mask_views", nullptr, &MvsContext::cb_mask_views},
     {"cb_mask_boxes", nullptr, &MvsContext::cb_mask_boxes},
     {"cb_line_launches", nullptr, &MvsContext::cb_line_launches},
diff --git a/multiview-stitcher_amd/csrc/mvs_fft.h b/multiview-stitcher_amd/csrc/mvs_fft.h
--- a/multiview-stitcher_amd/csrc/mvs_fft.h
+++ b/multiview-stitcher_amd/csrc/mvs_fft.h
@@ -1,9 +1,29 @@
 #pragma once
 #include "mvs_internal.h"
 
+struct MvsU16Src {
+    const unsigned short* src[2] = {nullptr, nullptr};
+    float* dst[2] = {nullptr, nullptr};
+    float lo[2] = {0.f, 0.f}, hi[2] = {0.f, 0.f};
+    int degenerate[2] = {0, 0};
+};
+__device__ __forceinline__ float mvs_rescale_value(float v, float lo, float hi, int degenerate) {
+    const float d = hi - lo;
+    v = fminf(fmaxf(v, lo), hi);
+    if (!degenerate) v = (v - lo) / d;
+    return v * 1.0f + 0.0f;
+}
+__device__ __forceinline__ float2 mvs_u16_load(const MvsU16Src& U, long long i) {
+    const float re = mvs_rescale_value((float)U.src[0][i], U.lo[0], U.hi[0], U.degenerate[0]);
+    const float im = mvs_rescale_value((float)U.src[1][i], U.lo[1], U.hi[1], U.degenerate[1]);
+    U.dst[0][i] = re;
+    U.dst[1][i] = im;
+    return make_float2(re, im);
+}
 struct MvsFftFuse {
     const float* re_src = nullptr;
     const float* im_src = nullptr;
+    MvsU16Src u16;
     const float2* xp_src = nullptr;
     float2* xp_p2 = nullptr;
     int xp_sel_a = 0, xp_sel_b = 0;
@@ -17,8 +37,11 @@
 int mvs_fft3_c2c(MvsContext* c, float2* data, const int64_t shape[3], bool inverse, MvsFftFuse* fuse = nullptr);
 int mvs_phasecorr_slab_axis(const MvsContext* c, const int64_t shape[3]);
 int mvs_phasecorr_slab_peaks(const int64_t shape[3], int short_axis);
-int mvs_phasecorr_slab(MvsContext* c, const float* a, const float* b, float2* Z, float2* CC, float2* P2, float2* dc, const int64_t shape[3],
+int mvs_phasecorr_slab(MvsContext* c, const float* a, const float* b, const MvsU16Src* u16, float2* Z, float2* CC, float2* P2, float2* dc, const int64_t shape[3],
                        int short_axis, int sel_a, int sel_b, float* const peak_val[2], long long* const peak_idx[2], float2* z0_out);
+int mvs_phasecorr_multi_impl(int device, const float* fixed, const float* moving, int32_t mem, int32_t ndim, const int64_t shape[3],
+                             const int32_t* normalizations, int32_t n_norm, int32_t upsample_factor, double* shifts_out, int64_t* peak_indices_out,
+                             float* peak_abs_out_all, const MvsU16Src* u16);
 bool mvs_fft_reg_length(int n);
 
 __device__ __forceinline__ void mvs_xpower_scales(float2 z0, long long n, float* scale_phase, float* scale_plain) {
diff --git a/multiview-stitcher_amd/csrc/mvs_fft.hip b/multiview-stitcher_amd/csrc/mvs_fft.hip
--- a/multiview-stitcher_amd/csrc/mvs_fft.hip
+++ b/multiview-stitcher_amd/csrc/mvs_fft.hip
@@ -642,7 +642,10 @@
         if (reg_pow2 || reg_blue || reg_line) {
             const int lpw = reg_line ? 64 : ((reg_pow2 && n == 64) || (reg_blue && p.M == 64)) ? 32 : 16;
             unsigned grid = (unsigned)((A.n_lines + lpw - 1) / lpw);
-            if (fuse && axis == first_axis && fuse->re_src && fuse->im_src) {
+            if (fuse && axis == first_axis && fuse->u16.src[0] && fuse->u16.src[1] && !inverse) {
+                A.u16 = fuse->u16;
+                fuse->src_used = true;
+            } else if (fuse && axis == first_axis && fuse->re_src && fuse->im_src) {
                 A.re_src = fuse->re_src;
                 A.im_src = fuse->im_src;
                 fuse->src_used = true;
diff --git a/multiview-stitcher_amd/csrc/mvs_fft_dev.h b/multiview-stitcher_amd/csrc/mvs_fft_dev.h
--- a/multiview-stitcher_amd/csrc/mvs_fft_dev.h
+++ b/multiview-stitcher_amd/csrc/mvs_fft_dev.h
@@ -16,6 +16,7 @@
     const float2* bfft;
     const float* re_src = nullptr;
     const float* im_src = nullptr;
+    MvsU16Src u16;
     float* peak_val[2] = {nullptr, nullptr};
     long long* peak_idx[2] = {nullptr, nullptr};
     const float2* xp_src = nullptr;
@@ -30,6 +31,7 @@
 }
 
 __device__ __forceinline__ float2 fft_load(const FftArgs& A, long long i) {
+    if (A.u16.src[0]) return mvs_u16_load(A.u16, i);
     if (!A.re_src) return A.data[i];
     float re = A.re_src[i], im = A.im_src[i];
     re = (re != re) ? 0.f : re;
@@ -65,6 +67,7 @@
     float2* data = nullptr;
     const float* re_src = nullptr;
     const float* im_src = nullptr;
+    MvsU16Src u16;
     int S = 0, L = 0;
     int short_contig = 0;
     int inverse = 0;
diff --git a/multiview-stitcher_amd/csrc/mvs_fft_slab.hip b/multiview-stitcher_amd/csrc/mvs_fft_slab.hip
--- a/multiview-stitcher_amd/csrc/mvs_fft_slab.hip
+++ b/multiview-stitcher_amd/csrc/mvs_fft_slab.hip
@@ -121,7 +121,7 @@
 }
 int mvs_phasecorr_slab_peaks(const int64_t shape[3], int short_axis) { return (int)(short_axis == 0 ? shape[1] : shape[0]); }
 
-int mvs_phasecorr_slab(MvsContext* c, const float* a, const float* b, float2* Z, float2* CC, float2* P2, float2* dc, const int64_t shape[3],
+int mvs_phasecorr_slab(MvsContext* c, const float* a, const float* b, const MvsU16Src* u16, float2* Z, float2* CC, float2* P2, float2* dc, const int64_t shape[3],
                        int short_axis, int sel_a, int sel_b, float* const peak_val[2], long long* const peak_idx[2], float2* z0_out) {
     const long long nz = shape[0], ny = shape[1], nx = shape[2];
     const int S = (int)shape[short_axis];
@@ -152,6 +152,7 @@
     rc = mvs_fft_twiddles(c, N2, &G.tw);
     if (rc) return rc;
     F.data = Z; F.re_src = a; F.im_src = b; F.inverse = 0; F.dc = dc;
+    if (u16) { F.u16 = *u16; F.re_src = nullptr; F.im_src = nullptr; }
     hipError_t err = hipSuccess;
     if (!(S <= 44 ? mvs_launch_slab_lo(c, F, (unsigned)nslab, lds, &err) : mvs_launch_slab_hi(c, F, (unsigned)nslab, lds, &err)))
         return mvs_fail(c, MVS_ERR_UNSUPPORTED, "phase correlation (slab path): no slab kernel for S = %d", S);
@@ -166,7 +167,7 @@
         else hipLaunchKernelGGL((long_xp_kernel<8, 8>), dim3(grid), dim3(256), 0, c->stream, G);
         MVS_HIP_TRY(c, hipGetLastError());
     }
-    F.data = CC; F.re_src = nullptr; F.im_src = nullptr; F.inverse = 1; F.dc = nullptr;
+    F.data = CC; F.re_src = nullptr; F.im_src = nullptr; F.u16 = MvsU16Src(); F.inverse = 1; F.dc = nullptr;
     for (int k = 0; k < 2; ++k) { F.peak_val[k] = peak_val[k]; F.peak_idx[k] = peak_idx[k]; }
     if (!(S <= 44 ? mvs_launch_slab_lo(c, F, (unsigned)nslab, lds, &err) : mvs_launch_slab_hi(c, F, (unsigned)nslab, lds, &err)))
         return mvs_fail(c, MVS_ERR_UNSUPPORTED, "phase correlation (slab path): no slab kernel for S = %d", S);
diff --git a/multiview-stitcher_amd/csrc/mvs_fft_slab.inc b/multiview-stitcher_amd/csrc/mvs_fft_slab.inc
--- a/multiview-stitcher_amd/csrc/mvs_fft_slab.inc
+++ b/multiview-stitcher_amd/csrc/mvs_fft_slab.inc
@@ -30,6 +30,7 @@
 }
 
 __device__ __forceinline__ float2 slab_load(const SlabArgs& A, long long g, bool inv) {
+    if (A.u16.src[0]) return mvs_u16_load(A.u16, g);
     if (A.re_src) {
         float re = A.re_src[g], im = A.im_src[g];
         re = (re != re) ? 0.f : re;
diff --git a/multiview-stitcher_amd/csrc/mvs_fuse.hip b/multiview-stitcher_amd/csrc/mvs_fuse.hip
--- a/multiview-stitcher_amd/csrc/mvs_fuse.hip
+++ b/multiview-stitcher_amd/csrc/mvs_fuse.hip
@@ -928,12 +928,19 @@
     }
 }
 
-template <typename TIn>
-__global__ __launch_bounds__(1024) void crop_bin_kernel(const TIn* __restrict__ data, long long stride_z, long long stride_y, int nz, int ny,
-                                                       int nx, int bz, int by, int bx, int tz, int ty, int tx, float* __restrict__ out, int oz,
-                                                       int oy, int ox, float cval, char* __restrict__ stats) {
+struct CropBinImage { const void* data; long long stride_z, stride_y; int nz, ny, nx, tz, ty, tx; void* out; char* stats; };
+struct CropBinArgs { CropBinImage im[2]; };
+template <typename TIn, typename TOut>
+__global__ __launch_bounds__(1024) void crop_bin_kernel(CropBinArgs P, int bz, int by, int bx, int oz, int oy, int ox, float cval) {
     typedef float f4_t __attribute__((ext_vector_type(4), aligned(4)));
     typedef unsigned int u32x4_t __attribute__((ext_vector_type(4), aligned(4)));
+    typedef unsigned short u16x8_t __attribute__((ext_vector_type(8), aligned(2)));
+    const CropBinImage& I = P.im[blockIdx.y];
+    const TIn* __restrict__ data = (const TIn*)I.data;
+    TOut* __restrict__ out = (TOut*)I.out;
+    char* __restrict__ stats = I.stats;
+    const long long stride_z = I.stride_z, stride_y = I.stride_y;
+    const int nz = I.nz, ny = I.ny, nx = I.nx, tz = I.tz, ty = I.ty, tx = I.tx;
     const int gpr = (ox + 7) / 8;
     const long long ngroups = (long long)oz * oy * gpr;
     const double inv = 1.0 / ((double)bz * by * bx);
@@ -947,7 +954,7 @@
         const long long row = g / gpr;
         const int y = (int)(row % oy), z = (int)(row / oy);
         const int iz = z + tz, iy = y + ty, ix = xg + tx;
-        float* o = out + row * ox + xg;
+        TOut* o = out + row * ox + xg;
         const bool zy = iz >= 0 && iz < nz && iy >= 0 && iy < ny;
         const TIn* p = data + (long long)iz * bz * stride_z + (long long)iy * by * stride_y + (long long)ix * bx;
         float v[8];
@@ -991,7 +998,16 @@
                 v[j] = (float)(TIn)(acc * inv);
             }
         }
-        if (xg + 8 <= ox) {
+        if constexpr (sizeof(TOut) == 2) {
+            if (xg + 8 <= ox) {
+                u16x8_t q;
+#pragma unroll
+                for (int j = 0; j < 8; ++j) q[j] = in[j] ? (unsigned short)v[j] : (unsigned short)0;
+                *reinterpret_cast<u16x8_t*>(o) = q;
+            } else {
+                for (int j = 0; j < 8 && xg + j < ox; ++j) o[j] = in[j] ? (TOut)v[j] : (TOut)0;
+            }
+        } else if (xg + 8 <= ox) {
             f4_t a, b;
             a.x = v[0]; a.y = v[1]; a.z = v[2]; a.w = v[3];
             b.x = v[4]; b.y = v[5]; b.z = v[6]; b.w = v[7];
@@ -1532,16 +1548,10 @@
 }
 
 
-int mvs_crop_bin_impl(int device, const mvs_view_t* view, const int32_t bin[3], const int64_t out_shape[3], float* out, const MvsResampleOpts& ro) {
-    MvsContext* c;
-    int rc = mvs_check_ready(device, &c);
-    if (rc) return rc;
-    std::lock_guard<std::recursive_mutex> lock(c->mu);
-    if (!view || !bin || !out_shape || !out) return mvs_fail(c, MVS_ERR_INVALID_ARG, "mvs_crop_bin: NULL argument");
+static int crop_bin_window(MvsContext* c, const mvs_view_t* view, const int32_t bin[3], const int64_t out_shape[3], int t[3], int nb3[3]) {
     if ((view->dtype != MVS_U8 && view->dtype != MVS_U16) || view->mem != MVS_MEM_DEVICE || view->stride[2] != 1)
         return mvs_fail(c, MVS_ERR_UNSUPPORTED, "mvs_crop_bin: needs a device-resident uint8 / uint16 window with unit x stride");
     const double I[9] = {1, 0, 0, 0, 1, 0, 0, 0, 1};
-    int t[3], nb3[3];
     for (int k = 0; k < 9; ++k)
         if (view->matrix[k] != I[k]) return mvs_fail(c, MVS_ERR_UNSUPPORTED, "mvs_crop_bin: the view must be a whole-pixel translation");
     for (int k = 0; k < 3; ++k) {
@@ -1553,6 +1563,25 @@
         nb3[k] = (int)(view->shape[k] / bin[k]);
     }
     if ((long long)bin[0] * bin[1] > 16384) return mvs_fail(c, MVS_ERR_UNSUPPORTED, "mvs_crop_bin: bin too large");
+    return MVS_OK;
+}
+static CropBinImage crop_bin_image(const mvs_view_t* view, const int t[3], const int nb3[3], void* out, char* stats) {
+    CropBinImage im;
+    im.data = view->data; im.stride_z = (long long)view->stride[0]; im.stride_y = (long long)view->stride[1];
+    im.nz = nb3[0]; im.ny = nb3[1]; im.nx = nb3[2]; im.tz = t[0]; im.ty = t[1]; im.tx = t[2];
+    im.out = out; im.stats = stats;
+    return im;
+}
+
+int mvs_crop_bin_impl(int device, const mvs_view_t* view, const int32_t bin[3], const int64_t out_shape[3], float* out, const MvsResampleOpts& ro) {
+    MvsContext* c;
+    int rc = mvs_check_ready(device, &c);
+    if (rc) return rc;
+    std::lock_guard<std::recursive_mutex> lock(c->mu);
+    if (!view || !bin || !out_shape || !out) return mvs_fail(c, MVS_ERR_INVALID_ARG, "mvs_crop_bin: NULL argument");
+    int t[3], nb3[3];
+    rc = crop_bin_window(c, view, bin, out_shape, t, nb3);
+    if (rc) return rc;
     MVS_HIP_TRY(c, hipSetDevice(mvs_hip_device(device)));
     const long long ng = (long long)out_shape[0] * out_shape[1] * ((out_shape[2] + 7) / 8);
     const int nthr = 1024;
@@ -1563,16 +1592,60 @@
         nblk = ro.stats->nb;
         ro.stats->done[ro.stats_k & 1] = true;
     }
+    CropBinArgs P;
+    P.im[0] = P.im[1] = crop_bin_image(view, t, nb3, out, stats);
     if (view->dtype == MVS_U8)
-        MVS_DUP("crop", hipLaunchKernelGGL(crop_bin_kernel<unsigned char>, dim3(nblk), dim3(nthr), 0, c->stream, (const unsigned char*)view->data, (long long)view->stride[0],
-                           (long long)view->stride[1], nb3[0], nb3[1], nb3[2], (int)bin[0], (int)bin[1], (int)bin[2], t[0], t[1], t[2], out,
-                           (int)out_shape[0], (int)out_shape[1], (int)out_shape[2], NAN, stats));
+        MVS_DUP("crop", hipLaunchKernelGGL((crop_bin_kernel<unsigned char, float>), dim3(nblk), dim3(nthr), 0, c->stream, P, (int)bin[0], (int)bin[1], (int)bin[2],
+                           (int)out_shape[0], (int)out_shape[1], (int)out_shape[2], NAN));
     else
-        MVS_DUP("crop", hipLaunchKernelGGL(crop_bin_kernel<unsigned short>, dim3(nblk), dim3(nthr), 0, c->stream, (const unsigned short*)view->data, (long long)view->stride[0],
-                           (long long)view->stride[1], nb3[0], nb3[1], nb3[2], (int)bin[0], (int)bin[1], (int)bin[2], t[0], t[1], t[2], out,
-                           (int)out_shape[0], (int)out_shape[1], (int)out_shape[2], NAN, stats));
+        MVS_DUP("crop", hipLaunchKernelGGL((crop_bin_kernel<unsigned short, float>), dim3(nblk), dim3(nthr), 0, c->stream, P, (int)bin[0], (int)bin[1], (int)bin[2],
+                           (int)out_shape[0], (int)out_shape[1], (int)out_shape[2], NAN));
     MVS_HIP_TRY(c, hipGetLastError());
     if (!ro.defer_sync) MVS_HIP_TRY(c, hipStreamSynchronize(c->stream));
+    return MVS_OK;
+}
+
+bool mvs_crop_bin_covers(const mvs_view_t* view, const int32_t bin[3], const int64_t out_shape[3]) {
+    if (!view || !bin || !out_shape) return false;
+    if ((view->dtype != MVS_U8 && view->dtype != MVS_U16) || view->mem != MVS_MEM_DEVICE || view->stride[2] != 1) return false;
+    for (int k = 0; k < 3; ++k) {
+        if (bin[k] < 1 || view->shape[k] < bin[k] || view->shape[k] % bin[k] || out_shape[k] < 1 || out_shape[k] > 0x7fffffffLL) return false;
+        if (!(view->offset[k] == std::floor(view->offset[k])) || std::fabs(view->offset[k]) > 1e9) return false;
+        const long long t = (long long)view->offset[k], nbk = view->shape[k] / bin[k];
+        if (t < 0 || t + out_shape[k] > nbk) return false;
+    }
+    return true;
+}
+
+int mvs_crop_bin_pair_u16_impl(int device, const mvs_view_t* fixed_view, const mvs_view_t* moving_view, const int32_t bin[3], const int64_t out_shape[3],
+                               unsigned short* out0, unsigned short* out1, MvsCropStats* stats) {
+    MvsContext* c;
+    int rc = mvs_check_ready(device, &c);
+    if (rc) return rc;
+    std::lock_guard<std::recursive_mutex> lock(c->mu);
+    if (!fixed_view || !moving_view || !bin || !out_shape || !out0 || !out1 || !stats || !stats->base || stats->nb < 1)
+        return mvs_fail(c, MVS_ERR_INVALID_ARG, "mvs_crop_bin_pair: NULL argument");
+    if (fixed_view->dtype != moving_view->dtype || !mvs_crop_bin_covers(fixed_view, bin, out_shape) || !mvs_crop_bin_covers(moving_view, bin, out_shape))
+        return mvs_fail(c, MVS_ERR_UNSUPPORTED, "mvs_crop_bin_pair: the 16-bit form needs two windows of one integer type that cover the crop");
+    const mvs_view_t* views[2] = {fixed_view, moving_view};
+    unsigned short* outs[2] = {out0, out1};
+    CropBinArgs P;
+    for (int k = 0; k < 2; ++k) {
+        int t[3], nb3[3];
+        rc = crop_bin_window(c, views[k], bin, out_shape, t, nb3);
+        if (rc) return rc;
+        P.im[k] = crop_bin_image(views[k], t, nb3, outs[k], stats->base + (size_t)k * (size_t)stats->nb * 16);
+    }
+    MVS_HIP_TRY(c, hipSetDevice(mvs_hip_device(device)));
+    const int nthr = 1024;
+    if (fixed_view->dtype == MVS_U8)
+        MVS_DUP("crop", hipLaunchKernelGGL((crop_bin_kernel<unsigned char, unsigned short>), dim3(stats->nb, 2), dim3(nthr), 0, c->stream, P, (int)bin[0], (int)bin[1],
+                           (int)bin[2], (int)out_shape[0], (int)out_shape[1], (int)out_shape[2], NAN));
+    else
+        MVS_DUP("crop", hipLaunchKernelGGL((crop_bin_kernel<unsigned short, unsigned short>), dim3(stats->nb, 2), dim3(nthr), 0, c->stream, P, (int)bin[0], (int)bin[1],
+                           (int)bin[2], (int)out_shape[0], (int)out_shape[1], (int)out_shape[2], NAN));
+    MVS_HIP_TRY(c, hipGetLastError());
+    stats->done[0] = stats->done[1] = true;
     return MVS_OK;
 }
 
diff --git a/multiview-stitcher_amd/csrc/mvs_internal.h b/multiview-stitcher_amd/csrc/mvs_internal.h
--- a/multiview-stitcher_amd/csrc/mvs_internal.h
+++ b/multiview-stitcher_amd/csrc/mvs_internal.h
@@ -35,12 +35,14 @@
     double reg_alg_bytes_full = 0.0;
     long long reg_pairs = 0, reg_candidates = 0, reg_pruned = 0;
     long long reg_slab_pairs = 0;
+    long long reg_u16_pairs = 0;
     double reg_cand_volumes = 0.0;
     hipStream_t aux_stream[4] = {nullptr, nullptr, nullptr, nullptr};
     hipEvent_t ev_fork = nullptr, ev_join[4] = {nullptr, nullptr, nullptr, nullptr};
     bool fuse_mixed = false;
     bool serial_classes = false;
     bool reg_unfused = false;
+    bool reg_u16_crops = true;
     bool ssim_f32 = true;
     long long reg_rewalks = 0;
     bool ssim_prune = true;
@@ -94,7 +96,8 @@
     bool both_crops_finite = false;
     bool argmax_only = false;
     double value_bound = INFINITY;
-    const float* raw_u16_keys[2] = {nullptr, nullptr};
+    const void* raw_u16_keys[2] = {nullptr, nullptr};
+    bool raw_keys_16bit = false;
     float raw_range[4] = {0.f, 0.f, 0.f, 0.f};
 };
 #ifdef MVS_PROFILING_ABLATIONS
@@ -118,6 +121,9 @@
                               const double* t_candidates, int32_t n_candidates, int32_t region_mode, double data_range, double im1_min,
                               int32_t quality_for_all, double* ssim_out, double* spearman_out, int32_t* code_out, const MvsScoreOpts& so);
 int mvs_crop_bin_impl(int device, const mvs_view_t* view, const int32_t bin[3], const int64_t out_shape[3], float* out, const MvsResampleOpts& ro);
+bool mvs_crop_bin_covers(const mvs_view_t* view, const int32_t bin[3], const int64_t out_shape[3]);
+int mvs_crop_bin_pair_u16_impl(int device, const mvs_view_t* fixed_view, const mvs_view_t* moving_view, const int32_t bin[3], const int64_t out_shape[3],
+                               unsigned short* out0, unsigned short* out1, MvsCropStats* stats);
 int mvs_resample_impl(int device, const mvs_view_t* view, const int64_t out_shape[3], int32_t order, float cval, float* out, int32_t out_mem,
                       const MvsResampleOpts& ro);
 
diff --git a/multiview-stitcher_amd/csrc/mvs_pair.hip b/multiview-stitcher_amd/csrc/mvs_pair.hip
--- a/multiview-stitcher_amd/csrc/mvs_pair.hip
+++ b/multiview-stitcher_amd/csrc/mvs_pair.hip
@@ -1,7 +1,7 @@
-#include "mvs_internal.h"
+#include "mvs_fft.h"
 
 int mvs_rescale_pair_device(MvsContext* c, const float* in0, const float* in1, long long n, float* out0, float* out1,
-                            float mn[2], float mx[2], long long nvalid[2], long long n_not_u16[2], const MvsCropStats* parked);
+                            float mn[2], float mx[2], long long nvalid[2], long long n_not_u16[2], const MvsCropStats* parked, MvsU16Src* u16);
 
 #include <algorithm>
 #include <cmath>
@@ -9,23 +9,24 @@
 
 static int register_crops_impl(int device, const float* fixed, const float* moving, int32_t mem, int32_t ndim, const int64_t shape[3],
                                int32_t upsample_factor, int32_t region_mode, int32_t constant_check, double t_out[3], double* quality_out,
-                               int32_t* status_out, int32_t* n_candidates_out, const MvsCropStats* parked);
+                               int32_t* status_out, int32_t* n_candidates_out, const MvsCropStats* parked, const unsigned short* const* crops16);
 
 extern "C" int mvs_register_crops(int device, const float* fixed, const float* moving, int32_t mem, int32_t ndim, const int64_t shape[3],
                                   int32_t upsample_factor, int32_t region_mode, int32_t constant_check, double t_out[3], double* quality_out,
                                   int32_t* status_out, int32_t* n_candidates_out) {
     return register_crops_impl(device, fixed, moving, mem, ndim, shape, upsample_factor, region_mode, constant_check, t_out, quality_out, status_out,
-                               n_candidates_out, nullptr);
+                               n_candidates_out, nullptr, nullptr);
 }
 
 static int register_crops_impl(int device, const float* fixed, const float* moving, int32_t mem, int32_t ndim, const int64_t shape[3],
                                int32_t upsample_factor, int32_t region_mode, int32_t constant_check, double t_out[3], double* quality_out,
-                               int32_t* status_out, int32_t* n_candidates_out, const MvsCropStats* parked) {
+                               int32_t* status_out, int32_t* n_candidates_out, const MvsCropStats* parked, const unsigned short* const* crops16) {
     MvsContext* c;
     int rc = mvs_check_ready(device, &c);
     if (rc) return rc;
     std::lock_guard<std::recursive_mutex> lock(c->mu);
-    if (!fixed || !moving || !shape || !t_out || !quality_out || !status_out)
+    if (crops16 && (mem != MVS_MEM_DEVICE || !crops16[0] || !crops16[1] || !parked)) return mvs_fail(c, MVS_ERR_INVALID_ARG, "mvs_register_crops: bad 16-bit crops");
+    if (((!fixed || !moving) && !crops16) || !shape || !t_out || !quality_out || !status_out)
         return mvs_fail(c, MVS_ERR_INVALID_ARG, "mvs_register_crops: NULL argument");
     if (ndim != 2 && ndim != 3) return mvs_fail(c, MVS_ERR_INVALID_ARG, "mvs_register_crops: ndim must be 2 or 3");
     if (ndim == 2 && shape[0] != 1) return mvs_fail(c, MVS_ERR_INVALID_ARG, "mvs_register_crops: 2D needs shape[0]==1");
@@ -43,16 +44,18 @@
     if (!r0 || !r1) return mvs_alloc_failed(c);
     float min0, max0, min1, max1;
     int64_t nv0, nv1;
-    const float* raw_keys0 = nullptr;
-    const float* raw_keys1 = nullptr;
+    const void* raw_keys0 = nullptr;
+    const void* raw_keys1 = nullptr;
+    MvsU16Src u16;
     if (mem == MVS_MEM_DEVICE) {
         MVS_HIP_TRY(c, hipSetDevice(mvs_hip_device(device)));
         float mn[2], mx[2];
         long long nv[2], not_u16[2];
-        rc = mvs_rescale_pair_device(c, fixed, moving, n, r0, r1, mn, mx, nv, not_u16, parked);
+        if (crops16) { u16.src[0] = crops16[0]; u16.src[1] = crops16[1]; }
+        rc = mvs_rescale_pair_device(c, fixed, moving, n, r0, r1, mn, mx, nv, not_u16, parked, crops16 ? &u16 : nullptr);
         if (rc) return rc;
-        raw_keys0 = (not_u16[0] == 0) ? fixed : nullptr;
-        raw_keys1 = (not_u16[1] == 0) ? moving : nullptr;
+        raw_keys0 = crops16 ? (const void*)crops16[0] : (not_u16[0] == 0) ? (const void*)fixed : nullptr;
+        raw_keys1 = crops16 ? (const void*)crops16[1] : (not_u16[1] == 0) ? (const void*)moving : nullptr;
         min0 = mn[0]; max0 = mx[0]; nv0 = nv[0];
         min1 = mn[1]; max1 = mx[1]; nv1 = nv[1];
     } else {
@@ -70,7 +73,7 @@
 
     const int32_t norms[2] = {1, 0};
     double shifts[6];
-    rc = mvs_phasecorr_multi(device, r0, r1, MVS_MEM_DEVICE, ndim, shape, norms, 2, upsample_factor, shifts, nullptr, nullptr);
+    rc = mvs_phasecorr_multi_impl(device, r0, r1, MVS_MEM_DEVICE, ndim, shape, norms, 2, upsample_factor, shifts, nullptr, nullptr, crops16 ? &u16 : nullptr);
     if (rc) return rc;
     std::vector<std::vector<float>> estimates;
     for (int e = 0; e < 2; ++e) {
@@ -142,6 +145,7 @@
                            !c->materialize_shifts;
     so.raw_u16_keys[0] = c->materialize_shifts ? nullptr : raw_keys0;
     so.raw_u16_keys[1] = c->materialize_shifts ? nullptr : raw_keys1;
+    so.raw_keys_16bit = crops16 != nullptr;
     so.raw_range[0] = min0; so.raw_range[1] = max0; so.raw_range[2] = min1; so.raw_range[3] = max1;
     so.argmax_only = true;
     so.value_bound = (double)std::max(std::max(std::fabs(lo0), std::fabs(hi0)), std::max(std::fabs(lo1), std::fabs(hi1)));
@@ -210,6 +214,14 @@
     stats.base = c->reg_unfused ? nullptr : (char*)mb_dev;
     stats.nb = nb_stats;
     stats.gen = c->mbox_gen;
+    if (bin && c->reg_u16_crops && !c->reg_unfused && fixed_view->dtype == moving_view->dtype && mvs_crop_bin_covers(fixed_view, bin, out_shape) &&
+        mvs_crop_bin_covers(moving_view, bin, out_shape)) {
+        const unsigned short* crops16[2] = {(const unsigned short*)crop0, (const unsigned short*)crop1};
+        rc = mvs_crop_bin_pair_u16_impl(device, fixed_view, moving_view, bin, out_shape, (unsigned short*)crop0, (unsigned short*)crop1, &stats);
+        if (rc) return rc;
+        return register_crops_impl(device, nullptr, nullptr, MVS_MEM_DEVICE, ndim, out_shape, upsample_factor, region_mode, constant_check, t_out,
+                                   quality_out, status_out, n_candidates_out, &stats, crops16);
+    }
     MvsResampleOpts ro;
     ro.defer_sync = true;
     ro.stats = &stats;
@@ -220,7 +232,7 @@
     rc = bin ? mvs_crop_bin_impl(device, moving_view, bin, out_shape, crop1, ro) : mvs_resample_impl(device, moving_view, out_shape, 1, NAN, crop1, MVS_MEM_DEVICE, ro);
     if (rc) return rc;
     return register_crops_impl(device, crop0, crop1, MVS_MEM_DEVICE, ndim, out_shape, upsample_factor, region_mode, constant_check, t_out,
-                               quality_out, status_out, n_candidates_out, &stats);
+                               quality_out, status_out, n_candidates_out, &stats, nullptr);
 }
 
 
diff --git a/multiview-stitcher_amd/csrc/mvs_reg.hip b/multiview-stitcher_amd/csrc/mvs_reg.hip
--- a/multiview-stitcher_amd/csrc/mvs_reg.hip
+++ b/multiview-stitcher_amd/csrc/mvs_reg.hip
@@ -316,10 +316,10 @@
     }
 }
 
-struct PairPtrs { const float* in[2]; float* out[2]; float lo[2], hi[2]; int degenerate[2]; };
+struct PairPtrs { const void* in[2]; float* out[2]; float lo[2], hi[2]; int degenerate[2]; };
 __global__ __launch_bounds__(256) void nanminmax_pair_kernel(PairPtrs P, long long n, char* __restrict__ partials, int nb) {
     const int k = blockIdx.y;
-    const float* __restrict__ a = P.in[k];
+    const float* __restrict__ a = (const float*)P.in[k];
     char* part = partials + (size_t)k * nb * 16;
     float mn = INFINITY, mx = -INFINITY;
     long long nv = 0;
@@ -347,15 +347,16 @@
         ((long long*)(part + (size_t)nb * 8))[blockIdx.x] = nv;
     }
 }
+template <typename TIn>
 __global__ void rescale_pair_kernel(PairPtrs P, long long n) {
     const int k = blockIdx.y;
-    const float* __restrict__ src = P.in[k];
+    const TIn* __restrict__ src = (const TIn*)P.in[k];
     float* __restrict__ dst = P.out[k];
     const float lo = P.lo[k], hi = P.hi[k];
     const int degenerate = P.degenerate[k];
     const float d = hi - lo;
     for (long long i = (long long)blockIdx.x * blockDim.x + threadIdx.x; i < n; i += (long long)gridDim.x * blockDim.x) {
-        float v = src[i];
+        float v = (float)src[i];
         if (v == v) {
             v = fminf(fmaxf(v, lo), hi);
             if (!degenerate) v = (v - lo) / d;
@@ -403,7 +404,7 @@
 }
 
 int mvs_rescale_pair_device(MvsContext* c, const float* in0, const float* in1, long long n, float* out0, float* out1,
-                            float mn[2], float mx[2], long long nvalid[2], long long n_not_u16[2], const MvsCropStats* parked) {
+                            float mn[2], float mx[2], long long nvalid[2], long long n_not_u16[2], const MvsCropStats* parked, MvsU16Src* u16) {
     const int nb = std::min(grid_for(n), 512);
     void *mb_host = nullptr, *mb_dev = nullptr;
     int rcm = mvs_mailbox(c, (size_t)nb * 32, &mb_host, &mb_dev);
@@ -411,7 +412,9 @@
     char* scratch = (char*)mb_dev;
     PairPtrs PP;
     PP.in[0] = in0; PP.in[1] = in1; PP.out[0] = out0; PP.out[1] = out1;
-    if (!(parked && parked->done[0] && parked->done[1] && parked->nb == nb && parked->gen == c->mbox_gen && (void*)parked->base == mb_dev))
+    const bool have_parked = parked && parked->done[0] && parked->done[1] && parked->nb == nb && parked->gen == c->mbox_gen && (void*)parked->base == mb_dev;
+    if (u16 && !have_parked) return mvs_fail(c, MVS_ERR_INVALID_ARG, "intensity normalisation: 16-bit crops without their parked statistics");
+    if (!have_parked)
         hipLaunchKernelGGL(nanminmax_pair_kernel, dim3(nb, 2), dim3(256), 0, c->stream, PP, n, scratch, nb);
     MVS_HIP_TRY(c, hipGetLastError());
     MVS_HIP_TRY(c, hipStreamSynchronize(c->stream));
@@ -429,7 +432,11 @@
         mn[k] = a; mx[k] = b; nvalid[k] = v;
         PP.lo[k] = a; PP.hi[k] = b; PP.degenerate[k] = a == b ? 1 : 0;
     }
-    MVS_DUP("rescale", hipLaunchKernelGGL(rescale_pair_kernel, dim3(nb, 2), dim3(256), 0, c->stream, PP, n));
+    if (u16) {
+        for (int k = 0; k < 2; ++k) { u16->dst[k] = PP.out[k]; u16->lo[k] = PP.lo[k]; u16->hi[k] = PP.hi[k]; u16->degenerate[k] = PP.degenerate[k]; }
+        return MVS_OK;
+    }
+    MVS_DUP("rescale", hipLaunchKernelGGL(rescale_pair_kernel<float>, dim3(nb, 2), dim3(256), 0, c->stream, PP, n));
     MVS_HIP_TRY(c, hipGetLastError());
     return MVS_OK;
 }
@@ -508,6 +515,14 @@
                                    const int64_t shape[3], const int32_t* normalizations, int32_t n_norm,
                                    int32_t upsample_factor, double* shifts_out, int64_t* peak_indices_out,
                                    float* peak_abs_out_all) {
+    return mvs_phasecorr_multi_impl(device, fixed, moving, mem, ndim, shape, normalizations, n_norm, upsample_factor, shifts_out, peak_indices_out,
+                                    peak_abs_out_all, nullptr);
+}
+
+int mvs_phasecorr_multi_impl(int device, const float* fixed, const float* moving, int32_t mem, int32_t ndim,
+                             const int64_t shape[3], const int32_t* normalizations, int32_t n_norm,
+                             int32_t upsample_factor, double* shifts_out, int64_t* peak_indices_out,
+                             float* peak_abs_out_all, const MvsU16Src* u16) {
     MvsContext* c;
     int rc = mvs_check_ready(device, &c);
     if (rc) return rc;
@@ -519,6 +534,8 @@
     for (int k = 0; k < 3; ++k)
         if (shape[k] < 1) return mvs_fail(c, MVS_ERR_INVALID_ARG, "mvs_phasecorr: bad shape");
     if (ndim == 2 && shape[0] != 1) return mvs_fail(c, MVS_ERR_INVALID_ARG, "mvs_phasecorr: 2D needs shape[0]==1");
+    if (u16 && (mem != MVS_MEM_DEVICE || !u16->src[0] || !u16->src[1] || u16->dst[0] != fixed || u16->dst[1] != moving))
+        return mvs_fail(c, MVS_ERR_INVALID_ARG, "mvs_phasecorr: bad 16-bit source");
     MVS_HIP_TRY(c, hipSetDevice(mvs_hip_device(device)));
     const long long n = (long long)shape[0] * shape[1] * shape[2];
     const int nz = (int)shape[0], ny = (int)shape[1], nx = (int)shape[2];
@@ -542,13 +559,27 @@
     const int slab_axis = (ndim == 3 && n_norm == 2 && (normalizations[0] != 0) != (normalizations[1] != 0) && !c->materialize_shifts &&
                            (int)ceilf((float)upsample_factor * 1.5f) <= 4)
                               ? mvs_phasecorr_slab_axis(c, shape) : -1;
+    const bool first_fused = slab_axis >= 0 || (first_axis >= 0 && mvs_fft_reg_length((int)shape[first_axis]) && !c->reg_unfused);
+    if (u16 && !first_fused) {
+        PairPtrs PP;
+        for (int k = 0; k < 2; ++k) {
+            PP.in[k] = u16->src[k]; PP.out[k] = u16->dst[k];
+            PP.lo[k] = u16->lo[k]; PP.hi[k] = u16->hi[k]; PP.degenerate[k] = u16->degenerate[k];
+        }
+        MVS_DUP("rescale", hipLaunchKernelGGL(rescale_pair_kernel<unsigned short>, dim3(std::min(gb, 512), 2), dim3(256), 0, c->stream, PP, n));
+        MVS_HIP_TRY(c, hipGetLastError());
+        u16 = nullptr;
+    }
+    if (u16) c->reg_u16_pairs += 1;
     if (slab_axis >= 0) {
         rc = MVS_OK;
-    } else if (first_axis >= 0 && mvs_fft_reg_length((int)shape[first_axis]) && !c->reg_unfused) {
+    } else if (first_fused) {
         MvsFftFuse ff;
         ff.re_src = da;
         ff.im_src = db;
+        if (u16) ff.u16 = *u16;
         rc = mvs_fft3_c2c(c, Z, shape, false, &ff);
+        if (!rc && u16 && !ff.src_used) return mvs_fail(c, MVS_ERR_UNSUPPORTED, "phase correlation: the normalising first pass was not taken");
     } else {
         hipLaunchKernelGGL(pack_pair_kernel, dim3(gb), dim3(256), 0, c->stream, da, db, Z, n);
         rc = mvs_fft3_c2c(c, Z, shape, false);
@@ -580,7 +611,7 @@
   if (packed && slab_axis >= 0) {
     float* pv[2] = {(float*)red, (float*)(red + (size_t)ga * 16)};
     long long* pi[2] = {(long long*)(red + (size_t)ga * 8), (long long*)(red + (size_t)ga * 24)};
-    rc = mvs_phasecorr_slab(c, da, db, Z, CC, P2, P1 , shape, slab_axis, normalizations[0] ? 1 : 0,
+    rc = mvs_phasecorr_slab(c, da, db, u16, Z, CC, P2, P1 , shape, slab_axis, normalizations[0] ? 1 : 0,
                             normalizations[1] ? 1 : 0, pv, pi, (float2*)((char*)mb_dev + mb_z0));
     if (rc) return rc;
     n_red_packed = mvs_phasecorr_slab_peaks(shape, slab_axis);
diff --git a/multiview-stitcher_amd/csrc/mvs_score.hip b/multiview-stitcher_amd/csrc/mvs_score.hip
--- a/multiview-stitcher_amd/csrc/mvs_score.hip
+++ b/multiview-stitcher_amd/csrc/mvs_score.hip
@@ -835,9 +835,10 @@
     }
 }
 
+template <typename TKey>
 __global__ __launch_bounds__(256) void compact_kernel(const float* __restrict__ im0, const float* __restrict__ im1t, long long n,
                                                       float* __restrict__ kx, float* __restrict__ ky,
-                                                      unsigned int* __restrict__ counter, const float* __restrict__ raw0) {
+                                                      unsigned int* __restrict__ counter, const TKey* __restrict__ raw0) {
     constexpr int K = 8;
     __shared__ unsigned int s_wave[4];
     __shared__ unsigned int s_base;
@@ -1010,7 +1011,8 @@
 
 constexpr int kHistParts = 256;
 constexpr int kHistBinsMax = 48 * 1024;
-__device__ __forceinline__ int shifted_keysum(const float* __restrict__ raw1, int sy, int sz, const AxisTap& Z, const AxisTap& Y,
+template <typename TKey>
+__device__ __forceinline__ int shifted_keysum(const TKey* __restrict__ raw1, int sy, int sz, const AxisTap& Z, const AxisTap& Y,
                                               const AxisTap& X) {
     if (!(Z.ok && Y.ok && X.ok)) return -1;
     const bool fz = Z.w != 0.0, fy = Y.w != 0.0, fx = X.w != 0.0;
@@ -1018,11 +1020,11 @@
     for (int a = 0; a <= (fz ? 1 : 0); ++a)
         for (int b = 0; b <= (fy ? 1 : 0); ++b)
             for (int q = 0; q <= (fx ? 1 : 0); ++q)
-                acc += raw1[(a ? Z.i1 : Z.i0) * sz + (b ? Y.i1 : Y.i0) * sy + (q ? X.i1 : X.i0)];
+                acc += (float)raw1[(a ? Z.i1 : Z.i0) * sz + (b ? Y.i1 : Y.i0) * sy + (q ? X.i1 : X.i0)];
     return (int)acc;
 }
-template <bool CORR>
-__global__ __launch_bounds__(CORR ? 256 : 1024) void hist_rank_kernel(const float* __restrict__ raw0, const float* __restrict__ raw1, Shape3 S, double tz,
+template <bool CORR, typename TKey>
+__global__ __launch_bounds__(CORR ? 256 : 1024) void hist_rank_kernel(const TKey* __restrict__ raw0, const TKey* __restrict__ raw1, Shape3 S, double tz,
                                                         double ty, double tx, int kx0, int nbx, int ky0, int nby,
                                                         unsigned int* __restrict__ hx, unsigned int* __restrict__ hy,
                                                         const float* __restrict__ rx, const float* __restrict__ ry,
@@ -1706,20 +1708,23 @@
            hp->nbx + hp->nby <= kHistBinsMax && hp->hgb <= 65535;
 }
 
+template <typename TKey>
 int spearman_hist(ScoreCall& sc, int ic, const HistPlan& hp) {
     MvsContext* c = sc.c;
     const MvsScoreOpts& so = *sc.so;
+    const TKey* key0 = (const TKey*)so.raw_u16_keys[0];
+    const TKey* key1 = (const TKey*)so.raw_u16_keys[1];
     const long long kx0 = hp.kx0, nbx = hp.nbx, ky0 = hp.ky0, nby = hp.nby, hgb = hp.hgb;
     unsigned int* d_hist = sc.d_hist;
     float* d_rank = sc.d_rank;
     static bool lds_attr[MVS_MAX_DEVICES] = {false};
     if (!lds_attr[mvs_hip_device(sc.device)]) {
-        MVS_HIP_TRY(c, hipFuncSetAttribute((const void*)hist_rank_kernel<false>, hipFuncAttributeMaxDynamicSharedMemorySize, 128 * 1024));
+        MVS_HIP_TRY(c, hipFuncSetAttribute((const void*)hist_rank_kernel<false, TKey>, hipFuncAttributeMaxDynamicSharedMemorySize, 128 * 1024));
         lds_attr[mvs_hip_device(sc.device)] = true;
     }
     const size_t lds_bytes = (size_t)((nbx + nby + 1) / 2) * 4;
     if (!hp.fold) MVS_HIP_TRY(c, hipMemsetAsync(d_hist, 0, sizeof(unsigned int) * (size_t)(nbx + nby), c->stream));
-    MVS_DUP("hist_count", hipLaunchKernelGGL(hist_rank_kernel<false>, dim3((unsigned)hgb), dim3(1024), lds_bytes, c->stream, so.raw_u16_keys[0], so.raw_u16_keys[1],
+    MVS_DUP("hist_count", hipLaunchKernelGGL((hist_rank_kernel<false, TKey>), dim3((unsigned)hgb), dim3(1024), lds_bytes, c->stream, key0, key1,
                        sc.S, hp.t[0], hp.t[1], hp.t[2], (int)kx0, (int)nbx, (int)ky0, (int)nby, d_hist, d_hist + nbx, (const float*)nullptr,
                        (const float*)nullptr, (double*)nullptr, hp.fold ? sc.d_parts : (unsigned int*)nullptr));
     if (hp.fold) {
@@ -1729,7 +1734,7 @@
     }
     MVS_DUP("rank_table", hipLaunchKernelGGL(rank_table_kernel, dim3(2), dim3(1024), 0, c->stream, d_hist, (int)nbx, d_rank, d_hist + nbx, (int)nby,
                        d_rank + nbx, sc.partial));
-    MVS_DUP("hist_corr", hipLaunchKernelGGL(hist_rank_kernel<true>, dim3(sc.gb), dim3(256), 0, c->stream, so.raw_u16_keys[0], so.raw_u16_keys[1], sc.S, hp.t[0], hp.t[1],
+    MVS_DUP("hist_corr", hipLaunchKernelGGL((hist_rank_kernel<true, TKey>), dim3(sc.gb), dim3(256), 0, c->stream, key0, key1, sc.S, hp.t[0], hp.t[1],
                        hp.t[2], (int)kx0, (int)nbx, (int)ky0, (int)nby, d_hist, d_hist + nbx, d_rank, d_rank + nbx, sc.partial + 4, (unsigned int*)nullptr));
     MVS_HIP_TRY(c, hipGetLastError());
     MVS_HIP_TRY(c, hipStreamSynchronize(c->stream));
@@ -1753,8 +1758,11 @@
         im1t = sc.im1t_buf[0];
     }
     MVS_HIP_TRY(c, hipMemsetAsync(sc.d_counter, 0, 4, c->stream));
-    const float* raw0 = sc.so->raw_u16_keys[0];
-    hipLaunchKernelGGL(compact_kernel, dim3(sc.gb), dim3(256), 0, c->stream, sc.im0, im1t, sc.n, setA[0], setA[1], sc.d_counter, raw0);
+    const void* raw0 = sc.so->raw_u16_keys[0];
+    if (raw0 && sc.so->raw_keys_16bit)
+        hipLaunchKernelGGL(compact_kernel<unsigned short>, dim3(sc.gb), dim3(256), 0, c->stream, sc.im0, im1t, sc.n, setA[0], setA[1], sc.d_counter, (const unsigned short*)raw0);
+    else
+        hipLaunchKernelGGL(compact_kernel<float>, dim3(sc.gb), dim3(256), 0, c->stream, sc.im0, im1t, sc.n, setA[0], setA[1], sc.d_counter, (const float*)raw0);
     const unsigned int m = (unsigned int)sc.cnts[ic];
     const int mgb = (int)std::min<long long>(((long long)m + kRankChunk - 1) / kRankChunk, 2048);
     if (raw0) {
@@ -1778,7 +1786,8 @@
 
 int spearman_from(ScoreCall& sc, int ic, const float* im1t) {
     HistPlan hp;
-    return hist_ranks_apply(sc, ic, &hp) ? spearman_hist(sc, ic, hp) : spearman_sorted(sc, ic, im1t);
+    if (!hist_ranks_apply(sc, ic, &hp)) return spearman_sorted(sc, ic, im1t);
+    return sc.so->raw_keys_16bit ? spearman_hist<unsigned short>(sc, ic, hp) : spearman_hist<float>(sc, ic, hp);
 }
 
 }
```

New measurement: 104,700, median of 6. +1.8%, better.
